# dgaddy/silent_speech

Measured on AMD Instinct MI355X. Metric: EMG frames/s training (transduction_model.py), higher is better.
Workload: dtype bf16

## Files before the change

include/silent_speech_hip.h:

```cpp
#ifndef SILENT_SPEECH_HIP_H
#define SILENT_SPEECH_HIP_H
#include <stdint.h>
#ifdef __cplusplus
extern "C" {
#endif

#define SS_F32 0
#define SS_BF16 1
#define SS_F32X3 3

const char* ss_last_error(void);
#define SS_ABI_VERSION 10
int ss_abi_version(void);
const char* ss_target_arch(void);

typedef struct ss_rowmap {
    int64_t base;
    int64_t batch_stride;
    int64_t row_stride;
    int32_t rows_per_batch;
} ss_rowmap;

typedef struct ss_gemm_epilogue {
    const float* bias;
    const void* gate;
    float gate_scale;
    float alpha;
    int32_t relu;
    float dropout_p;
    uint64_t seed;
    uint32_t rng_stream;
    int32_t mode;
    int32_t col_mod, col_mul, col_div_mul;
    float log_clamp;
    void* c2;
    ss_rowmap cmap2;
    int64_t col_stride2;
    float* col_sum;
    float* col_sumsq;
    const float* col_shift;
    void* planes_hi;
    void* planes_lo;
    int32_t planes_only;
    void* sign_out;
    int64_t sign_pitch;
    const void* gate_bits;
    int64_t gate_bits_pitch;
} ss_gemm_epilogue;

#define SS_OP_KC 0
#define SS_OP_OC 1

int ss_gemm(int dtype_in, int dtype_out, int a_mode, int b_mode, const void* A, const void* B, void* C,
            int M, int N, int K, const ss_rowmap* amap, const ss_rowmap* bmap, const ss_rowmap* cmap,
            const ss_gemm_epilogue* epilogue, int split_k, void* stream);

int ss_split_planes(const float* x, void* hi, void* lo, int64_t n, void* stream);
int ss_gemm_planes(int dtype_out, const void* A_hi, const void* A_lo, const void* B_hi, const void* B_lo, void* C, int M, int N, int K,
                   const ss_rowmap* amap, const ss_rowmap* bmap, const ss_rowmap* cmap, const ss_gemm_epilogue* epilogue, void* stream);
int ss_gemm_sign_bits_supported(int dtype_in, int dtype_out, int a_mode, int b_mode, const void* C, int M, int N, int K, const ss_rowmap* amap,
                                const ss_rowmap* bmap, const ss_rowmap* cmap, const ss_gemm_epilogue* epilogue, int split_k);
int ss_gemm_planes_supported(int dtype_out, const void* C, int M, int N, int K, const ss_rowmap* amap, const ss_rowmap* bmap, const ss_rowmap* cmap,
                             const ss_gemm_epilogue* epilogue);

int ss_gemm_set_blocks_per_cu(int n);
int ss_gemm_last_kernel(void);
int ss_gemm_fuses_column_stats(int dtype_in, int dtype_out, int a_mode, int b_mode, const void* C, int M, int N, int K, const ss_rowmap* amap,
                               const ss_rowmap* bmap, const ss_rowmap* cmap, const ss_gemm_epilogue* epilogue, int split_k);
int ss_gemm_set_option(int what, int value);

typedef struct ss_dw_job {
    const void* A;
    const void* B;
    float* C;
    ss_rowmap amap, bmap;
    int64_t ldc;
    int32_t M, N, K;
    int32_t flags;
} ss_dw_job;
int ss_gemm_dw_grouped(int n_jobs, const ss_dw_job* jobs , void* stream);
int ss_gemm_dw_set_option(int what, int value);

int ss_permute3d(const void* in, int in_dtype, void* out, int out_dtype, int d0, int d1, int d2,
                 int64_t s0, int64_t s1, int64_t s2, int valid1, int valid2, float scale, int accumulate,
                 void* stream);

int ss_permute3d_batch(const void* jobs_dev, const int32_t* job_of_block_dev, int total_blocks, int all_f32, void* stream);

int ss_dtw_source(int n, int m, int64_t stride_i, int64_t stride_j);
int64_t ss_dtw_workspace_bytes(int n, int m, int64_t* sk_bytes, int64_t* dirs_bytes, int64_t* bnd_bytes);
int ss_dtw_align(const float* costs, const int64_t* desc_dev, int n, int max_n, int max_m, void* workspace,
                 int32_t* results, void* stream);
int ss_dtw_align_skewed(const int64_t* desc_dev, int n, void* workspace, int32_t* results, void* stream);
int ss_dtw_cumulative(int dtype, const void* costs, int64_t stride_i, int64_t stride_j, int N, int M, void* dtw_out,
                      int32_t* results, void* stream);

int64_t ss_bn_scratch_floats(int B, int T, int C);
int ss_bn_stats_sums(int dtype, const void* x, int B, int T, int C, int pad, float* scratch, const float* shift, float* sums, void* stream);
int ss_bn_finalize(const float* sums, double n_total, int C, float* mean, float* invstd, float* running_mean, float* running_var,
                   float momentum, float eps, int training, void* stream);
int ss_bn_finalize_shift(const float* sums, const float* shift, double n_total, int C, float* mean, float* invstd, float* running_mean,
                         float* running_var, float momentum, float eps, int training, void* stream);
int ss_bn_apply(int dtype, const void* xa, const float* mean_a, const float* invstd_a, const float* gamma_a, const float* beta_a, int pad_xa,
                const void* xb, const float* mean_b, const float* invstd_b, const float* gamma_b, const float* beta_b, int pad_xb,
                void* y, int pad_y, int B, int T, int C, int relu, void* stream);
int ss_bn_backward_sums(int dtype, const void* dy, int pad_dy, const void* y, int pad_y,
                        const void* xa, int pad_xa, const float* mean_a, const float* invstd_a,
                        const void* xb, int pad_xb, const float* mean_b, const float* invstd_b,
                        float* dgamma_a, float* dbeta_a, float* dgamma_b, float* dbeta_b,
                        float* scratch, float* sums, int B, int T, int C, int relu,
                        const float* gate_gamma_a, const float* gate_beta_a, const float* gate_gamma_b, const float* gate_beta_b, void* stream);
int ss_bn_backward_apply(int dtype, const void* dy, int pad_dy, const void* y, int pad_y,
                         const void* xa, int pad_xa, const float* mean_a, const float* invstd_a, const float* gamma_a,
                         const void* xb, int pad_xb, const float* mean_b, const float* invstd_b, const float* gamma_b,
                         const float* sums, double n_total, void* dxa, int pad_dxa, void* dxb, int pad_dxb,
                         int B, int T, int C, int relu, const float* gate_beta_a, const float* gate_beta_b, void* stream);
int64_t ss_colsum_scratch_floats(int rows, int C);
int ss_colsum(int dtype, const void* x, int rows, int C, int64_t ld, float* scratch, float* out_accum, void* stream);

int ss_add_dropout_layernorm_forward(int dtype, const void* x, void* branch_inout, const float* gamma, const float* beta, void* y,
                                     float* mean, float* rstd, int rows, int C, float eps, float dropout_p, uint64_t seed,
                                     uint32_t rng_stream, void* stream);
int ss_layernorm_backward(int dtype, const void* dy, const void* z, const float* mean, const float* rstd, const float* gamma,
                          void* dres, void* dbranch, float* dgamma, float* dbeta, int rows, int C, float dropout_p, uint64_t seed,
                          uint32_t rng_stream, void* stream);

int ss_layernorm_backward_bias(int dtype, const void* dy, const void* z, const float* mean, const float* rstd, const float* gamma,
                               void* dres, void* dbranch, float* dgamma, float* dbeta, float* dbranch_colsum, int rows, int C, float dropout_p,
                               uint64_t seed, uint32_t rng_stream, void* stream);
int64_t ss_layernorm_backward_scratch_floats(int rows, int C);
int ss_layernorm_backward_ws(int dtype, const void* dy, const void* z, const float* mean, const float* rstd, const float* gamma,
                             void* dres, void* dbranch, float* dgamma, float* dbeta, float* dbranch_colsum, float* scratch, int64_t scratch_floats,
                             int rows, int C, float dropout_p, uint64_t seed, uint32_t rng_stream, void* stream);
int ss_add_dropout_layernorm_forward_planes(int dtype, const void* x, void* branch_inout, const float* gamma, const float* beta, void* y, void* y_hi, void* y_lo,
                                            float* mean, float* rstd, int rows, int C, float eps, float dropout_p, uint64_t seed, uint32_t rng_stream, void* stream);
int ss_layernorm_backward_ws_planes(int dtype, const void* dy, const void* z, const float* mean, const float* rstd, const float* gamma,
                                    void* dres, void* dbranch, void* dbranch_hi, void* dbranch_lo, float* dgamma, float* dbeta, float* dbranch_colsum, float* scratch,
                                    int64_t scratch_floats, int rows, int C, float dropout_p, uint64_t seed, uint32_t rng_stream, void* stream);

int ss_emg_prepare(int dtype, const float* x_raw, void* out_padded, float* shifted_copy, int B, int T0, int Cin, int shift, void* stream);

int ss_loss_index_tables(const int64_t* utt_dev, int n_utt, int32_t* vo_pred, int32_t* vo_tgt, int32_t* si_tgt, int32_t* si_base,
                         int32_t* si_res, void* stream);
int ss_frame_lse(const float* head, int64_t ld, int col0, int ncls, int rows, float* lse, int32_t* argmax, void* stream);
int ss_voiced_loss(const float* head, int64_t ld, int n_mel, int n_phone, const float* lse, const int32_t* argmax, const float* Y,
                   const int64_t* phones, const int32_t* pred_row, const int32_t* tgt_row, int nframes, float lam, float inv_total,
                   float* dhead, float* loss_accum, int32_t* correct_accum, void* stream);
int ss_silent_cost_skewed(const float* head, int64_t ld, int n_mel, const float* lse, const float* Y, const int64_t* phones,
                          const int64_t* desc_dev, int n, int max_n, int max_m, float lam, void* workspace, int32_t* results, void* stream);
int ss_silent_loss(const float* head, int64_t ld, int n_mel, int n_phone, const float* lse, const int32_t* argmax, const float* Y,
                   const int64_t* phones, const int32_t* results, const int32_t* tgt_row, const int32_t* pred_base,
                   const int32_t* res_idx, int nframes, float lam, float inv_total, float* dhead, float* loss_accum,
                   int32_t* correct_accum, void* stream);
int ss_phoneme_confusion(const int32_t* argmax, const int64_t* phones, const int32_t* results, const int32_t* vo_pred, const int32_t* vo_tgt,
                         int n_voiced, const int32_t* si_tgt, const int32_t* si_base, const int32_t* si_res, int n_silent_frames,
                         int32_t* confusion, int n_phone, void* stream);

int ss_ctc_loss(const float* logits, int64_t ld, int V, int blank, const float* lse, const int64_t* desc_dev, int n_utt, int max_target_len,
                int64_t rows, const int32_t* targets, float* alpha_ws, float* beta_ws, float* nll, float* dlogits, float* loss, void* stream);

int ss_adamw_step(float* p, const float* g, float* m, float* v, int64_t n, float lr, float beta1, float beta2, float eps,
                  float weight_decay, int step, float grad_scale, void* stream);
int ss_cast_f32(const float* in, void* out, int out_dtype, int64_t n, void* stream);
int ss_soft_clip(const float* x, float* out, int64_t n, int C, const float* mean, const float* stdv, float pre_div, float limit, void* stream);

int ss_concat_pad(const void* table_dev, int n, void* out, int64_t total_bytes, int granule, void* stream);

int ss_reflect_pad(const float* y, float* out, int B, int L, int pad, int64_t ld_out, void* stream);
int ss_reflect_pad_ragged(const float* y, const int64_t* offsets_dev, const int32_t* lengths_dev, float* out, int B, int min_len,
                          int pad, int64_t ld_out, int clip, void* stream);
int ss_stft_magnitude(const float* spec, int64_t ld_spec, int n_bins, float* mag, int64_t ld_mag, int rows, void* stream);
int ss_stft_logmel_fft(const float* y, const int64_t* offsets_dev, const int32_t* lengths_dev, int64_t uniform_len, int B, int F, int pad, int clip,
                       int n_fft, int hop, const float* window,
                       const int32_t* band_lo, const int32_t* band_cnt, const int32_t* band_off, const float* band_w, const int32_t* lane_bands, int n_mels, int n_w,
                       float log_clamp, float* out, int64_t stride_b, int64_t stride_f, int64_t stride_m, void* stream);

int ss_relpos_attention_needs_transposed(int dtype, int T, int dp, int D);
int ss_relpos_attention_family(int dtype, int T, int dp, int D);
int64_t ss_relpos_attention_table_bytes(int H, int dp, int D);
int ss_relpos_attention_prepare_tables(const float* emb, void* tab, int H, int D, int dh, int dp, float scale, void* stream);
int ss_relpos_attention_forward(int dtype, const void* qkv, const void* qkvT, const void* E, const void* tab, void* out, float* lse,
                                int B, int H, int T, int Tp, int dp, int D, float scale, float dropout_p, uint64_t seed,
                                uint32_t rng_stream, void* stream);
int ss_relpos_attention_backward(int dtype, const void* qkv, const void* qkvT, const void* E, const void* ET, const void* tab, const void* out,
                                 const float* lse, const void* dO, const void* dOT, float* Dscratch, void* dqkv,
                                 int B, int H, int T, int Tp, int dp, int D, float scale, float dropout_p, uint64_t seed,
                                 uint32_t rng_stream, void* stream);

int64_t ss_relpos_attention_saved_bytes(int dtype, int B, int H, int T, int dp, int D);
int ss_relpos_attention_forward_p(int dtype, const void* qkv, const void* qkvT, const void* E, const void* tab, void* out, float* lse, void* pimg,
                                  int B, int H, int T, int Tp, int dp, int D, float scale, float dropout_p, uint64_t seed,
                                  uint32_t rng_stream, void* stream);
int ss_relpos_attention_backward_p(int dtype, const void* qkv, const void* qkvT, const void* E, const void* ET, const void* tab, const void* out,
                                   const float* lse, const void* dO, const void* dOT, float* Dscratch, void* dqkv, const void* pimg,
                                   int B, int H, int T, int Tp, int dp, int D, float scale, float dropout_p, uint64_t seed,
                                   uint32_t rng_stream, void* stream);

int ss_relpos_attention_x3_supported(int T, int dp, int D);
int64_t ss_relpos_attention_x3_saved_bytes(int B, int H, int T, int dp, int D);
int64_t ss_relpos_attention_x3_table_bytes(int H, int dp, int D);
int ss_relpos_attention_x3_prepare_tables(const float* emb, void* tab, int H, int D, int dh, int dp, float scale, void* stream);
// ... 47 lines not shown
```

silent_speech_amd/_lib.py:

```python
import ctypes
import os

import torch

_HERE = os.path.dirname(os.path.abspath(__file__))
_LIB_PATH = os.environ.get('SS_AMD_LIBRARY') or os.path.join(_HERE, 'lib', 'libsilent_speech_hip.so')

SS_F32, SS_BF16, SS_F64, SS_F32X3 = 0, 1, 2, 3
ABI_VERSION = 10
OP_KC, OP_OC = 0, 1


class RowMap(ctypes.Structure):
    _fields_ = [('base', ctypes.c_int64), ('batch_stride', ctypes.c_int64), ('row_stride', ctypes.c_int64),
                ('rows_per_batch', ctypes.c_int32)]


class GemmEpilogue(ctypes.Structure):
    _fields_ = [('bias', ctypes.c_void_p), ('gate', ctypes.c_void_p), ('gate_scale', ctypes.c_float),
                ('alpha', ctypes.c_float), ('relu', ctypes.c_int32), ('dropout_p', ctypes.c_float),
                ('seed', ctypes.c_uint64), ('rng_stream', ctypes.c_uint32), ('mode', ctypes.c_int32),
                ('col_mod', ctypes.c_int32), ('col_mul', ctypes.c_int32), ('col_div_mul', ctypes.c_int32),
                ('log_clamp', ctypes.c_float), ('c2', ctypes.c_void_p), ('cmap2', RowMap), ('col_stride2', ctypes.c_int64),
                ('col_sum', ctypes.c_void_p), ('col_sumsq', ctypes.c_void_p), ('col_shift', ctypes.c_void_p),
                ('planes_hi', ctypes.c_void_p), ('planes_lo', ctypes.c_void_p), ('planes_only', ctypes.c_int32),
                ('sign_out', ctypes.c_void_p), ('sign_pitch', ctypes.c_int64), ('gate_bits', ctypes.c_void_p), ('gate_bits_pitch', ctypes.c_int64)]


class DwJob(ctypes.Structure):
    _fields_ = [('A', ctypes.c_void_p), ('B', ctypes.c_void_p), ('C', ctypes.c_void_p), ('amap', RowMap), ('bmap', RowMap),
                ('ldc', ctypes.c_int64), ('M', ctypes.c_int32), ('N', ctypes.c_int32), ('K', ctypes.c_int32), ('flags', ctypes.c_int32)]


class ProfileRow(ctypes.Structure):
    _fields_ = [('name', ctypes.c_char * 64), ('calls', ctypes.c_int64), ('seconds', ctypes.c_double), ('flops', ctypes.c_double), ('bytes', ctypes.c_double)]


class PermuteJob(ctypes.Structure):
    _fields_ = [('inp', ctypes.c_void_p), ('out', ctypes.c_void_p), ('s0', ctypes.c_int64), ('s1', ctypes.c_int64), ('s2', ctypes.c_int64),
                ('o0', ctypes.c_int64), ('o1', ctypes.c_int64), ('d0', ctypes.c_int32), ('d1', ctypes.c_int32), ('d2', ctypes.c_int32),
                ('valid1', ctypes.c_int32), ('valid2', ctypes.c_int32), ('in_dtype', ctypes.c_int32), ('out_dtype', ctypes.c_int32),
                ('accumulate', ctypes.c_int32), ('scale', ctypes.c_float), ('first_block', ctypes.c_int32), ('nblocks', ctypes.c_int32),
                ('pad_', ctypes.c_int32)]


_P, _I, _F, _L = ctypes.c_void_p, ctypes.c_int, ctypes.c_float, ctypes.c_int64
_U64, _U32 = ctypes.c_uint64, ctypes.c_uint32

SIGNATURES = {
    'ss_gemm': [_I, _I, _I, _I, _P, _P, _P, _I, _I, _I, ctypes.POINTER(RowMap), ctypes.POINTER(RowMap),
                ctypes.POINTER(RowMap), ctypes.POINTER(GemmEpilogue), _I, _P],
    'ss_gemm_dw_grouped': [_I, ctypes.POINTER(DwJob), _P],
    'ss_split_planes': [_P, _P, _P, _L, _P],
    'ss_gemm_planes': [_I, _P, _P, _P, _P, _P, _I, _I, _I, ctypes.POINTER(RowMap), ctypes.POINTER(RowMap), ctypes.POINTER(RowMap), ctypes.POINTER(GemmEpilogue), _P],
    'ss_permute3d': [_P, _I, _P, _I, _I, _I, _I, _L, _L, _L, _I, _I, _F, _I, _P],
    'ss_permute3d_batch': [_P, _P, _I, _I, _P],
    'ss_dtw_align': [_P, _P, _I, _I, _I, _P, _P, _P],
    'ss_dtw_align_skewed': [_P, _I, _P, _P, _P],
    'ss_reflect_pad_ragged': [_P, _P, _P, _P, _I, _I, _I, _L, _I, _P],
    'ss_concat_pad': [_P, _I, _P, _L, _I, _P],
    'ss_dtw_cumulative': [_I, _P, _L, _L, _I, _I, _P, _P, _P],
    'ss_relpos_attention_forward': [_I, _P, _P, _P, _P, _P, _P, _I, _I, _I, _I, _I, _I, _F, _F, _U64, _U32, _P],
    'ss_relpos_attention_backward': [_I, _P, _P, _P, _P, _P, _P, _P, _P, _P, _P, _P, _I, _I, _I, _I, _I, _I, _F, _F, _U64, _U32, _P],
    'ss_relpos_attention_forward_p': [_I, _P, _P, _P, _P, _P, _P, _P, _I, _I, _I, _I, _I, _I, _F, _F, _U64, _U32, _P],
    'ss_relpos_attention_backward_p': [_I, _P, _P, _P, _P, _P, _P, _P, _P, _P, _P, _P, _P, _I, _I, _I, _I, _I, _I, _F, _F, _U64, _U32, _P],
    'ss_relpos_attention_prepare_tables': [_P, _P, _I, _I, _I, _I, _F, _P],
    'ss_relpos_attention_x3_prepare_tables': [_P, _P, _I, _I, _I, _I, _F, _P],
    'ss_relpos_attention_x3_forward': [_P, _P, _P, _P, _P, _P, _P, _I, _I, _I, _I, _I, _F, _F, _U64, _U32, _P],
    'ss_relpos_attention_x3_backward': [_P, _P, _P, _P, _P, _P, _P, _P, _P, _P, _P, _I, _I, _I, _I, _I, _F, _F, _U64, _U32, _P],
    'ss_bn_stats_sums': [_I, _P, _I, _I, _I, _I, _P, _P, _P, _P],
    'ss_bn_finalize': [_P, ctypes.c_double, _I, _P, _P, _P, _P, _F, _F, _I, _P],
    'ss_bn_finalize_shift': [_P, _P, ctypes.c_double, _I, _P, _P, _P, _P, _F, _F, _I, _P],
    'ss_bn_apply': [_I, _P, _P, _P, _P, _P, _I, _P, _P, _P, _P, _P, _I, _P, _I, _I, _I, _I, _I, _P],
    'ss_bn_backward_sums': [_I, _P, _I, _P, _I, _P, _I, _P, _P, _P, _I, _P, _P, _P, _P, _P, _P, _P, _P, _I, _I, _I, _I, _P, _P, _P, _P, _P],
    'ss_bn_backward_apply': [_I, _P, _I, _P, _I, _P, _I, _P, _P, _P, _P, _I, _P, _P, _P, _P, ctypes.c_double, _P, _I, _P, _I, _I, _I, _I, _I, _P, _P, _P],
    'ss_colsum': [_I, _P, _I, _I, _L, _P, _P, _P],
    'ss_add_dropout_layernorm_forward': [_I, _P, _P, _P, _P, _P, _P, _P, _I, _I, _F, _F, _U64, _U32, _P],
    'ss_add_dropout_layernorm_forward_planes': [_I, _P, _P, _P, _P, _P, _P, _P, _P, _P, _I, _I, _F, _F, _U64, _U32, _P],
    'ss_layernorm_backward': [_I, _P, _P, _P, _P, _P, _P, _P, _P, _P, _I, _I, _F, _U64, _U32, _P],
    'ss_layernorm_backward_bias': [_I, _P, _P, _P, _P, _P, _P, _P, _P, _P, _P, _I, _I, _F, _U64, _U32, _P],
    'ss_layernorm_backward_ws': [_I, _P, _P, _P, _P, _P, _P, _P, _P, _P, _P, _P, _L, _I, _I, _F, _U64, _U32, _P],
    'ss_layernorm_backward_ws_planes': [_I, _P, _P, _P, _P, _P, _P, _P, _P, _P, _P, _P, _P, _P, _L, _I, _I, _F, _U64, _U32, _P],
    'ss_emg_prepare': [_I, _P, _P, _P, _I, _I, _I, _I, _P],
    'ss_frame_lse': [_P, _L, _I, _I, _I, _P, _P, _P],
    'ss_loss_index_tables': [_P, _I, _P, _P, _P, _P, _P, _P],
    'ss_voiced_loss': [_P, _L, _I, _I, _P, _P, _P, _P, _P, _P, _I, _F, _F, _P, _P, _P, _P],
    'ss_silent_cost_skewed': [_P, _L, _I, _P, _P, _P, _P, _I, _I, _I, _F, _P, _P, _P],
    'ss_silent_loss': [_P, _L, _I, _I, _P, _P, _P, _P, _P, _P, _P, _P, _I, _F, _F, _P, _P, _P, _P],
    'ss_phoneme_confusion': [_P, _P, _P, _P, _P, _I, _P, _P, _P, _I, _P, _I, _P],
    'ss_ctc_loss': [_P, _L, _I, _I, _P, _P, _I, _I, _L, _P, _P, _P, _P, _P, _P, _P],
    'ss_adamw_step': [_P, _P, _P, _P, _L, _F, _F, _F, _F, _F, _I, _F, _P],
    'ss_cast_f32': [_P, _P, _I, _L, _P],
    'ss_soft_clip': [_P, _P, _L, _I, _P, _P, _F, _F, _P],
    'ss_reflect_pad': [_P, _P, _I, _I, _I, _L, _P],
    'ss_iir_filtfilt': [_P, _P, _I, _I, _I, _P, _P, _L, _P],
    'ss_linear_resample': [_P, _P, _I, _I, ctypes.c_double, ctypes.c_double, _I, _P],
    'ss_iir_filtfilt_batch': [_P, _P, _P, _I, _I, _I, _P, _P, _L, _P],
    'ss_linear_resample_batch': [_P, _P, _P, _I, _I, ctypes.c_double, ctypes.c_double, _L, _P],
    'ss_emg_features_batch': [_P, _P, _P, _I, _I, _L, _P],
    'ss_stft_magnitude': [_P, _L, _I, _P, _L, _I, _P],
    'ss_stft_logmel_fft': [_P, _P, _P, _L, _I, _I, _I, _I, _I, _I, _P, _P, _P, _P, _P, _P, _I, _I, _F, _P, _L, _L, _L, _P],
}
_LP = ctypes.POINTER(ctypes.c_int64)
_HOST_FUNCS = {'ss_dtw_workspace_bytes': ([_I, _I, _LP, _LP, _LP], ctypes.c_int64),
               'ss_dtw_source': ([_I, _I, _L, _L], ctypes.c_int),
               'ss_bn_scratch_floats': ([_I, _I, _I], ctypes.c_int64),
               'ss_iir_filtfilt_workspace_bytes': ([_I, _I, _I], ctypes.c_int64),
               'ss_iir_filtfilt_batch_workspace_bytes': ([_P, _I, _I, _I, _I], ctypes.c_int64),
               'ss_colsum_scratch_floats': ([_I, _I], ctypes.c_int64),
               'ss_gemm_set_blocks_per_cu': ([_I], ctypes.c_int),
               'ss_gemm_last_kernel': ([], ctypes.c_int),
               'ss_gemm_set_option': ([_I, _I], ctypes.c_int),
               'ss_gemm_fuses_column_stats': ([_I, _I, _I, _I, _P, _I, _I, _I, ctypes.POINTER(RowMap), ctypes.POINTER(RowMap), ctypes.POINTER(RowMap),
                                               ctypes.POINTER(GemmEpilogue), _I], ctypes.c_int),
               'ss_gemm_sign_bits_supported': ([_I, _I, _I, _I, _P, _I, _I, _I, ctypes.POINTER(RowMap), ctypes.POINTER(RowMap), ctypes.POINTER(RowMap),
                                                ctypes.POINTER(GemmEpilogue), _I], ctypes.c_int),
               'ss_gemm_planes_supported': ([_I, _P, _I, _I, _I, ctypes.POINTER(RowMap), ctypes.POINTER(RowMap), ctypes.POINTER(RowMap), ctypes.POINTER(GemmEpilogue)], ctypes.c_int),
               'ss_gemm_dw_set_option': ([_I, _I], ctypes.c_int),
               'ss_plan_create': ([_P], _P), 'ss_plan_destroy': ([_P], None), 'ss_plan_slot_count': ([_P], ctypes.c_int),
               'ss_plan_slot_name': ([_P, _I], ctypes.c_char_p), 'ss_plan_bind': ([_P, _I, _P], ctypes.c_int),
               'ss_plan_set_option': ([_P, _I, _I], ctypes.c_int), 'ss_plan_set_reduce_hook': ([_P, _P, _P], ctypes.c_int),
               'ss_plan_set_event_hook': ([_P, _P, _P], ctypes.c_int), 'ss_plan_ctx_bytes': ([], ctypes.c_int64),
               'ss_plan_workspace_bytes': ([_P, _I, _I, _I], ctypes.c_int64),
               'ss_plan_forward': ([_P, _P, _P, _P, _L, _I, _I, _I, _I, _F, _U64, _P, _P, _P], ctypes.c_int),
               'ss_plan_backward': ([_P, _P, _P, _P, _P], ctypes.c_int),
               'ss_counters_add': ([_I, _P, _L, _P], ctypes.c_int),
               'ss_plan_profile': ([_P, _I], ctypes.c_int), 'ss_plan_profile_read': ([_P, _P, _I], ctypes.c_int),
               'ss_relpos_attention_needs_transposed': ([_I, _I, _I, _I], ctypes.c_int),
               'ss_relpos_attention_family': ([_I, _I, _I, _I], ctypes.c_int),
               'ss_relpos_attention_table_bytes': ([_I, _I, _I], ctypes.c_int64),
               'ss_relpos_attention_x3_supported': ([_I, _I, _I], ctypes.c_int),
               'ss_relpos_attention_x3_saved_bytes': ([_I, _I, _I, _I, _I], ctypes.c_int64),
               'ss_relpos_attention_x3_table_bytes': ([_I, _I, _I], ctypes.c_int64),
               'ss_relpos_attention_saved_bytes': ([_I, _I, _I, _I, _I, _I], ctypes.c_int64),
               'ss_layernorm_backward_scratch_floats': ([_I, _I], ctypes.c_int64)}
_RESTYPES = {'ss_last_error': ctypes.c_char_p, 'ss_target_arch': ctypes.c_char_p, 'ss_abi_version': ctypes.c_int}

_lib = None
_is_emulator = False


def _declare(lib):
    for name, restype in _RESTYPES.items():
        fn = getattr(lib, name)
        fn.restype = restype
        fn.argtypes = []
    for name, argtypes in SIGNATURES.items():
        fn = getattr(lib, name)
        fn.argtypes = argtypes
        fn.restype = ctypes.c_int
    for name, (argtypes, restype) in _HOST_FUNCS.items():
        fn = getattr(lib, name)
        fn.argtypes = argtypes
        fn.restype = restype
    return lib


def load(path=None, _testing=False):
    global _lib, _is_emulator
# ... 75 lines not shown
```

silent_speech_amd/csrc/gemm8_dw.hip:

```cpp
#include "gemm8_common.h"

struct DwJob {
    const bf16_t* A; const bf16_t* B; float* C;
    RowMap amap, bmap;
    long long ldc;
    int M, N, K;
    int tiles_n, ntiles, split, k_chunk, item0, nitem, atomic;
};
constexpr int DW_MAX_JOBS = 24;
struct DwJobs { DwJob job[DW_MAX_JOBS]; int n; };

namespace g8 {
constexpr int TRP = 544;
constexpr int TR_STAGE = 2 * 64 * TRP;

template <int NR>
struct StageTR8 {
    static constexpr int RS = 64 / NR;
    const unsigned char* pa; const unsigned char* pb;
    unsigned offa[NR], offb[NR];
    int tt[NR];
    int c, r0, rpb, wraps;
    unsigned stepa, stepb, wrapa, wrapb;
    __device__ __forceinline__ void init(const DwJob& J, int m0, int n0, int k_begin, int tid) {
        c = tid & 31; r0 = tid >> 5;
        const int ca = m0 + c * 8 < J.M ? m0 + c * 8 : 0, cb = n0 + c * 8 < J.N ? n0 + c * 8 : 0;
        pa = (const unsigned char*)(J.A + J.amap.base + ca); pb = (const unsigned char*)(J.B + J.bmap.base + cb);
        rpb = J.amap.rows_per_batch;
        wraps = rpb >= BK8 ? 1 : (BK8 + rpb - 1) / rpb;
        stepa = (unsigned)(J.amap.row_stride * BK8 * 2); stepb = (unsigned)(J.bmap.row_stride * BK8 * 2);
        wrapa = (unsigned)((J.amap.batch_stride - (long long)rpb * J.amap.row_stride) * 2);
        wrapb = (unsigned)((J.bmap.batch_stride - (long long)rpb * J.bmap.row_stride) * 2);
#pragma unroll
        for (int i = 0; i < NR; ++i) {
            const int rr = k_begin + r0 + RS * i;
            int b_ = 0, t_ = rr;
            if (rpb != 0x7fffffff) { b_ = rr / rpb; t_ = rr - b_ * rpb; }
            tt[i] = t_;
            offa[i] = (unsigned)(((long long)b_ * J.amap.batch_stride + (long long)t_ * J.amap.row_stride) * 2);
            offb[i] = (unsigned)(((long long)b_ * J.bmap.batch_stride + (long long)t_ * J.bmap.row_stride) * 2);
        }
    }
    __device__ __forceinline__ void advance() {
#pragma unroll
        for (int i = 0; i < NR; ++i) {
            tt[i] += BK8; offa[i] += stepa; offb[i] += stepb;
            for (int w = 0; w < wraps; ++w) { const bool over = tt[i] >= rpb; tt[i] -= over ? rpb : 0; offa[i] += over ? wrapa : 0u; offb[i] += over ? wrapb : 0u; }
        }
    }
    template <bool PRED>
    __device__ __forceinline__ void load(int k0, int kend, u32x4 (&ra)[NR], u32x4 (&rb)[NR]) {
#pragma unroll
        for (int i = 0; i < NR; ++i) {
            if (PRED) {
                u32x4 z = {0u, 0u, 0u, 0u};
                const bool v = k0 + r0 + RS * i < kend;
                ra[i] = v ? *(const u32x4*)(pa + offa[i]) : z;
                rb[i] = v ? *(const u32x4*)(pb + offb[i]) : z;
            } else {
                ra[i] = *(const u32x4*)(pa + offa[i]);
                rb[i] = *(const u32x4*)(pb + offb[i]);
            }
        }
    }
    __device__ __forceinline__ void store(unsigned char* stage, const u32x4 (&ra)[NR], const u32x4 (&rb)[NR]) {
#pragma unroll
        for (int i = 0; i < NR; ++i) { *(u32x4*)(stage + (r0 + RS * i) * TRP + c * 16) = ra[i]; *(u32x4*)(stage + (64 + r0 + RS * i) * TRP + c * 16) = rb[i]; }
    }
};
__device__ __forceinline__ bf16x8 tr_frag8(const unsigned char* tile, int sub, int kk, int c, int q) {
    const unsigned char* a0 = tile + (kk * 32 + q * 4 + (c >> 2)) * TRP + sub * 32 + (c & 3) * 8;
    const s16x4 lo = lds_read_tr16(a0), hi = lds_read_tr16(a0 + 16 * TRP);
    bf16x8 f = {lo[0], lo[1], lo[2], lo[3], hi[0], hi[1], hi[2], hi[3]};
    return f;
}
}

template <int PIN, int NW>
__global__ __launch_bounds__(NW * 64) void gemm8_dw_kernel(DwJobs jobs, int nitems, int xorder)
{
    constexpr int NWN = NW / 2, NJ = 16 / NWN, NR = 2048 / (NW * 64);
    using namespace g8;
    SS_DYN_SMEM(lds_raw);
    unsigned char* lds = (unsigned char*)lds_raw;
    const int tid = threadIdx.x, lane = tid & 63, c = lane & 15, q = lane >> 4;
    const int wave = wave_uniform(tid >> 6);
    const int wm = wave / NWN, wn = wave % NWN, G = gridDim.x;
    StageTR8<NR> st;
    u32x4 ra[NR], rb[NR];
    int it = blockIdx.x, ji = 0, m0, n0, k_begin, k_end, nsteps;

#define G8_SETUP()                                                                                                          \
    do {                                                                                                                     \
                                                                                   \
        const int ch0_ = it / G * G, pos_ = it - ch0_;                                                                       \
        int R_ = nitems - ch0_; R_ = R_ > G ? G : R_;                                                                        \
        const int xq_ = R_ >> 3, xr_ = R_ & 7, xcd_ = pos_ & 7;                                                             \
        const int lit = xorder ? ch0_ + (xcd_ < xr_ ? xcd_ * (xq_ + 1) : xr_ * (xq_ + 1) + (xcd_ - xr_) * xq_) + (pos_ >> 3) : it; \
        ji = 0;                                                                                                              \
        while (ji + 1 < jobs.n && lit >= jobs.job[ji].item0 + jobs.job[ji].nitem) ++ji;                                     \
        const DwJob& J_ = jobs.job[ji];                                                                                      \
        const int local = lit - J_.item0, z = local / J_.ntiles, tile = local - z * J_.ntiles;                               \
        const int mt_ = tile / J_.tiles_n, nt_ = tile - mt_ * J_.tiles_n;                                                    \
        m0 = mt_ * 256; n0 = nt_ * 256;                                                                                      \
        k_begin = z * J_.k_chunk; k_end = min(J_.K, k_begin + J_.k_chunk);                                                   \
        nsteps = (k_end - k_begin + BK8 - 1) / BK8;                                                                          \
        st.init(J_, m0, n0, k_begin, tid);                                                                                   \
        if (nsteps == 1) st.template load<true>(k_begin, k_end, ra, rb); else if (nsteps > 1) st.template load<false>(k_begin, k_end, ra, rb); \
    } while (0)

    G8_SETUP();
    for (;;) {
        f32x4 acc[8][NJ];
#pragma unroll
        for (int i = 0; i < 8; ++i)
#pragma unroll
            for (int j = 0; j < NJ; ++j) { f32x4 z = {0.f, 0.f, 0.f, 0.f}; acc[i][j] = z; }
        if (nsteps > 0) st.store(lds, ra, rb);
        __syncthreads();
        for (int s = 0; s < nsteps; ++s) {
            const int cur = s & 1;
            const bool more = s + 1 < nsteps;
            if (more) {
                st.advance();
                const int k0 = k_begin + (s + 1) * BK8;
                if (s + 2 == nsteps) st.template load<true>(k0, k_end, ra, rb); else st.template load<false>(k0, k_end, ra, rb);
            }
            const unsigned char* As = lds + cur * TR_STAGE;
            const unsigned char* Bs = As + 64 * TRP;
#pragma unroll
            for (int kk = 0; kk < 2; ++kk) {
                bf16x8 a[8], b[NJ];
#pragma unroll
                for (int i = 0; i < 8; ++i) a[i] = tr_frag8(As, wm * 8 + i, kk, c, q);
#pragma unroll
                for (int j = 0; j < NJ; ++j) b[j] = tr_frag8(Bs, wn * NJ + j, kk, c, q);
                if (PIN) sched_fence();
#pragma unroll
                for (int i = 0; i < 8; ++i)
#pragma unroll
                    for (int j = 0; j < NJ; ++j) acc[i][j] = mfma_bf16_16x16x32(a[i], b[j], acc[i][j]);
                if (PIN) sched_fence();
            }
            if (more) st.store(lds + (cur ^ 1) * TR_STAGE, ra, rb);
            __syncthreads();
        }
        const DwJob& J = jobs.job[ji];
        float* Cj = J.C; const long long ldc = J.ldc; const int Mj = J.M, Nj = J.N, atomic = J.atomic, cm0 = m0, cn0 = n0;
        const bool has_next = it + G < nitems;
        if (has_next) { it += G; G8_SETUP(); }
#pragma unroll
        for (int i = 0; i < 8; ++i)
#pragma unroll
            for (int j = 0; j < NJ; ++j) {
                const int col = cn0 + (wn * NJ + j) * 16 + c, row0 = cm0 + (wm * 8 + i) * 16 + q * 4;
                if (col < Nj) {
#pragma unroll
                    for (int reg = 0; reg < 4; ++reg) {
                        if (row0 + reg < Mj) {
                            float* dst = Cj + (long long)(row0 + reg) * ldc + col;
                            if (atomic) atomicAdd(dst, acc[i][j][reg]); else *dst += acc[i][j][reg];
                        }
                    }
                }
            }
        if (!has_next) break;
    }
#undef G8_SETUP
}

namespace g8 {
constexpr int KP = 144;
constexpr int KS = 34;
constexpr int KROWS = 8 * KS;
constexpr int KT_STAGE = 2 * KROWS * KP;

__device__ __forceinline__ unsigned perm_lo(unsigned hi_src, unsigned lo_src) {
#if defined(SS_EMU)
    return (lo_src & 0xffffu) | (hi_src << 16);
#else
    return __builtin_amdgcn_perm(hi_src, lo_src, 0x05040100u);
#endif
}
__device__ __forceinline__ unsigned perm_hi(unsigned hi_src, unsigned lo_src) {
#if defined(SS_EMU)
    return (lo_src >> 16) | (hi_src & 0xffff0000u);
#else
    return __builtin_amdgcn_perm(hi_src, lo_src, 0x07060302u);
#endif
}

struct StageKT {
    const unsigned char* p;
    unsigned off[2], step, wrap, rs;
    int tt[2], rpb, kb;
    unsigned wr;
    __device__ __forceinline__ void init(const DwJob& J, int opsel, int m0, int n0, int k_begin, int wave, int lane) {
        const int c = (lane & 15) + 16 * (wave & 1), r = (lane >> 4) + 4 * ((wave >> 1) & 1);
        const RowMap& map = opsel ? J.bmap : J.amap;
        const int outer = opsel ? n0 : m0, lim = opsel ? J.N : J.M;
        const int col = outer + c * 8 < lim ? outer + c * 8 : 0;
        p = (const unsigned char*)((opsel ? J.B : J.A) + map.base + col);
        rpb = map.rows_per_batch; kb = 4 * r;
        rs = (unsigned)(map.row_stride * 2); step = (unsigned)(map.row_stride * BK8 * 2);
        wrap = (unsigned)((map.batch_stride - (long long)rpb * map.row_stride) * 2);
#pragma unroll
        for (int h = 0; h < 2; ++h) {
            const int rr = k_begin + 32 * h + kb;
            int b_ = 0, t_ = rr;
            if (rpb != 0x7fffffff) { b_ = rr / rpb; t_ = rr - b_ * rpb; }
            tt[h] = t_;
            off[h] = (unsigned)(((long long)b_ * map.batch_stride + (long long)t_ * map.row_stride) * 2);
        }
        wr = (unsigned)((opsel * KROWS + c) * KP + r * 8);
    }
    template <int H>
    __device__ __forceinline__ void advance() {
        tt[H] += BK8; off[H] += step;
        const bool over = tt[H] >= rpb; tt[H] -= over ? rpb : 0; off[H] += over ? wrap : 0u;
    }
    template <int H, bool PRED>
    __device__ __forceinline__ void load(int k0, int kend, u32x4 (&L)[4]) {
        const unsigned char* q = p + off[H];
        if constexpr (PRED) {
            u32x4 T[4];
#pragma unroll
            for (int i = 0; i < 4; ++i) { const u32x4 z = {0u, 0u, 0u, 0u}; T[i] = k0 + 32 * H + kb + i < kend ? *(const u32x4*)(q + i * rs) : z; }
#if !defined(SS_EMU)
            __builtin_amdgcn_s_waitcnt(0x0F70);
#endif
#pragma unroll
            for (int i = 0; i < 4; ++i) L[i] = T[i];
        } else {
#pragma unroll
            for (int i = 0; i < 4; ++i) {
#if defined(SS_EMU)
                L[i] = *(const u32x4*)(q + i * rs);
#else
                asm volatile("global_load_dwordx4 %0, %1, off" : "=v"(L[i]) : "v"(q + i * rs) : "memory");
#endif
            }
        }
    }
    template <int N>
    __device__ __forceinline__ static void wait_vm(u32x4 (&L)[4]) {
#if !defined(SS_EMU)
        asm volatile("s_waitcnt vmcnt(%4)" : "+v"(L[0]), "+v"(L[1]), "+v"(L[2]), "+v"(L[3]) : "n"(N));
#endif
// ... 56 lines not shown
    } while (0)

    G8K_SETUP();
    for (;;) {
        f32x4 acc[8][4];
#pragma unroll
        for (int i = 0; i < 8; ++i)
#pragma unroll
            for (int j = 0; j < 4; ++j) { f32x4 z = {0.f, 0.f, 0.f, 0.f}; acc[i][j] = z; }
        bf16x8 fa[2][HR], fb[2][4];
        auto read_a = [&](auto phc, auto xc, unsigned sb) {
            constexpr int ph = phc, x = xc, kk = ph / NPK, i = (ph % NPK) * HR + x;
            lds_read128_async<i * 2 * KP + kk * 64>(fa[ph & 1][x], lds, lbase + sb + aoff);
        };
        auto read_b = [&](auto phc, auto jc, unsigned sb) {
            constexpr int ph = phc, j = jc, kk = ph / NPK;
            lds_read128_async<j * 2 * KP + kk * 64>(fb[kk][j], lds, lbase + sb + boff);
        };
        auto wait_frags = [&](auto phc) {
            constexpr int ph = phc;
            lds_wait_pin(fa[ph & 1]);
            if constexpr (ph % NPK == 0) lds_wait_pin(fb[ph / NPK]);
        };
        auto mfma_row = [&](auto phc, auto xc) {
            constexpr int ph = phc, x = xc, kk = ph / NPK, i = (ph % NPK) * HR + x;
#pragma unroll
            for (int j = 0; j < 4; ++j) acc[i][j] = mfma_bf16_16x16x32(fa[ph & 1][x], fb[kk][j], acc[i][j]);
        };
        auto phase = [&](auto phc, auto steady_c, auto shc, const unsigned S, const unsigned O, const int s) {
            constexpr int ph = phc, nx = ph + 1 < NPH ? ph + 1 : 0, SH = shc;
            constexpr bool last = ph + 1 == NPH, STEADY = steady_c;
            bool rd = true; unsigned rst = S;
            if constexpr (last) {
                if (STEADY || s + 1 < nsteps) { barrier_lds(); rst = O; }
                else rd = false;
            }
            static_for<0, HR>([&](auto xc) {
                constexpr int x = xc, g = ph * HR + x;
                if (rd) {
                    read_a(std::integral_constant<int, nx>{}, xc, rst);
                    if constexpr (nx % NPK == 0) static_for<x * 4 / HR, (x + 1) * 4 / HR>([&](auto j) { read_b(std::integral_constant<int, nx>{}, j, rst); });
                }
                const bool wr_ok = (STEADY && !(ABL & 2)) || (!STEADY && s + 1 < nsteps);
                if constexpr (g == 0 + SH) { if (wr_ok) { if (STEADY) StageKT::wait_vm<4>(L0); else StageKT::wait_vm<0>(L0); st.template write2<0, 0>(lds + O, L0); st.template write2<0, 1>(lds + O, L0); } }
                if constexpr (g == 1 + SH) { if (wr_ok) { st.template write2<0, 2>(lds + O, L0); st.template write2<0, 3>(lds + O, L0); } }
                if constexpr (g == 8 + SH) { if (wr_ok) { if (STEADY) StageKT::wait_vm<4>(L1); else StageKT::wait_vm<0>(L1); st.template write2<1, 0>(lds + O, L1); st.template write2<1, 1>(lds + O, L1); } }
                if constexpr (g == 9 + SH) { if (wr_ok) { st.template write2<1, 2>(lds + O, L1); st.template write2<1, 3>(lds + O, L1); } }
                if constexpr (g == 2 + SH) {
                    if (STEADY) { st.template advance<0>(); if (!(ABL & 1)) st.template load<0, false>(0, 0, L0); }
                    else if (s + 2 < nsteps) { st.template advance<0>(); st.template load<0, true>(k_begin + (s + 2) * BK8, k_end, L0); }
                }
                if constexpr (g == 10 + SH) {
                    if (STEADY) { st.template advance<1>(); if (!(ABL & 1)) st.template load<1, false>(0, 0, L1); }
                    else if (s + 2 < nsteps) { st.template advance<1>(); st.template load<1, true>(k_begin + (s + 2) * BK8, k_end, L1); }
                }
                sched_fence();
                if (!(STEADY && (ABL & 4))) mfma_row(phc, xc);
                sched_fence();
            });
            if (rd) wait_frags(std::integral_constant<int, nx>{});
            sched_fence();
        };
        if (nsteps > 0) { StageKT::wait_vm<0>(L0); StageKT::wait_vm<0>(L1); st.template write_all<0>(lds + cur * KT_STAGE, L0); st.template write_all<1>(lds + cur * KT_STAGE, L1); }
        if (nsteps > 1) {
            st.template advance<0>(); st.template advance<1>();
            if (nsteps == 2) { st.template load<0, true>(k_begin + BK8, k_end, L0); st.template load<1, true>(k_begin + BK8, k_end, L1); }
            else { st.template load<0, false>(0, 0, L0); st.template load<1, false>(0, 0, L1); }
        }
        barrier_lds();
        if (nsteps > 0) {
            static_for<0, HR>([&](auto x) { read_a(std::integral_constant<int, 0>{}, x, (unsigned)(cur * KT_STAGE)); });
            static_for<0, 4>([&](auto j) { read_b(std::integral_constant<int, 0>{}, j, (unsigned)(cur * KT_STAGE)); });
            wait_frags(std::integral_constant<int, 0>{});
        }
        sched_fence();
        {
            auto run = [&](auto shc) {
                int s = 0;
                for (; s + 3 < nsteps; ++s) { const unsigned S = cur * KT_STAGE, O = (cur ^ 1) * KT_STAGE; static_for<0, NPH>([&](auto ph) { phase(ph, std::true_type{}, shc, S, O, s); }); cur ^= 1; }
                for (; s < nsteps; ++s) { const unsigned S = cur * KT_STAGE, O = (cur ^ 1) * KT_STAGE; static_for<0, NPH>([&](auto ph) { phase(ph, std::false_type{}, shc, S, O, s); }); cur ^= 1; }
            };
            if (SHIFT && opsel) run(std::integral_constant<int, 2>{}); else run(std::integral_constant<int, 0>{});
        }
        const DwJob& J = jobs.job[ji];
        float* Cj = J.C; const long long ldc = J.ldc; const int Mj = J.M, Nj = J.N, atomic = J.atomic, cm0 = m0, cn0 = n0;
        const bool has_next = it + G < nitems;
        if (has_next) { it += G; G8K_SETUP(); }
#pragma unroll
        for (int i = 0; i < 8; ++i)
#pragma unroll
            for (int j = 0; j < 4; ++j) {
                const int col = cn0 + (wn * 4 + j) * 16 + c, row0 = cm0 + (wm * 8 + i) * 16 + q * 4;
                if (col < Nj && !((ABL & 8) && acc[i][j][0] != 12345.f)) {
#pragma unroll
                    for (int reg = 0; reg < 4; ++reg) {
                        if (row0 + reg < Mj) {
                            float* dst = Cj + (long long)(row0 + reg) * ldc + col;
                            if (atomic) atomicAdd(dst, acc[i][j][reg]); else *dst += acc[i][j][reg];
                        }
                    }
                }
            }
        if (!has_next) break;
    }
#undef G8K_SETUP
}

static thread_local int g_dw_split_override = 0, g_dw_pin = 1, g_dw_xorder = -1, g_dw_kt = -1;
extern "C" int ss_gemm_dw_set_option(int what, int value) {
    int old = 0;
    if (what == 0) { old = g_dw_split_override; g_dw_split_override = value; }
    else if (what == 1) { old = g_dw_pin; g_dw_pin = value; }
    else if (what == 2) { old = g_dw_xorder; g_dw_xorder = value; }
    else if (what == 3) { old = g_dw_kt; g_dw_kt = value; }
    return old;
}

extern "C" int ss_gemm_dw_grouped(int n_jobs, const ss_dw_job* jobs, void* stream)
{
    SS_CHECK(jobs && n_jobs >= 1 && n_jobs <= DW_MAX_JOBS, "ss_gemm_dw_grouped: 1..%d jobs per launch", DW_MAX_JOBS);
    DwJobs J; memset(&J, 0, sizeof(J));
    J.n = n_jobs;
    long long tiles_total = 0; int kmax = 0;
    int s_flags[DW_MAX_JOBS];
    for (int i = 0; i < n_jobs; ++i) {
        const ss_dw_job& s = jobs[i];
        s_flags[i] = s.flags;
        SS_CHECK(s.A && s.B && s.C, "ss_gemm_dw_grouped: null pointer in job %d", i);
        SS_CHECK(s.M > 0 && s.N > 0 && s.K > 0 && s.M % 8 == 0 && s.N % 8 == 0, "ss_gemm_dw_grouped: job %d: M=%d, N=%d must be positive multiples of 8 (16-byte rows), K=%d > 0", i, s.M, s.N, s.K);
        SS_CHECK(((uintptr_t)s.A) % 16 == 0 && ((uintptr_t)s.B) % 16 == 0, "ss_gemm_dw_grouped: job %d: operands must be 16-byte aligned", i);
        const ss_rowmap* maps[2] = {&s.amap, &s.bmap};
        for (int o = 0; o < 2; ++o)
            SS_CHECK(maps[o]->base % 8 == 0 && maps[o]->batch_stride % 8 == 0 && maps[o]->row_stride % 8 == 0, "ss_gemm_dw_grouped: job %d operand %d: strides must be multiples of 8 elements", i, o);
        DwJob& d = J.job[i];
        d.A = (const bf16_t*)s.A; d.B = (const bf16_t*)s.B; d.C = s.C; d.ldc = s.ldc; d.M = s.M; d.N = s.N; d.K = s.K;
        d.amap.base = s.amap.base; d.amap.batch_stride = s.amap.batch_stride; d.amap.row_stride = s.amap.row_stride; d.amap.rows_per_batch = s.amap.rows_per_batch > 0 ? s.amap.rows_per_batch : 0x7fffffff;
        d.bmap.base = s.bmap.base; d.bmap.batch_stride = s.bmap.batch_stride; d.bmap.row_stride = s.bmap.row_stride; d.bmap.rows_per_batch = s.bmap.rows_per_batch > 0 ? s.bmap.rows_per_batch : 0x7fffffff;
        SS_CHECK(d.amap.rows_per_batch == d.bmap.rows_per_batch, "ss_gemm_dw_grouped: job %d: both operands must split their rows into batches of the same length", i);
        d.tiles_n = (s.N + 255) / 256; d.ntiles = ((s.M + 255) / 256) * d.tiles_n;
        tiles_total += d.ntiles; kmax = s.K > kmax ? s.K : kmax;
    }
    const int cus = g8_cus();
    int split = (int)(cus / (tiles_total > 0 ? tiles_total : 1)); split = split < 1 ? 1 : split;
    if (tiles_total > cus) {
        const int ks = (kmax + 63) / 64;
        double best = 0;
        for (int cand = 1; cand <= 8; ++cand) {
            const long long items = tiles_total * cand, rounds = (items + cus - 1) / cus;
            const double cost = (double)rounds * ((ks + cand - 1) / cand + 12);
            if (cand == 1 || cost < best) { best = cost; split = cand; }
        }
    }
    if (g_dw_split_override > 0) split = g_dw_split_override;
    int item0 = 0;
    for (int i = 0; i < n_jobs; ++i) {
        DwJob& d = J.job[i];
        const int ksteps = (d.K + 63) / 64;
        int sp = split; if (sp > ksteps / 4) sp = ksteps / 4 > 0 ? ksteps / 4 : 1;
        const int per = (ksteps + sp - 1) / sp;
        d.k_chunk = per * 64; d.split = (ksteps + per - 1) / per;
        d.atomic = (d.split > 1 || (s_flags[i] & 1)) ? 1 : 0;
        d.item0 = item0; d.nitem = d.ntiles * d.split; item0 += d.nitem;
    }
    const int nitems = item0;
    if (g_dw_xorder < 0) { const char* e = getenv("SS_GEMM_DW_XCD"); g_dw_xorder = e ? atoi(e) : 1; }
    dim3 grid(nitems < cus ? nitems : cus), block(512);
    if (g_dw_kt < 0) { const char* e = getenv("SS_GEMM_DW_KT"); g_dw_kt = e ? atoi(e) : 4; }
    bool kt_ok = g_dw_kt != 0;
    for (int i = 0; i < n_jobs; ++i) { const int rpb = J.job[i].amap.rows_per_batch; if (rpb != 0x7fffffff && (rpb % 8 != 0 || rpb < 64)) kt_ok = false; }
    if (kt_ok) {
        const size_t smem = 2 * g8::KT_STAGE;
#define G8_DWK(HR_)                                                                                                          \
    do {                                                                                                                      \
        static bool granted = false;                                                                                          \
        if (!granted) { if (g8_grant((const void*)gemm8_dwk_kernel<HR_, ABL_>, smem)) return 1; granted = true; }             \
        SS_LAUNCH(SS_KERNEL(gemm8_dwk_kernel<HR_, ABL_>), grid, block, smem, stream, J, nitems, g_dw_xorder);                 \
    } while (0)
#define ABL_ 0
        static const int abl = getenv("SS_GEMM_DW_ABL") ? atoi(getenv("SS_GEMM_DW_ABL")) : 0;
        if (abl == 0) { if (g_dw_kt == 2) G8_DWK(2); else G8_DWK(4); }
#undef ABL_
#if defined(G8_DW_ABLATION)
#define ABL_CASE(A_) else if (abl == A_) { constexpr int ABL_ = A_; G8_DWK(4); }
        ABL_CASE(1) ABL_CASE(2) ABL_CASE(3) ABL_CASE(4) ABL_CASE(8) ABL_CASE(11) ABL_CASE(7)
#undef ABL_CASE
#endif
        else { ss_set_error("ss_gemm_dw_grouped: SS_GEMM_DW_ABL needs a -DG8_DW_ABLATION build"); return 1; }
#undef G8_DWK
        SS_LAUNCH_CHECK("ss_gemm_dw_grouped");
        return 0;
    }
    const size_t smem = 2 * g8::TR_STAGE;
#define G8_DW(PIN_, NW_)                                                                                                     \
    do {                                                                                                                      \
        static bool granted = false;                                                                                          \
        if (!granted) { if (g8_grant((const void*)gemm8_dw_kernel<PIN_, NW_>, smem)) return 1; granted = true; }              \
        SS_LAUNCH(SS_KERNEL(gemm8_dw_kernel<PIN_, NW_>), grid, block, smem, stream, J, nitems, g_dw_xorder);                  \
    } while (0)
    if (g_dw_pin) G8_DW(1, 8); else G8_DW(0, 8);
#undef G8_DW
    SS_LAUNCH_CHECK("ss_gemm_dw_grouped");
    return 0;
}
```

silent_speech_amd/csrc/norm.hip:

```cpp
#include "common.h"
#include <stdlib.h>
#include "silent_speech_hip.h"

namespace {
struct Seq {
    int T, pad;
    __device__ __forceinline__ long long row(int r) const { int b = r / T, t = r - b * T; return (long long)b * (T + 2 * pad) + pad + t; }
    __device__ __forceinline__ long long at(int b, int t) const { return (long long)b * (T + 2 * pad) + pad + t; }
};

__device__ __forceinline__ void ld8(const float* __restrict__ p, float (&v)[8]) {
    const f32x4 a = *(const f32x4*)p, b = *(const f32x4*)(p + 4);
    v[0] = a[0]; v[1] = a[1]; v[2] = a[2]; v[3] = a[3]; v[4] = b[0]; v[5] = b[1]; v[6] = b[2]; v[7] = b[3];
}

struct ColMap {
    int CV, CVb, RY, cx0, ry; bool active;
    __device__ __forceinline__ ColMap(int C, int tid, int nthreads) {
        CV = C >> 3; CVb = CV < nthreads ? CV : nthreads; RY = nthreads / CVb;
        cx0 = tid % CVb; ry = tid / CVb; active = ry < RY;
    }
};
constexpr int RED_THREADS = 256;

// ... 512 lines not shown
                  (const TT*)xb, sb, mean_b, invstd_b, gate_gamma_a, gate_beta_a, gate_gamma_b, gate_beta_b, rows, C, rpc, relu, scratch);       \
    SS_LAUNCH(bn_bwd_finalize_kernel, dim3((C + 31) / 32), dim3(256), 0, stream, (const float*)scratch, nch, C, sums, dgamma_a, dbeta_a, dgamma_b, dbeta_b)
    if (dtype == SS_BF16) { SS_BNB(bf16_t); } else { SS_BNB(float); }
#undef SS_BNB
    SS_LAUNCH_CHECK("ss_bn_backward_sums");
    return 0;
}

extern "C" int ss_bn_backward_apply(int dtype, const void* dy, int pad_dy, const void* y, int pad_y,
                                    const void* xa, int pad_xa, const float* mean_a, const float* invstd_a, const float* gamma_a,
                                    const void* xb, int pad_xb, const float* mean_b, const float* invstd_b, const float* gamma_b,
                                    const float* sums, double n_total, void* dxa, int pad_dxa, void* dxb, int pad_dxb,
                                    int B, int T, int C, int relu, const float* gate_beta_a, const float* gate_beta_b, void* stream)
{
    SS_CHECK(dy && xa && mean_a && invstd_a && gamma_a && dxa && sums, "ss_bn_backward_apply: null pointer");
    SS_CHECK(!relu || y || gate_beta_a, "ss_bn_backward_apply: relu backward needs the saved output or the affine parameters to recompute its sign");
    SS_CHECK(!gate_beta_a || !xb || gate_beta_b, "ss_bn_backward_apply: gate recomputation needs beta of every branch");
    SS_CHECK(!xb || (mean_b && invstd_b && gamma_b && dxb), "ss_bn_backward_apply: second branch incomplete");
    SS_CHECK(C % 8 == 0 && C > 0 && B > 0 && T > 0 && n_total >= 1.0, "ss_bn_backward_apply: bad shape");
    Seq sdy = {T, pad_dy}, sy = {T, pad_y}, sa = {T, pad_xa}, sb = {T, pad_xb}, sda = {T, pad_dxa}, sdb = {T, pad_dxb};
    const int padmax = pad_dxa > pad_dxb ? pad_dxa : pad_dxb;
    const long long total = (long long)B * (T + 2 * padmax) * (C / 8);
    SS_CHECK(total < (1LL << 31) - (1LL << 22), "ss_bn_backward_apply: tensor too large for 32-bit chunk indices");
    const float inv_n = (float)(1.0 / n_total);
#define SS_BNA(TT)                                                                                                                             \
    if (relu && gate_beta_a)                                                                                                                  \
        SS_LAUNCH(SS_KERNEL(bn_bwd_apply_kernel<TT, true>), ew_grid(total, 256, C / 8), dim3(256), 0, stream, (const TT*)dy, sdy, (const TT*)y, sy, (const TT*)xa, sa, mean_a, invstd_a, gamma_a, \
                  (const TT*)xb, sb, mean_b, invstd_b, gamma_b, sums, inv_n, (TT*)dxa, sda, (TT*)dxb, sdb, B, C, relu, gate_beta_a, gate_beta_b); \
    else                                                                                                                                      \
        SS_LAUNCH(SS_KERNEL(bn_bwd_apply_kernel<TT, false>), ew_grid(total, 256, C / 8), dim3(256), 0, stream, (const TT*)dy, sdy, (const TT*)y, sy, (const TT*)xa, sa, mean_a, invstd_a, gamma_a, \
                  (const TT*)xb, sb, mean_b, invstd_b, gamma_b, sums, inv_n, (TT*)dxa, sda, (TT*)dxb, sdb, B, C, relu, gate_beta_a, gate_beta_b)
    if (dtype == SS_BF16) { SS_BNA(bf16_t); } else { SS_BNA(float); }
#undef SS_BNA
    SS_LAUNCH_CHECK("ss_bn_backward_apply");
    return 0;
}

template <class T>
__global__ __launch_bounds__(RED_THREADS) void colsum_partial_kernel(const T* __restrict__ x, int rows, int C, long long ld, int rows_per_chunk, float* __restrict__ partial)
{
    __shared__ float red[RED_THREADS * 8];
    ColMap m(C, threadIdx.x, (int)blockDim.x);
    const int r0 = blockIdx.x * rows_per_chunk, r1 = min(rows, r0 + rows_per_chunk);
    for (int cb = 0; cb < m.CV; cb += m.CVb) {
        const int cx = cb + m.cx0;
        float s[8];
#pragma unroll
        for (int e = 0; e < 8; ++e) s[e] = 0.f;
        const bool cv = m.active && cx < m.CV;
        if (cv) {
            int r = r0 + m.ry;
            for (; r + 3 * m.RY < r1; r += 4 * m.RY) {
                float v[4][8];
#pragma unroll
                for (int u = 0; u < 4; ++u) Vec8<T>::load(x + (long long)(r + u * m.RY) * ld + cx * 8, v[u]);
#pragma unroll
                for (int e = 0; e < 8; ++e) s[e] += (v[0][e] + v[1][e]) + (v[2][e] + v[3][e]);
            }
            for (; r < r1; r += m.RY) { float v[8]; Vec8<T>::load(x + (long long)r * ld + cx * 8, v);
#pragma unroll
                for (int e = 0; e < 8; ++e) s[e] += v[e]; }
        }
        __syncthreads();
#pragma unroll
        for (int e = 0; e < 8; ++e) red[threadIdx.x * 8 + e] = s[e];
        __syncthreads();
        if (cv && m.ry == 0) {
            for (int yy = 1; yy < m.RY; ++yy)
#pragma unroll
                for (int e = 0; e < 8; ++e) s[e] += red[(yy * m.CVb + m.cx0) * 8 + e];
#pragma unroll
            for (int e = 0; e < 8; ++e) partial[(long long)blockIdx.x * C + cx * 8 + e] = s[e];
        }
    }
}

__global__ __launch_bounds__(256) void colsum_finalize_kernel(const float* __restrict__ partial, int nchunks, int C, float* __restrict__ out)
{
    float t[1]; int c;
    if (!chunk_reduce<1>(partial, nchunks, C, t, c)) return;
    out[c] += t[0];
}

static int colsum_chunks(int rows) { int c = (rows + 31) / 32; if (c > 512) c = 512; if (c < 1) c = 1; return c; }
extern "C" int64_t ss_colsum_scratch_floats(int rows, int C) { return (int64_t)colsum_chunks(rows) * C; }

extern "C" int ss_colsum(int dtype, const void* x, int rows, int C, int64_t ld, float* scratch, float* out_accum, void* stream)
{
    SS_CHECK(x && out_accum && scratch, "ss_colsum: null pointer");
    SS_CHECK(C % 8 == 0 && C > 0 && rows >= 0 && ld % 8 == 0, "ss_colsum: C and ld must be multiples of 8");
    if (rows == 0) return 0;
    const int nch = colsum_chunks(rows), rpc = (rows + nch - 1) / nch;
    if (dtype == SS_BF16) SS_LAUNCH(colsum_partial_kernel<bf16_t>, dim3(nch), dim3(red_threads(C)), 0, stream, (const bf16_t*)x, rows, C, (long long)ld, rpc, scratch);
    else SS_LAUNCH(colsum_partial_kernel<float>, dim3(nch), dim3(red_threads(C)), 0, stream, (const float*)x, rows, C, (long long)ld, rpc, scratch);
    SS_LAUNCH(colsum_finalize_kernel, dim3((C + 31) / 32), dim3(256), 0, stream, (const float*)scratch, nch, C, out_accum);
    SS_LAUNCH_CHECK("ss_colsum");
    return 0;
}

template <class T, int NV>
__global__ __launch_bounds__(256) void add_dropout_ln_fwd_kernel(const T* __restrict__ x, T* __restrict__ a_z, const float* __restrict__ gamma, const float* __restrict__ beta,
                                                                 T* __restrict__ y, float* __restrict__ mean, float* __restrict__ rstd, int rows, int C, float eps,
                                                                 unsigned thresh, float keep_scale, unsigned long long seed, unsigned stream_id,
                                                                 bf16_t* __restrict__ y_hi = nullptr, bf16_t* __restrict__ y_lo = nullptr)
{
    const int lane = threadIdx.x & 63, wpb = blockDim.x >> 6, CV = C >> 3;
    typedef typename RawVec8<T>::type Raw;
    constexpr bool HOIST = NV <= 2;
    float gm[HOIST ? NV : 1][8], bt[HOIST ? NV : 1][8];
    if (HOIST) {
#pragma unroll
        for (int i = 0; i < NV; ++i) {
            const int cx = lane + 64 * i, cc = cx < CV ? cx : CV - 1;
            ld8(gamma + cc * 8, gm[HOIST ? i : 0]); ld8(beta + cc * 8, bt[HOIST ? i : 0]);
        }
    }
    const int rstep = gridDim.x * wpb;
    int r = blockIdx.x * wpb + (threadIdx.x >> 6);
    Raw nx[NV], na[NV];
    auto fetch = [&](int row) {
#pragma unroll
        for (int i = 0; i < NV; ++i) {
            const int cx = lane + 64 * i;
            if (cx < CV) { nx[i] = RawVec8<T>::load(x + (long long)row * C + cx * 8); na[i] = RawVec8<T>::load(a_z + (long long)row * C + cx * 8); }
            else { nx[i] = RawVec8<T>::zero(); na[i] = RawVec8<T>::zero(); }
        }
    };
    if (r < rows) fetch(r);
    for (; r < rows; r += rstep) {
        Raw cx_[NV], ca_[NV];
#pragma unroll
        for (int i = 0; i < NV; ++i) { cx_[i] = nx[i]; ca_[i] = na[i]; }
        if (r + rstep < rows) fetch(r + rstep);
        float z[NV][8];
        float s = 0.f;
#pragma unroll
        for (int i = 0; i < NV; ++i) {
            const int cx = lane + 64 * i;
            if (cx < CV) {
                float xv[8], av[8];
                RawVec8<T>::unpack(cx_[i], xv); RawVec8<T>::unpack(ca_[i], av);
                bool kp[8];
#pragma unroll
                for (int e = 0; e < 8; ++e) kp[e] = true;
                if (thresh) {
                    bool k0[4], k1[4];
                    dropout_keep4(seed, stream_id, ((unsigned long long)r * C + cx * 8) >> 2, thresh, k0);
                    dropout_keep4(seed, stream_id, (((unsigned long long)r * C + cx * 8) >> 2) + 1, thresh, k1);
#pragma unroll
                    for (int e = 0; e < 4; ++e) { kp[e] = k0[e]; kp[4 + e] = k1[e]; }
                }
#pragma unroll
                for (int e = 0; e < 8; ++e) {
                    float br = av[e];
                    if (thresh) br = kp[e] ? br * keep_scale : 0.f;
                    z[i][e] = rnd<T>(xv[e] + br);
                    s += z[i][e];
                }
                Vec8<T>::store(a_z + (long long)r * C + cx * 8, z[i]);
            } else {
#pragma unroll
                for (int e = 0; e < 8; ++e) z[i][e] = 0.f;
            }
        }
        const float mu = wave_sum(s) / (float)C;
        float q = 0.f;
#pragma unroll
        for (int i = 0; i < NV; ++i)
            if (lane + 64 * i < CV)
#pragma unroll
                for (int e = 0; e < 8; ++e) { const float d = z[i][e] - mu; q += d * d; }
        const float rs = rsqrtf(wave_sum(q) / (float)C + eps);
        if (lane == 0) { mean[r] = mu; rstd[r] = rs; }
#pragma unroll
        for (int i = 0; i < NV; ++i) {
            const int cx = lane + 64 * i;
            if (cx < CV) {
                float o[8];
                if (!HOIST) { ld8(gamma + cx * 8, gm[0]); ld8(beta + cx * 8, bt[0]); }
// ... 380 lines not shown
```

silent_speech_amd/csrc/plan.hip:

```cpp
#include "common.h"
#include "silent_speech_hip.h"
#include <math.h>
#include <stdlib.h>
#include <string>
#include <vector>

namespace {

struct BnP { float *gamma = 0, *beta = 0, *rmean = 0, *rvar = 0, *dgamma = 0, *dbeta = 0; long long* nbt = 0; };
struct PermB { void* jobs = 0; void* blocks = 0; long long total = 0, all_f32 = 0; };
struct BlockP {
    void *w1f = 0, *w2f = 0, *wr = 0, *wrT = 0, *w2b = 0, *w1b_even = 0, *w1b_odd = 0;
    float *b1 = 0, *br = 0, *b2 = 0;
    BnP bn1, bn2, bnr;
    float *c2_stage = 0, *c1_stage = 0, *wr_grad = 0;
    PermB unpack;
    int O = 0, I = 0;
};
struct LayerP {
    void *wqkv = 0, *wqkvT = 0, *wo = 0, *woT = 0, *E = 0, *ET = 0, *EF = 0, *w1 = 0, *w2 = 0, *w1T = 0, *w2T = 0;
    float *b1 = 0, *b2 = 0, *g1 = 0, *be1 = 0, *g2 = 0, *be2 = 0;
    float *dg1 = 0, *dbe1 = 0, *dg2 = 0, *dbe2 = 0, *dw1 = 0, *db1 = 0, *dw2 = 0, *db2 = 0, *wo_stage = 0, *wqkv_stage = 0;
    PermB unpack;
};

struct BlockCtx { void *xin, *c1, *cr, *h1, *c2, *y; float *m1, *i1, *m2, *i2, *mr, *ir, *scratch; int Tin, Cin, Tout, O, pad_y; };
struct LayerCtx { void *x, *qkv, *qkvT, *o, *z1, *y1, *hid, *z2, *pimg; float *lse, *mean1, *rstd1, *mean2, *rstd2; unsigned char* hid_sign; };
constexpr int MAX_LAYERS = 16;
constexpr int MAX_PLANES = 384;
struct PlaneCache { int n; const void* key[MAX_PLANES]; void* hi[MAX_PLANES]; long long elems[MAX_PLANES]; };
struct Ctx {
    int B, T0, T, M, Tp, need_T, n_layers;
    float p_drop, scale; unsigned long long seed;
    BlockCtx blk[3];
    LayerCtx layer[MAX_LAYERS];
    void *conv_out, *x_final;
    PlaneCache planes;
    unsigned long long ws_used;
    char* ws; unsigned long long ws_bytes;
};

struct Exec {
    bool dry; char* base; size_t off, cap; void* stream; void* side;
    void* alloc(size_t bytes) { off = (off + 255) & ~(size_t)255; char* p = base + off; off += bytes; return p; }
};

static ss_rowmap RM(long long row_stride, int rows_per_batch = 0, long long batch_stride = 0, long long base = 0) {
    ss_rowmap m; m.base = base; m.batch_stride = batch_stride; m.row_stride = row_stride; m.rows_per_batch = rows_per_batch; return m;
}
static ss_gemm_epilogue EPI() { ss_gemm_epilogue e; memset(&e, 0, sizeof(e)); e.alpha = 1.f; e.gate_scale = 1.f; return e; }
static int round_up(int x, int m) { return (x + m - 1) / m * m; }

typedef double (*reduce_fn)(void* user, float* sums, int n_floats, double n_local, void* stream);
typedef void (*event_fn)(void* user, int what, void* stream);

struct Plan {
    ss_model_dims D;
    std::vector<std::string> names; std::vector<void**> targets;
    BlockP blk[3]; std::vector<LayerP> layers;
    void *w_raw_in = 0, *w_raw_in_T = 0, *w_head = 0, *w_head_T = 0;
    float *b_raw_in = 0, *dw_raw_in = 0, *db_raw_in = 0, *b_head = 0, *head_w_stage = 0, *head_b_stage = 0, *stage_arena = 0;
    long long stage_arena_bytes = 0;
    PermB unpack_enc, unpack_all;
    reduce_fn hook = 0; void* hook_user = 0;
    event_fn on_event = 0; void* event_user = 0;
    int side_enabled = 1, dw_grouped = 1, side_blocks = 2, fuse_stats = 1, regate_on = 1, f32_x3 = 0;
    int x3_attn = 0;
    int sign_gate = 1;
    int x3_emit = 1;
    int x3_planes = 1;
    Ctx* cur = nullptr;
    bool use_planes() const { return D.dtype == SS_F32 && f32_x3 && x3_planes; }
    bool use_x3_attention(int T) const { return use_planes() && x3_attn && dw_grouped && ss_relpos_attention_x3_supported(T, D.dp, D.max_rel); }
    void adopt_planes(const void* key, void* hi, long long n) {
        PlaneCache& pc = cur->planes;
        if (key && pc.n < MAX_PLANES) { pc.key[pc.n] = key; pc.hi[pc.n] = hi; pc.elems[pc.n] = n; ++pc.n; }
    }
    int keep_input = 0;
    hipEvent_t ev_fork = 0, ev_join = 0;
    size_t esz() const { return D.dtype == SS_BF16 ? 2 : 4; }

    struct ProfRec { const char* tag; int sub; double flops, bytes; hipEvent_t e0, e1; };
    bool profiling = false;
    std::vector<ProfRec> recs; std::vector<hipEvent_t> ev_pool; size_t ev_used = 0;
    hipEvent_t prof_event() {
#if !defined(SS_EMU)
        if (ev_used == ev_pool.size()) { hipEvent_t e; hipEventCreate(&e); ev_pool.push_back(e); }
        return ev_pool[ev_used++];
#else
        return 0;
#endif
    }
    template <class F>
    int timed(Exec& X, const char* tag, double flops, double bytes, void* stream, F&& f, bool gemm_sub = false) {
        if (X.dry) return f();
#if !defined(SS_EMU)
        if (profiling) {
            ProfRec r{tag, 0, flops, bytes, prof_event(), prof_event()};
            hipEventRecord(r.e0, (hipStream_t)stream);
            const int rc = f();
            hipEventRecord(r.e1, (hipStream_t)stream);
            if (gemm_sub) r.sub = ss_gemm_last_kernel();
            recs.push_back(r);
            return rc;
        }
#endif
        return f();
    }

    void slot(const std::string& n, void** t) { names.push_back(n); targets.push_back(t); }
    void slot_bn(const std::string& p, BnP& b) {
        slot(p + ".weight", (void**)&b.gamma); slot(p + ".bias", (void**)&b.beta); slot(p + ".running_mean", (void**)&b.rmean); slot(p + ".running_var", (void**)&b.rvar);
        slot(p + ".weight.grad", (void**)&b.dgamma); slot(p + ".bias.grad", (void**)&b.dbeta); slot(p + ".num_batches_tracked", (void**)&b.nbt);
    }
    void slot_perm(const std::string& p, PermB& b) { slot(p + ".jobs", &b.jobs); slot(p + ".blocks", &b.blocks); slot(p + ".total", (void**)&b.total); slot(p + ".all_f32", (void**)&b.all_f32); }

    explicit Plan(const ss_model_dims& d) : D(d), layers(d.n_layers) {
        for (int i = 0; i < 3; ++i) {
            const std::string p = "conv_blocks." + std::to_string(i) + ".";
            BlockP& b = blk[i];
            b.O = D.d_model; b.I = i == 0 ? 8 : D.d_model;
            slot(p + "w1f", &b.w1f); slot(p + "w2f", &b.w2f); slot(p + "wr", &b.wr); slot(p + "wrT", &b.wrT); slot(p + "w2b", &b.w2b);
            if (i > 0) { slot(p + "w1b_even", &b.w1b_even); slot(p + "w1b_odd", &b.w1b_odd); }
            slot(p + "conv1.bias", (void**)&b.b1); slot(p + "residual_path.bias", (void**)&b.br); slot(p + "conv2.bias", (void**)&b.b2);
            slot_bn(p + "bn1", b.bn1); slot_bn(p + "bn2", b.bn2); slot_bn(p + "res_norm", b.bnr);
            slot(p + "conv2.weight.stage", (void**)&b.c2_stage); slot(p + "conv1.weight.stage", (void**)&b.c1_stage); slot(p + "residual_path.weight.grad", (void**)&b.wr_grad);
            slot_perm(p + "unpack", b.unpack);
        }
        slot("w_raw_in", &w_raw_in); slot("w_raw_in_T", &w_raw_in_T); slot("w_raw_in.bias", (void**)&b_raw_in);
        slot("w_raw_in.weight.grad", (void**)&dw_raw_in); slot("w_raw_in.bias.grad", (void**)&db_raw_in);
        for (int l = 0; l < D.n_layers; ++l) {
            const std::string p = "transformer.layers." + std::to_string(l) + ".";
            LayerP& L = layers[l];
            slot(p + "wqkv", &L.wqkv); slot(p + "wqkvT", &L.wqkvT); slot(p + "wo", &L.wo); slot(p + "woT", &L.woT); slot(p + "E", &L.E); slot(p + "ET", &L.ET); slot(p + "EF", &L.EF);
            slot(p + "w1", &L.w1); slot(p + "w2", &L.w2); slot(p + "w1T", &L.w1T); slot(p + "w2T", &L.w2T);
            slot(p + "linear1.bias", (void**)&L.b1); slot(p + "linear2.bias", (void**)&L.b2);
            slot(p + "norm1.weight", (void**)&L.g1); slot(p + "norm1.bias", (void**)&L.be1); slot(p + "norm2.weight", (void**)&L.g2); slot(p + "norm2.bias", (void**)&L.be2);
            slot(p + "norm1.weight.grad", (void**)&L.dg1); slot(p + "norm1.bias.grad", (void**)&L.dbe1); slot(p + "norm2.weight.grad", (void**)&L.dg2); slot(p + "norm2.bias.grad", (void**)&L.dbe2);
            slot(p + "linear1.weight.grad", (void**)&L.dw1); slot(p + "linear1.bias.grad", (void**)&L.db1); slot(p + "linear2.weight.grad", (void**)&L.dw2); slot(p + "linear2.bias.grad", (void**)&L.db2);
            slot(p + "w_o.stage", (void**)&L.wo_stage); slot(p + "w_qkv.stage", (void**)&L.wqkv_stage);
            slot_perm(p + "unpack", L.unpack);
        }
        slot("w_head", &w_head); slot("w_head_T", &w_head_T); slot("b_head", (void**)&b_head);
        slot("head_w.stage", (void**)&head_w_stage); slot("head_b.stage", (void**)&head_b_stage);
        slot("stage_arena", (void**)&stage_arena); slot("stage_arena.bytes", (void**)&stage_arena_bytes);
        slot_perm("unpack_encoder", unpack_enc); slot_perm("unpack_encoder_all", unpack_all);
    }

    static long long extent(const ss_rowmap& m, int rows, int row_len) {
        const long long nb = m.rows_per_batch > 0 ? (rows - 1) / m.rows_per_batch : 0, rr = m.rows_per_batch > 0 ? (rows < m.rows_per_batch ? rows : m.rows_per_batch) - 1 : rows - 1;
        return m.base + nb * m.batch_stride + rr * m.row_stride + row_len;
    }
    struct Pl { void* hi; void* lo; };
    Pl new_planes(Exec& X, const void* key, long long n) {
        if (!(use_planes() && x3_emit)) return Pl{nullptr, nullptr};
        n = (n + 7) & ~7LL;
        void* hi = X.alloc((size_t)n * 4);
        adopt_planes(key, hi, n);
        return Pl{hi, (char*)hi + n * 2};
    }
    Pl planes(Exec& X, const void* key, const void* src, long long n) {
        PlaneCache& pc = cur->planes;
        if (key) for (int i = 0; i < pc.n; ++i) if (pc.key[i] == key && pc.elems[i] >= n) return Pl{pc.hi[i], (char*)pc.hi[i] + pc.elems[i] * 2};
        n = (n + 7) & ~7LL;
        void* hi = X.alloc((size_t)n * 4);
        if (key && pc.n < MAX_PLANES) { pc.key[pc.n] = key; pc.hi[pc.n] = hi; pc.elems[pc.n] = n; ++pc.n; }
        if (!X.dry) {
            if (timed(X, "split_planes", 0, (double)n * 8, X.stream, [&] { return ss_split_planes((const float*)src, hi, (char*)hi + n * 2, n, X.stream); })) return Pl{nullptr, nullptr};
        }
        return Pl{hi, (char*)hi + n * 2};
    }

    int gemm(Exec& X, int dt_out, const void* A, const void* B, void* C, int M, int N, int K, ss_rowmap am, ss_rowmap bm, ss_rowmap cm, const ss_gemm_epilogue* e = 0,
             int a_mode = SS_OP_KC, int b_mode = SS_OP_KC, int split = 1, void* stream = 0, const void* wkey = nullptr, int emit = 0) {
        void* st = stream ? stream : X.stream;
        if (use_planes() && st == X.stream && a_mode == SS_OP_KC && b_mode == SS_OP_KC && dt_out == SS_F32 && split == 1 &&
            ss_gemm_planes_supported(SS_F32, C, M, N, K, &am, &bm, &cm, e)) {
            const Pl a = planes(X, A, A, extent(am, M, K)), b = planes(X, wkey ? wkey : B, B, extent(bm, N, K));
            ss_gemm_epilogue ee = e ? *e : EPI();
            if (emit && x3_emit) {
                const long long n = (extent(cm, M, N) + 7) & ~7LL;
                void* hi = X.alloc((size_t)n * 4);
                adopt_planes(C, hi, n);
                ee.planes_hi = hi; ee.planes_lo = (char*)hi + n * 2; ee.planes_only = emit == 2;
            }
            if (X.dry) return 0;
            if (!a.hi || !b.hi) return 1;
            return timed(X, "gemm", 2.0 * M * N * K, ((double)M * K + (double)N * K) * 4 + (double)M * N * 4.0, st,
                         [&] { return ss_gemm_planes(SS_F32, a.hi, a.lo, b.hi, b.lo, C, M, N, K, &am, &bm, &cm, &ee, st); }, true);
        }
        if (X.dry) return 0;
        const double ob = dt_out == SS_BF16 ? 2.0 : 4.0;
        return timed(X, a_mode == SS_OP_OC && b_mode == SS_OP_OC ? "gemm_dw" : "gemm", 2.0 * M * N * K, ((double)M * K + (double)N * K) * esz() + (double)M * N * ob, st,
                     [&] { return ss_gemm(D.dtype == SS_F32 && f32_x3 ? SS_F32X3 : D.dtype, dt_out, a_mode, b_mode, A, B, C, M, N, K, &am, &bm, &cm, e, split, st); }, true);
    }
    int colsum(Exec& X, const void* x, int rows, int C, float* out, void* stream) {
        float* scratch = (float*)X.alloc((size_t)ss_colsum_scratch_floats(rows, C) * 4);
        if (X.dry) return 0;
        return timed(X, "colsum", 0, (double)rows * C * esz(), stream, [&] { return ss_colsum(D.dtype, x, rows, C, C, scratch, out, stream); });
    }
    int permute_batch(Exec& X, const PermB& b, void* stream) {
        if (X.dry || !b.jobs || b.total <= 0) return 0;
        return timed(X, "grad_unlayout", 0, 0, stream, [&] { return ss_permute3d_batch(b.jobs, (const int32_t*)b.blocks, (int)b.total, (int)b.all_f32, stream); });
    }
    int bn_stats(Exec& X, const void* x, int B, int T, int C, float* scratch, BnP& bn, bool training, float** mean, float** invstd, float* fused = nullptr, double reduced_n = 0.0) {
        *mean = (float*)X.alloc((size_t)C * 4); *invstd = (float*)X.alloc((size_t)C * 4);
        float* sums = (training && !fused) ? (float*)X.alloc((size_t)3 * C * 4) : fused;
        if (X.dry) return 0;
        double n_total = (double)B * T;
        if (training) {
            if (!fused && timed(X, "bn_stats", 0, (double)B * T * C * esz(), X.stream, [&] { return ss_bn_stats_sums(D.dtype, x, B, T, C, 0, scratch, hook ? bn.rmean : nullptr, sums, X.stream); })) return 1;
            if (reduced_n > 0.0) n_total = reduced_n;
            else if (hook) n_total = hook(hook_user, sums, 2 * C, n_total, X.stream);
        }
        if (fused) return timed(X, "bn_finalize", 0, 0, X.stream, [&] { return ss_bn_finalize_shift(sums, bn.rmean, n_total, C, *mean, *invstd, bn.rmean, bn.rvar, 0.1f, 1e-5f, 1, X.stream); });
        return timed(X, "bn_finalize", 0, 0, X.stream, [&] { return ss_bn_finalize(sums, n_total, C, *mean, *invstd, bn.rmean, bn.rvar, 0.1f, 1e-5f, training ? 1 : 0, X.stream); });
    }
    float* conv_gemm(Exec& X, const void* A, const void* Bw, void* C, int M, int N, int K, ss_rowmap am, ss_rowmap bm, const float* bias, BnP& bn, float* stat_slot, int* rc) {
        ss_gemm_epilogue e = EPI(); e.bias = bias;
        ss_rowmap cm = RM(N);
        float* fused = nullptr;
        if (!X.dry && stat_slot && fuse_stats) {
            ss_gemm_epilogue es = e; es.col_sum = stat_slot; es.col_sumsq = stat_slot + N; es.col_shift = bn.rmean;
            const bool ok = use_planes() ? ss_gemm_planes_supported(SS_F32, C, M, N, K, &am, &bm, &cm, &es) != 0
                                         : ss_gemm_fuses_column_stats(D.dtype, D.dtype, SS_OP_KC, SS_OP_KC, C, M, N, K, &am, &bm, &cm, &e, 1) != 0;
            if (ok) { fused = stat_slot; e = es; }
        }
        *rc = gemm(X, D.dtype, A, Bw, C, M, N, K, am, bm, cm, &e);
        return fused;
    }
    void fork(Exec& X) {
#if !defined(SS_EMU)
        if (X.dry || !X.side || X.side == X.stream) return;
        hipEventRecord(ev_fork, (hipStream_t)X.stream); hipStreamWaitEvent((hipStream_t)X.side, ev_fork, 0);
#endif
    }
    void join(Exec& X) {
#if !defined(SS_EMU)
        if (X.dry || !X.side || X.side == X.stream) return;
        hipEventRecord(ev_join, (hipStream_t)X.side); hipStreamWaitEvent((hipStream_t)X.stream, ev_join, 0);
#endif
    }
    int split_k(int M, int N, int K, bool overlapped) const {
        const int tiles = ((M + 127) / 128) * ((N + 127) / 128);
        int s = (overlapped ? 400 : 512) / (tiles > 0 ? tiles : 1); s = s < 1 ? 1 : (s > 64 ? 64 : s);
        const int cap = K >= 512 ? K / 512 : 1;
        return s < cap ? s : (cap < 1 ? 1 : cap);
    }

    struct DwGroup {
        Plan* P; Exec* X; bool grouped; int n = 0; ss_dw_job jobs[24];
        int add(const void* dy, const void* x, float* grad, int N, int K, int rows, ss_rowmap am, ss_rowmap bm, void* stream) {
            if (grouped && P->use_planes()) {
                if (n + 3 > 24 && launch(stream)) return 1;
                const Pl a = P->planes(*X, dy, dy, extent(am, rows, N)), b = P->planes(*X, x, x, extent(bm, rows, K));
                if (X->dry) return 0;
                if (!a.hi || !b.hi) return 1;
                const void* as[3] = {a.lo, a.hi, a.hi}; const void* bs[3] = {b.hi, b.lo, b.hi};
                for (int t = 0; t < 3; ++t) {
                    ss_dw_job& j = jobs[n++]; memset(&j, 0, sizeof(j));
                    j.A = as[t]; j.B = bs[t]; j.C = grad; j.amap = am; j.bmap = bm; j.ldc = K; j.M = N; j.N = K; j.K = rows; j.flags = 1;
                }
                return 0;
            }
            if (grouped) {
                if (n == 8 && launch(stream)) return 1;
                ss_dw_job& j = jobs[n++]; memset(&j, 0, sizeof(j));
                j.A = dy; j.B = x; j.C = grad; j.amap = am; j.bmap = bm; j.ldc = K; j.M = N; j.N = K; j.K = rows;
                return 0;
            }
            ss_gemm_epilogue e = EPI(); e.mode = 2;
            const bool ov = X->side && X->side != X->stream;
            P->fork(*X);
            if (ov) ss_gemm_set_blocks_per_cu(P->side_blocks);
            const int rc = P->gemm(*X, SS_F32, dy, x, grad, N, K, rows, am, bm, RM(K), &e, SS_OP_OC, SS_OP_OC, P->split_k(N, K, rows, ov), stream);
            if (ov) ss_gemm_set_blocks_per_cu(2);
            return rc;
        }
        int launch(void* stream) {
            int rc = 0;
            if (n && !X->dry) {
                double fl = 0, by = 0;
                const double pl = P->use_planes() ? 3.0 : 1.0;
                for (int i = 0; i < n; ++i) { fl += 2.0 * jobs[i].M * jobs[i].N * jobs[i].K / pl; by += ((double)jobs[i].M + jobs[i].N) * jobs[i].K * 2.0 + (double)jobs[i].M * jobs[i].N * 4.0 / pl; }
                rc = P->timed(*X, "gemm_dw_grouped", fl, by, stream, [&] { return ss_gemm_dw_grouped(n, jobs, stream); });
            }
            n = 0; return rc;
        }
    };

    int forward(Exec& X, const float* x_raw, float* shifted, int B, int T0, int training, int shift_r, float p_drop, unsigned long long seed, float* head, Ctx* c);
    int backward(Exec& X, Ctx* c, const float* dhead);
};

#define L_(call) do { if (call) return 1; } while (0)

static double band_pairs(int T, int D) { double n = 0; for (int q = 0; q < T; ++q) { const int lo = q - (D - 1) < 0 ? 0 : q - (D - 1), hi = q + (D - 1) > T - 1 ? T - 1 : q + (D - 1); n += hi - lo + 1; } return n; }

int Plan::forward(Exec& X, const float* x_raw, float* shifted, int B, int T0, int training, int shift_r, float p_drop, unsigned long long seed, float* head, Ctx* c)
{
    const int dt = D.dtype, d = D.d_model; const size_t es = esz();
    const int Cin0 = 8;
    SS_CHECK(T0 % 8 == 0, "raw EMG length %d must be a multiple of 8 (three stride-2 convolutions)", T0);
    SS_CHECK(D.n_layers <= MAX_LAYERS, "at most %d encoder layers", MAX_LAYERS);
    void* stream = X.stream;
    cur = c; c->planes.n = 0;
    if (!training) p_drop = 0.f;
    c->B = B; c->T0 = T0; c->p_drop = p_drop; c->seed = seed; c->n_layers = D.n_layers;

    void* xin = X.alloc((size_t)B * (T0 + 2) * Cin0 * es);
    if (!X.dry) {
        L_(timed(X, "emg_prepare", 0, (double)B * T0 * Cin0 * (4 + es), stream, [&] { return ss_emg_prepare(dt, x_raw, xin, (training && shift_r > 0) ? shifted : nullptr, B, T0, Cin0, training ? shift_r : 0, stream); }));
        if (training && shift_r > 0 && shifted && !keep_input)
            if (!ss_copy_d2d_async((void*)x_raw, shifted, (size_t)B * T0 * Cin0 * 4, stream)) { ss_set_error("forward: input write-back failed"); return 1; }
    }
    float* bnsums = training ? (float*)X.alloc((size_t)9 * 2 * d * 4) : nullptr;
    if (bnsums && !X.dry) {
        if (!ss_memset_async(bnsums, 0, (size_t)9 * 2 * d * 4, stream)) { ss_set_error("forward: memset failed"); return 1; }
    }
    int Tin = T0, Cin = Cin0;
    for (int i = 0; i < 3; ++i) {
        BlockP& w = blk[i]; BlockCtx& s = c->blk[i];
        const int O = w.O, Tout = Tin / 2, rows = B * Tout;
        s.xin = xin; s.Tin = Tin; s.Cin = Cin; s.Tout = Tout; s.O = O;
        s.scratch = (float*)X.alloc((size_t)ss_bn_scratch_floats(B, Tout, O) * 4);
        const long long in_bs = (long long)(Tin + 2) * Cin;
        int rc = 0;
        float* slot = bnsums ? bnsums + (size_t)i * 3 * 2 * d : nullptr;
        void* c1 = X.alloc((size_t)rows * O * es);
        float* f1 = conv_gemm(X, xin, w.w1f, c1, rows, O, 3 * Cin, RM(2 * Cin, Tout, in_bs), RM(3 * Cin), w.b1, w.bn1, slot, &rc); L_(rc);
        void* cr = X.alloc((size_t)rows * O * es);
        float* fr = conv_gemm(X, xin, w.wr, cr, rows, O, Cin, RM(2 * Cin, Tout, in_bs, Cin), RM(Cin), w.br, w.bnr, slot ? slot + 2 * d : nullptr, &rc); L_(rc);
        double nred = 0.0;
        if (training && hook && f1 && fr == f1 + 2 * d && O == d && !X.dry) nred = hook(hook_user, f1, 4 * O, (double)B * Tout, stream);
        L_(bn_stats(X, c1, B, Tout, O, s.scratch, w.bn1, training, &s.m1, &s.i1, f1, nred));
        void* h1 = X.alloc((size_t)B * (Tout + 2) * O * es);
        if (!X.dry) L_(timed(X, "bn_apply", 0, (double)B * Tout * O * es * 2, stream, [&] { return ss_bn_apply(dt, c1, s.m1, s.i1, w.bn1.gamma, w.bn1.beta, 0, nullptr, nullptr, nullptr, nullptr, nullptr, 0, h1, 1, B, Tout, O, 1, stream); }));
        void* c2 = X.alloc((size_t)rows * O * es);
        float* f2 = conv_gemm(X, h1, w.w2f, c2, rows, O, 3 * O, RM(O, Tout, (long long)(Tout + 2) * O), RM(3 * O), w.b2, w.bn2, slot ? slot + 4 * d : nullptr, &rc); L_(rc);
        L_(bn_stats(X, c2, B, Tout, O, s.scratch, w.bn2, training, &s.m2, &s.i2, f2));
        L_(bn_stats(X, cr, B, Tout, O, s.scratch, w.bnr, training, &s.mr, &s.ir, fr, nred));
        const int pad_y = i == 2 ? 0 : 1;
        void* y = X.alloc((size_t)B * (Tout + 2 * pad_y) * O * es);
        if (!X.dry) L_(timed(X, "bn_apply", 0, (double)B * Tout * O * es * 3, stream, [&] { return ss_bn_apply(dt, c2, s.m2, s.i2, w.bn2.gamma, w.bn2.beta, 0, cr, s.mr, s.ir, w.bnr.gamma, w.bnr.beta, 0, y, pad_y, B, Tout, O, 1, stream); }));
        s.c1 = c1; s.cr = cr; s.h1 = h1; s.c2 = c2; s.y = y; s.pad_y = pad_y;
        xin = y; Tin = Tout; Cin = O;
    }
    if (training && !X.dry) {
        long long* ctrs[9];
        for (int i = 0; i < 3; ++i) { ctrs[3 * i] = blk[i].bn1.nbt; ctrs[3 * i + 1] = blk[i].bn2.nbt; ctrs[3 * i + 2] = blk[i].bnr.nbt; }
        L_(timed(X, "counters", 0, 0, stream, [&] { return ss_counters_add(9, (int64_t**)ctrs, 1, stream); }));
    }
    const int T = Tin, M = B * T;
    c->T = T; c->M = M; c->conv_out = xin;
    void* x = X.alloc((size_t)M * d * es);
    { ss_gemm_epilogue e = EPI(); e.bias = b_raw_in; L_(gemm(X, dt, xin, w_raw_in, x, M, d, d, RM(d), RM(d), RM(d), &e, SS_OP_KC, SS_OP_KC, 1, 0, nullptr, 1)); }

    const int H = D.n_head, dp = D.dp, Dr = D.max_rel, ff = D.ff, HD = H * dp;
    const int Tp = round_up(T, 8);
    const float scale = 1.0f / sqrtf((float)D.d_qkv);
    c->Tp = Tp; c->scale = scale;
    const bool x3att = use_x3_attention(T);
    c->need_T = x3att ? 0 : ss_relpos_attention_needs_transposed(dt, T, dp, Dr);
    for (int l = 0; l < D.n_layers; ++l) {
        LayerP& w = layers[l]; LayerCtx& s = c->layer[l];
        s.x = x;
        void* qkv = X.alloc((size_t)M * 3 * HD * es);
        void* qkvT = nullptr;
        if (c->need_T) {
            qkvT = X.alloc((size_t)B * 3 * HD * Tp * es);
            ss_gemm_epilogue e = EPI(); e.c2 = qkvT; e.cmap2 = RM(1, T, (long long)3 * HD * Tp); e.col_stride2 = Tp;
            L_(gemm(X, dt, x, w.wqkv, qkv, M, 3 * HD, d, RM(d), RM(d), RM(3 * HD), &e));
        } else L_(gemm(X, dt, x, w.wqkv, qkv, M, 3 * HD, d, RM(d), RM(d), RM(3 * HD), nullptr, SS_OP_KC, SS_OP_KC, 1, 0, nullptr, x3att ? 2 : 0));
        void* o = X.alloc((size_t)M * HD * es);
        float* lse = (float*)X.alloc((size_t)B * H * T * 4);
        const size_t pimg_bytes = training ? (size_t)(x3att ? ss_relpos_attention_x3_saved_bytes(B, H, T, dp, Dr) : ss_relpos_attention_saved_bytes(dt, B, H, T, dp, Dr)) : 0;
        void* pimg = pimg_bytes ? X.alloc(pimg_bytes) : nullptr;
        if (x3att) {
            const Pl q = planes(X, qkv, qkv, (long long)M * 3 * HD);
            adopt_planes(o, o, (long long)M * HD);
            if (!X.dry) {
                if (!q.hi) return 1;
                L_(timed(X, "attn_fwd", 2.0 * B * H * band_pairs(T, Dr) * dp * 3.0, (double)M * 4 * HD * es, stream, [&] { return ss_relpos_attention_x3_forward(q.hi, q.lo, w.EF, o, (char*)o + (size_t)M * HD * 2, lse, pimg, B, H, T, dp, Dr, scale, p_drop, seed, 4 * l, stream); }));
            }
        } else
        if (!X.dry) L_(timed(X, "attn_fwd", 2.0 * B * H * band_pairs(T, Dr) * dp * 3.0, (double)M * 4 * HD * es, stream, [&] { return ss_relpos_attention_forward_p(dt == SS_F32 && f32_x3 ? SS_F32X3 : dt, qkv, qkvT, w.E, w.EF, o, lse, pimg, B, H, T, Tp, dp, Dr, scale, p_drop, seed, 4 * l, stream); }));
        s.pimg = pimg;
        void* a = X.alloc((size_t)M * d * es);
        L_(gemm(X, dt, o, w.wo, a, M, d, HD, RM(HD), RM(HD), RM(d)));
        void* y1 = X.alloc((size_t)M * d * es);
        float* mean1 = (float*)X.alloc((size_t)M * 4); float* rstd1 = (float*)X.alloc((size_t)M * 4);
        const Pl y1p = new_planes(X, y1, (long long)M * d);
        if (!X.dry) L_(timed(X, "add_dropout_ln_fwd", 0, (double)M * d * es * 5, stream, [&] { return ss_add_dropout_layernorm_forward_planes(dt, x, a, w.g1, w.be1, y1, y1p.hi, y1p.lo, mean1, rstd1, M, d, D.ln_eps, p_drop, seed, 4 * l + 1, stream); }));
        void* hid = X.alloc((size_t)M * ff * es);
        unsigned char* hid_sign = nullptr;
        { ss_gemm_epilogue e = EPI(); e.bias = w.b1; e.relu = 1; e.dropout_p = p_drop; e.seed = seed; e.rng_stream = 4 * l + 2;
          ss_rowmap am_ = RM(d), bm_ = RM(d), cm_ = RM(ff);
          if (training && dt == SS_BF16 && sign_gate && ff % 8 == 0 && ss_gemm_sign_bits_supported(dt, dt, SS_OP_KC, SS_OP_KC, hid, M, ff, d, &am_, &bm_, &cm_, &e, 1)) {
              hid_sign = (unsigned char*)X.alloc((size_t)M * (ff / 8));
              e.sign_out = hid_sign; e.sign_pitch = ff / 8;
          }
          L_(gemm(X, dt, y1, w.w1, hid, M, ff, d, am_, bm_, cm_, &e, SS_OP_KC, SS_OP_KC, 1, 0, nullptr, 1)); }
        void* f = X.alloc((size_t)M * d * es);
        { ss_gemm_epilogue e = EPI(); e.bias = w.b2; L_(gemm(X, dt, hid, w.w2, f, M, d, ff, RM(ff), RM(ff), RM(d), &e)); }
        void* y2 = X.alloc((size_t)M * d * es);
        float* mean2 = (float*)X.alloc((size_t)M * 4); float* rstd2 = (float*)X.alloc((size_t)M * 4);
        const Pl y2p = new_planes(X, y2, (long long)M * d);
        if (!X.dry) L_(timed(X, "add_dropout_ln_fwd", 0, (double)M * d * es * 5, stream, [&] { return ss_add_dropout_layernorm_forward_planes(dt, y1, f, w.g2, w.be2, y2, y2p.hi, y2p.lo, mean2, rstd2, M, d, D.ln_eps, p_drop, seed, 4 * l + 3, stream); }));
        s.qkv = qkv; s.qkvT = qkvT; s.o = o; s.lse = lse; s.z1 = a; s.mean1 = mean1; s.rstd1 = rstd1; s.y1 = y1;
        s.hid = hid; s.hid_sign = hid_sign; s.z2 = f; s.mean2 = mean2; s.rstd2 = rstd2;
        x = y2;
    }
    c->x_final = x;
    const int nh = D.n_head_cols;
    { ss_gemm_epilogue e = EPI(); e.bias = b_head; L_(gemm(X, SS_F32, x, w_head, head, M, nh, d, RM(d), RM(d), RM(nh), &e)); }
    c->ws_used = X.off;
    return 0;
}

int Plan::backward(Exec& X, Ctx* c, const float* dhead)
{
    const int dt = D.dtype, d = D.d_model; const size_t es = esz();
    const int B = c->B, T = c->T, M = c->M, H = D.n_head, dp = D.dp, Dr = D.max_rel, ff = D.ff, HD = H * dp, Tp = c->Tp, nh = D.n_head_cols;
    const float p_drop = c->p_drop, keep_scale = 1.0f / (1.0f - p_drop);
    const unsigned long long seed = c->seed;
    void* stream = X.stream;
    void* side = (side_enabled && X.side) ? X.side : X.stream;
    const bool overlapped = side != stream;
    X.side = side;
    Exec& XS = X;
    const bool grouped = (dt == SS_BF16 || use_planes()) && dw_grouped;
    cur = c;
    const bool x3att = use_x3_attention(T);

    const void* dh_t = dhead;
    if (dt != SS_F32) { void* t = X.alloc((size_t)M * nh * es); if (!X.dry) L_(timed(X, "cast", 0, (double)M * nh * (4 + es), stream, [&] { return ss_cast_f32(dhead, t, dt, (long long)M * nh, stream); })); dh_t = t; }
    if (!X.dry && stage_arena && stage_arena_bytes > 0) {
        if (!ss_memset_async(stage_arena, 0, (size_t)stage_arena_bytes, stream)) { ss_set_error("backward: memset failed"); return 1; }
    }
    const int old_blocks = ss_gemm_set_blocks_per_cu(overlapped ? side_blocks : 2);
    struct Restore { int v; ~Restore() { ss_gemm_set_blocks_per_cu(v); } } restore{old_blocks};
    ss_gemm_set_blocks_per_cu(2);
#define SIDE_BEGIN() do { fork(X); if (overlapped) ss_gemm_set_blocks_per_cu(side_blocks); } while (0)
#define SIDE_END() do { if (overlapped) ss_gemm_set_blocks_per_cu(2); } while (0)

    DwGroup grp{this, &XS, grouped};
    L_(grp.add(dh_t, c->x_final, head_w_stage, nh, d, M, RM(nh), RM(d), side));
    SIDE_BEGIN(); L_(colsum(X, dh_t, M, nh, head_b_stage, side)); SIDE_END();
    void* G = X.alloc((size_t)M * d * es);
    L_(gemm(X, dt, dh_t, w_head_T, G, M, d, nh, RM(nh), RM(nh), RM(d)));

    const int64_t ln_floats = ss_layernorm_backward_scratch_floats(M, d);
    float* ln_scratch = ln_floats ? (float*)X.alloc((size_t)ln_floats * 4) : nullptr;
    const bool per_layer = on_event != nullptr || !unpack_all.jobs;
    for (int l = c->n_layers - 1; l >= 0; --l) {
        LayerP& w = layers[l]; LayerCtx& s = c->layer[l];
        void* dF = X.alloc((size_t)M * d * es);
        const Pl dFp = ln_floats ? new_planes(X, dF, (long long)M * d) : Pl{nullptr, nullptr};
        if (!X.dry) L_(timed(X, "ln_bwd", 0, (double)M * d * es * 4, stream, [&] { return ss_layernorm_backward_ws_planes(dt, G, s.z2, s.mean2, s.rstd2, w.g2, G, dF, dFp.hi, dFp.lo, w.dg2, w.dbe2, w.db2, ln_scratch, ln_floats, M, d, p_drop, seed, 4 * l + 3, stream); }));
        L_(grp.add(dF, s.hid, w.dw2, d, ff, M, RM(d), RM(ff), side));
        void* dHid = X.alloc((size_t)M * ff * es);
        bool db1_fused = false;
        { ss_gemm_epilogue e = EPI(); e.gate = s.hid; e.gate_scale = keep_scale;
          ss_rowmap am_ = RM(d), bm_ = RM(d), cm_ = RM(ff);
          if (!X.dry && fuse_stats) {
              ss_gemm_epilogue es = e; es.col_sum = w.db1;
              if (s.hid_sign && !use_planes()) {
                  ss_gemm_epilogue eb = es; eb.gate = nullptr; eb.gate_bits = s.hid_sign; eb.gate_bits_pitch = ff / 8;
                  if (ss_gemm_fuses_column_stats(dt, dt, SS_OP_KC, SS_OP_KC, dHid, M, ff, d, &am_, &bm_, &cm_, &eb, 1) != 0) { e = eb; db1_fused = true; }
              }
              if (db1_fused) {}
              else if (use_planes() ? ss_gemm_planes_supported(SS_F32, dHid, M, ff, d, &am_, &bm_, &cm_, &es) != 0 : ss_gemm_fuses_column_stats(dt, dt, SS_OP_KC, SS_OP_KC, dHid, M, ff, d, &am_, &bm_, &cm_, &e, 1) != 0) { e = es; db1_fused = true; }
          }
          L_(gemm(X, dt, dF, w.w2T, dHid, M, ff, d, am_, bm_, cm_, &e, SS_OP_KC, SS_OP_KC, 1, 0, nullptr, db1_fused ? 2 : 1)); }
        L_(grp.add(dHid, s.y1, w.dw1, ff, d, M, RM(ff), RM(d), side));
        if (!db1_fused) { SIDE_BEGIN(); L_(colsum(X, dHid, M, ff, w.db1, side)); SIDE_END(); }
        { ss_gemm_epilogue e = EPI(); e.mode = 1; L_(gemm(X, dt, dHid, w.w1T, G, M, d, ff, RM(ff), RM(ff), RM(d), &e)); }
        void* dA = X.alloc((size_t)M * d * es);
        const Pl dAp = ln_floats ? new_planes(X, dA, (long long)M * d) : Pl{nullptr, nullptr};
        if (!X.dry) L_(timed(X, "ln_bwd", 0, (double)M * d * es * 4, stream, [&] { return ss_layernorm_backward_ws_planes(dt, G, s.z1, s.mean1, s.rstd1, w.g1, G, dA, dAp.hi, dAp.lo, w.dg1, w.dbe1, nullptr, ln_scratch, ln_floats, M, d, p_drop, seed, 4 * l + 1, stream); }));
        L_(grp.add(dA, s.o, w.wo_stage, d, HD, M, RM(d), RM(HD), side));
        void* dO = X.alloc((size_t)M * HD * es);
        void* dOT = nullptr;
        if (c->need_T) {
            dOT = X.alloc((size_t)B * HD * Tp * es);
            ss_gemm_epilogue e = EPI(); e.c2 = dOT; e.cmap2 = RM(1, T, (long long)HD * Tp); e.col_stride2 = Tp;
            L_(gemm(X, dt, dA, w.woT, dO, M, HD, d, RM(d), RM(d), RM(HD), &e));
        } else L_(gemm(X, dt, dA, w.woT, dO, M, HD, d, RM(d), RM(d), RM(HD), nullptr, SS_OP_KC, SS_OP_KC, 1, 0, nullptr, x3att ? 2 : 0));
        void* dqkv = X.alloc((size_t)M * 3 * HD * es);
        float* dsc = (float*)X.alloc((size_t)B * H * T * 4);
        if (x3att) {
            const Pl q = planes(X, s.qkv, s.qkv, (long long)M * 3 * HD), ol = planes(X, s.o, s.o, (long long)M * HD), dop = planes(X, dO, dO, (long long)M * HD);
            adopt_planes(dqkv, dqkv, (long long)M * 3 * HD);
            if (!X.dry) {
                if (!q.hi || !ol.hi || !dop.hi) return 1;
                L_(timed(X, "attn_bwd", 2.0 * B * H * band_pairs(T, Dr) * dp * 5.0, (double)M * 8 * HD * es, stream, [&] { return ss_relpos_attention_x3_backward(q.hi, q.lo, w.EF, ol.hi, ol.lo, dop.hi, dop.lo, dsc, dqkv, (char*)dqkv + (size_t)M * 3 * HD * 2, s.pimg, B, H, T, dp, Dr, c->scale, p_drop, seed, 4 * l, stream); }));
            }
        } else
        if (!X.dry) L_(timed(X, "attn_bwd", 2.0 * B * H * band_pairs(T, Dr) * dp * 5.0, (double)M * 8 * HD * es, stream, [&] { return ss_relpos_attention_backward_p(dt == SS_F32 && f32_x3 ? SS_F32X3 : dt, s.qkv, s.qkvT, w.E, w.ET, w.EF, s.o, s.lse, dO, dOT, dsc, dqkv, s.pimg, B, H, T, Tp, dp, Dr, c->scale, p_drop, seed, 4 * l, stream); }));
        L_(grp.add(dqkv, s.x, w.wqkv_stage, 3 * HD, d, M, RM(3 * HD), RM(d), side));
        { ss_gemm_epilogue e = EPI(); e.mode = 1; L_(gemm(X, dt, dqkv, w.wqkvT, G, M, d, 3 * HD, RM(3 * HD), RM(3 * HD), RM(d), &e)); }
        if (l > 0) {
            SIDE_BEGIN(); L_(grp.launch(side)); if (per_layer) L_(permute_batch(X, w.unpack, side)); SIDE_END();
            if (on_event && !X.dry) on_event(event_user, 4 + l, side);
        }
    }
    L_(grp.add(G, c->conv_out, dw_raw_in, d, d, M, RM(d), RM(d), side));
    SIDE_BEGIN(); L_(grp.launch(side)); L_(colsum(X, G, M, d, db_raw_in, side));
    if (per_layer) {
        if (c->n_layers > 0) L_(permute_batch(X, layers[0].unpack, side));
        L_(permute_batch(X, unpack_enc, side));
    } else L_(permute_batch(X, unpack_all, side));
    SIDE_END();
    if (on_event && !X.dry) {
        if (c->n_layers > 0) on_event(event_user, 4, side);
        on_event(event_user, 0, side);
    }
    void* dy = X.alloc((size_t)M * d * es);
    L_(gemm(X, dt, G, w_raw_in_T, dy, M, d, d, RM(d), RM(d), RM(d)));

    const bool regate = regate_on != 0;
    for (int i = 2; i >= 0; --i) {
        BlockP& w = blk[i]; BlockCtx& s = c->blk[i];
        const int O = s.O, Cin = s.Cin, Tin = s.Tin, Tout = s.Tout, rows = B * Tout;
        const long long pbs = (long long)(Tout + 2) * O;
        void* dc2 = X.alloc((size_t)B * (Tout + 2) * O * es);
        void* dcr = X.alloc((size_t)rows * O * es);
        float* sums = (float*)X.alloc((size_t)3 * O * 4);
        if (!X.dry) {
            L_(timed(X, "bn_bwd_sums", 0, (double)B * Tout * O * es * (regate ? 3 : 4), stream, [&] { return ss_bn_backward_sums(dt, dy, 0, s.y, s.pad_y, s.c2, 0, s.m2, s.i2, s.cr, 0, s.mr, s.ir, w.bn2.dgamma, w.bn2.dbeta, w.bnr.dgamma, w.bnr.dbeta, s.scratch, sums, B, Tout, O, 1, regate ? w.bn2.gamma : nullptr, regate ? w.bn2.beta : nullptr, regate ? w.bnr.gamma : nullptr, regate ? w.bnr.beta : nullptr, stream); }));
            double n_total = (double)B * Tout;
            if (hook) n_total = hook(hook_user, sums, 3 * O, n_total, stream);
            L_(timed(X, "bn_bwd_apply", 0, (double)B * Tout * O * es * (regate ? 5 : 6), stream, [&] { return ss_bn_backward_apply(dt, dy, 0, s.y, s.pad_y, s.c2, 0, s.m2, s.i2, w.bn2.gamma, s.cr, 0, s.mr, s.ir, w.bnr.gamma, sums, n_total, dc2, 1, dcr, 0, B, Tout, O, 1, regate ? w.bn2.beta : nullptr, regate ? w.bnr.beta : nullptr, stream); }));
        }
        DwGroup cg{this, &XS, grouped};
        L_(cg.add(dc2, s.h1, w.c2_stage, O, 3 * O, rows, RM(O, Tout, pbs, O), RM(O, Tout, pbs), side));
        void* dh1 = X.alloc((size_t)rows * O * es);
        L_(gemm(X, dt, dc2, w.w2b, dh1, rows, O, 3 * O, RM(O, Tout, pbs), RM(3 * O), RM(O)));
        void* dc1 = X.alloc((size_t)B * (Tout + 2) * O * es);
        float* sums1 = (float*)X.alloc((size_t)3 * O * 4);
        if (!X.dry) {
            L_(timed(X, "bn_bwd_sums", 0, (double)B * Tout * O * es * (regate ? 2 : 3), stream, [&] { return ss_bn_backward_sums(dt, dh1, 0, s.h1, 1, s.c1, 0, s.m1, s.i1, nullptr, 0, nullptr, nullptr, w.bn1.dgamma, w.bn1.dbeta, nullptr, nullptr, s.scratch, sums1, B, Tout, O, 1, regate ? w.bn1.gamma : nullptr, regate ? w.bn1.beta : nullptr, nullptr, nullptr, stream); }));
            double n_total = (double)B * Tout;
            if (hook) n_total = hook(hook_user, sums1, 3 * O, n_total, stream);
            L_(timed(X, "bn_bwd_apply", 0, (double)B * Tout * O * es * (regate ? 3 : 4), stream, [&] { return ss_bn_backward_apply(dt, dh1, 0, s.h1, 1, s.c1, 0, s.m1, s.i1, w.bn1.gamma, nullptr, 0, nullptr, nullptr, nullptr, sums1, n_total, dc1, 1, nullptr, 0, B, Tout, O, 1, regate ? w.bn1.beta : nullptr, nullptr, stream); }));
        }
        const long long in_bs = (long long)(Tin + 2) * Cin;
        L_(cg.add(dc1, s.xin, w.c1_stage, O, 3 * Cin, rows, RM(O, Tout, pbs, O), RM(2 * Cin, Tout, in_bs), side));
        L_(cg.add(dcr, s.xin, w.wr_grad, O, Cin, rows, RM(O, Tout, (long long)Tout * O), RM(2 * Cin, Tout, in_bs, Cin), side));
        SIDE_BEGIN(); L_(cg.launch(side)); L_(permute_batch(X, w.unpack, side)); SIDE_END();
        if (on_event && !X.dry) on_event(event_user, 1 + (2 - i), side);
        if (i > 0) {
            void* dx = X.alloc((size_t)B * Tin * Cin * es);
            const ss_rowmap out_even = RM(2 * Cin, Tout, (long long)Tin * Cin), out_odd = RM(2 * Cin, Tout, (long long)Tin * Cin, Cin);
            L_(gemm(X, dt, dc1, w.w1b_even, dx, rows, Cin, O, RM(O, Tout, pbs, O), RM(O), out_even));
            { ss_gemm_epilogue e = EPI(); e.mode = 1; L_(gemm(X, dt, dcr, w.wrT, dx, rows, Cin, O, RM(O), RM(O), out_even, &e)); }
            L_(gemm(X, dt, dc1, w.w1b_odd, dx, rows, Cin, 2 * O, RM(O, Tout, pbs, O), RM(2 * O), out_odd));
            dy = dx;
        }
    }
    join(X);
#undef SIDE_BEGIN
#undef SIDE_END
    c->ws_used = X.off;
    return 0;
}

}

struct ss_plan { Plan* p; };

extern "C" ss_plan* ss_plan_create(const ss_model_dims* dims)
{
    if (!dims || dims->n_layers < 0 || dims->n_layers > MAX_LAYERS || dims->d_model % 8 || (dims->dtype != SS_F32 && dims->dtype != SS_BF16)) { ss_set_error("ss_plan_create: bad model dimensions"); return nullptr; }
    ss_plan* h = new ss_plan; h->p = new Plan(*dims);
#if !defined(SS_EMU)
    hipEventCreateWithFlags(&h->p->ev_fork, hipEventDisableTiming); hipEventCreateWithFlags(&h->p->ev_join, hipEventDisableTiming);
#endif
    return h;
}
extern "C" void ss_plan_destroy(ss_plan* h)
{
    if (!h) return;
#if !defined(SS_EMU)
    if (h->p->ev_fork) hipEventDestroy(h->p->ev_fork);
    if (h->p->ev_join) hipEventDestroy(h->p->ev_join);
#endif
    delete h->p; delete h;
}
extern "C" int ss_plan_slot_count(const ss_plan* h) { return h ? (int)h->p->names.size() : 0; }
extern "C" const char* ss_plan_slot_name(const ss_plan* h, int i) { return (h && i >= 0 && i < (int)h->p->names.size()) ? h->p->names[i].c_str() : nullptr; }
extern "C" int ss_plan_bind(ss_plan* h, int i, void* ptr)
{
    SS_CHECK(h && i >= 0 && i < (int)h->p->names.size(), "ss_plan_bind: bad slot %d", i);
    *h->p->targets[i] = ptr;
    return 0;
}
extern "C" int ss_plan_set_option(ss_plan* h, int what, int value)
{
    SS_CHECK(h, "ss_plan_set_option: null plan");
    int old = -1;
    if (what == 0) { old = h->p->side_enabled; h->p->side_enabled = value; }
    else if (what == 1) { old = h->p->dw_grouped; h->p->dw_grouped = value; }
    else if (what == 2) { old = h->p->side_blocks; h->p->side_blocks = value >= 1 && value <= 2 ? value : 2; }
    else if (what == 3) { old = h->p->fuse_stats; h->p->fuse_stats = value; }
    else if (what == 4) { old = h->p->regate_on; h->p->regate_on = value; }
    else if (what == 5) { old = h->p->f32_x3; h->p->f32_x3 = value != 0; }
    else if (what == 6) { old = h->p->keep_input; h->p->keep_input = value != 0; }
    else if (what == 7) { old = h->p->x3_planes; h->p->x3_planes = value != 0; }
    else if (what == 9) { old = h->p->x3_emit; h->p->x3_emit = value != 0; }
    else if (what == 10) { old = h->p->sign_gate; h->p->sign_gate = value != 0; }
    else if (what == 8) { old = h->p->x3_attn; h->p->x3_attn = value != 0; }
    return old;
}
extern "C" int ss_plan_set_reduce_hook(ss_plan* h, ss_reduce_hook fn, void* user) { SS_CHECK(h, "null plan"); h->p->hook = (reduce_fn)fn; h->p->hook_user = user; return 0; }
extern "C" int ss_plan_set_event_hook(ss_plan* h, ss_event_hook fn, void* user) { SS_CHECK(h, "null plan"); h->p->on_event = (event_fn)fn; h->p->event_user = user; return 0; }
extern "C" int64_t ss_plan_ctx_bytes(void) { return (int64_t)sizeof(Ctx); }

extern "C" int ss_plan_profile(ss_plan* h, int enable)
{
    SS_CHECK(h, "ss_plan_profile: null plan");
    const int old = h->p->profiling ? 1 : 0;
    h->p->profiling = enable != 0;
    return old;
}
extern "C" int ss_plan_profile_read(ss_plan* h, ss_profile_row* rows, int max_rows)
{
    SS_CHECK(h && rows && max_rows > 0, "ss_plan_profile_read: bad arguments");
    int n = 0;
#if !defined(SS_EMU)
    Plan* P = h->p;
    static const char* gemm_names[5] = {"gemm_kernel (128x128, register-staged)", "gemm_glds_kernel (128x128)", "gemm_w2_kernel (128|144 x 128)", "gemm8_kc_kernel (256x256)", "gemm8_kc_kernel (288x256)"};
    for (const Plan::ProfRec& r : P->recs) {
        hipEventSynchronize(r.e1);
        float ms = 0.f; hipEventElapsedTime(&ms, r.e0, r.e1);
        const char* name = r.tag;
        double flops = r.flops;
        if (!strcmp(r.tag, "gemm") && r.sub >= 0 && r.sub < 5) name = gemm_names[r.sub];
        else if (!strcmp(r.tag, "gemm") && r.sub == 5) { name = "gemm_smallk_kernel (K <= 32, first conv)"; flops = 0; }
        else if (!strcmp(r.tag, "gemm_dw")) name = "gemm_kernel<OC,OC> (128x128 dW, split-K atomics)";
        int k = 0;
        for (; k < n; ++k) if (!strcmp(rows[k].name, name)) break;
        if (k == n) { if (n == max_rows) continue; memset(&rows[n], 0, sizeof(rows[n])); strncpy(rows[n].name, name, sizeof(rows[n].name) - 1); ++n; }
        rows[k].calls += 1; rows[k].seconds += ms * 1e-3; rows[k].flops += flops; rows[k].bytes += r.bytes;
    }
    P->recs.clear(); P->ev_used = 0;
#else
    (void)h; (void)rows; (void)max_rows;
#endif
    return n;
}

extern "C" int64_t ss_plan_workspace_bytes(ss_plan* h, int B, int T0, int training)
{
    if (!h) return -1;
    Exec X{true, nullptr, 0, 0, nullptr, nullptr};
    Ctx c; memset(&c, 0, sizeof(c));
    if (h->p->forward(X, nullptr, nullptr, B, T0, training, 0, 0.f, 0, nullptr, &c)) return -1;
    if (training && h->p->backward(X, &c, nullptr)) return -1;
    return (int64_t)((X.off + 255) & ~(size_t)255) + 256;
}

extern "C" int ss_plan_forward(ss_plan* h, const float* x_raw, float* shifted_scratch, void* workspace, int64_t workspace_bytes, int B, int T0, int training, int shift_r,
                               float dropout_p, uint64_t seed, float* head, void* ctx_out, void* stream)
{
    SS_CHECK(h && x_raw && workspace && head && ctx_out, "ss_plan_forward: null pointer");
    for (size_t i = 0; i < h->p->targets.size(); ++i) {
        const std::string& n = h->p->names[i];
        const bool optional = n.find(".grad") != std::string::npos || n.find(".stage") != std::string::npos || n.find("unpack") != std::string::npos || n.find("stage_arena") != std::string::npos ||
                              n.find("num_batches_tracked") != std::string::npos;
        SS_CHECK(*h->p->targets[i] || optional, "ss_plan_forward: slot '%s' is not bound", n.c_str());
    }
    Exec X{false, (char*)workspace, 0, (size_t)workspace_bytes, stream, nullptr};
    Ctx* c = (Ctx*)ctx_out; memset(c, 0, sizeof(Ctx));
    c->ws = (char*)workspace; c->ws_bytes = (unsigned long long)workspace_bytes;
    const int64_t need = ss_plan_workspace_bytes(h, B, T0, training);
    SS_CHECK(need >= 0 && need <= workspace_bytes, "ss_plan_forward: workspace of %lld bytes, %lld needed", (long long)workspace_bytes, (long long)need);
    return h->p->forward(X, x_raw, shifted_scratch, B, T0, training, shift_r, dropout_p, seed, head, c);
}

extern "C" int ss_plan_backward(ss_plan* h, void* ctx, const float* dhead, void* stream, void* side_stream)
{
    SS_CHECK(h && ctx && dhead, "ss_plan_backward: null pointer");
    Ctx* c = (Ctx*)ctx;
    SS_CHECK(c->ws && c->M > 0, "ss_plan_backward: context of an eval-mode or failed forward");
    for (size_t i = 0; i < h->p->targets.size(); ++i) SS_CHECK(*h->p->targets[i] || h->p->names[i].find("w1b_") != std::string::npos, "ss_plan_backward: slot '%s' is not bound", h->p->names[i].c_str());
    Exec X{false, c->ws, (size_t)c->ws_used, (size_t)c->ws_bytes, stream, side_stream};
    return h->p->backward(X, c, dhead);
}
```

silent_speech_amd/engine.py:

```python
import ctypes
import math
import os

import torch

from . import _lib, ops
from ._lib import OP_KC, OP_OC

RM = ops.rowmap


def _round_up(x, m):
    return (x + m - 1) // m * m


class Prepared(object):

    def __init__(self, model):
        self.build(model)

    @staticmethod
    def layout_signature(model):
        return (tuple(p.data_ptr() for p in model.all_parameters()), model.compute_dtype, str(model.w_out.weight.device))

# ... 23 lines not shown
        for blk in model.conv_blocks:
            O, I, _ = blk.conv1.weight.shape
            e = {}
            w1, w2 = blk.conv1.weight.detach(), blk.conv2.weight.detach()
            e['w1f'] = b1.add(w1, new(O, 3 * I), (O, 3, I), (3 * I, 1, 3))
            e['w2f'] = b1.add(w2, new(O, 3 * O), (O, 3, O), (3 * O, 1, 3))
            e['wr'] = b1.add(blk.residual_path.weight.detach(), new(O, I), (O, 1, I), (I, 0, 1))
            e['wrT'] = transposed(e['wr'], O, I)
            e['w2b'] = b1.add(w2.view(-1)[2:], new(O, 3 * O), (O, 3, O), (3, -1, 3 * O))
            if I % 8 == 0:
                e['w1b_even'] = b1.add(w1.view(-1)[1:], new(I, O), (I, 1, O), (3, 0, 3 * I))
                e['w1b_odd'] = b1.add(w1.view(-1)[2:], new(I, 2 * O), (I, 2, O), (3, -2, 3 * I))
            self.blocks.append(e)

        self.w_raw_in = cast(model.w_raw_in.weight)
        self.w_raw_in_T = transposed(self.w_raw_in, d, d)
        H, dh, dp, D = model.n_head, model.d_qkv, model.dp, model.max_rel
        MPt = _round_up(2 * D - 1, 32)
        self.layers = []
        for layer in model.transformer.layers:
            a = layer.self_attn
            e = {}
            wqkv = new(3, H, dp, d)
            for i, w in enumerate((a.w_q, a.w_k, a.w_v)):
                b1.add(w.detach(), wqkv[i], (H, dp, d), (d * dh, 1, dh), valid1=dh)
            e['wqkv'] = wqkv.view(3 * H * dp, d)
            e['wqkvT'] = transposed(e['wqkv'], 3 * H * dp, d)
            e['wo'] = b1.add(a.w_o.detach(), new(d, H * dp), (d, H, dp), (1, dh * d, d), valid2=dh)
            e['woT'] = transposed(e['wo'], d, H * dp)
            emb = a.relative_positional.embeddings.detach()
            e['E'] = b1.add(emb, new(H, 2 * D - 1, dp), (H, 2 * D - 1, dp), ((2 * D - 1) * dh, dh, 1), valid2=dh)
            e['ET'] = b1.add(emb, new(H, dp, MPt), (H, dp, MPt), ((2 * D - 1) * dh, 1, dh), valid1=dh, valid2=2 * D - 1)
            nb = int(_lib.lib().ss_relpos_attention_table_bytes(H, dp, D)) if dt == torch.bfloat16 else int(_lib.lib().ss_relpos_attention_x3_table_bytes(H, dp, D))
            e['EF.x3'] = dt != torch.bfloat16 and nb > 0
            e['EF'] = new(max(nb // 2, 8), dtype=torch.bfloat16)
            e['EF.src'], e['EF.version'], e['EF.scale'] = a.relative_positional.embeddings, None, 1.0 / math.sqrt(dh)
            e['w1'] = cast(layer.linear1.weight)
            e['w2'] = cast(layer.linear2.weight)
            e['w1T'] = transposed(e['w1'], layer.linear1.weight.shape[0], d)
            e['w2T'] = transposed(e['w2'], d, layer.linear2.weight.shape[1])
            self.layers.append(e)
        n_out = model.w_out.weight.shape[0]
        n_aux = model.w_aux.weight.shape[0] if model.has_aux_out else 0
        nh = _round_up(n_out + n_aux, 8)
        wh = new(nh, d, zero=True)
        bh = new(nh, dtype=torch.float32, zero=True)
        b1.add(model.w_out.weight.detach(), wh[:n_out], (1, n_out, d), (0, d, 1))
        b1.add(model.w_out.bias.detach(), bh[:n_out], (1, 1, n_out), (0, 0, 1))
        if n_aux:
            b1.add(model.w_aux.weight.detach(), wh[n_out:n_out + n_aux], (1, n_aux, d), (0, d, 1))
            b1.add(model.w_aux.bias.detach(), bh[n_out:n_out + n_aux], (1, 1, n_aux), (0, 0, 1))
        self.w_head, self.b_head, self.n_head_cols = wh, bh, nh
        self.w_head_T = transposed(wh, nh, d)
        self.layout_sig = self.layout_signature(model)
        self.refresh(model)

    def refresh(self, model):
        self.b1.run(self.dev)
        self.b2.run(self.dev)
        for e in self.layers:
            src = e['EF.src']
            if e['EF'].numel() > 8 and e['EF.version'] != (src._version, src.data_ptr()):
                (ops.relpos_attention_x3_tables if e['EF.x3'] else ops.relpos_attention_tables)(src, model.dp, e['EF.scale'], out=e['EF'])
                e['EF.version'] = (src._version, src.data_ptr())
        self.version_sig = self.version_signature(model)


def prepared(model):
    pr = getattr(model, '_prepared', None)
    if pr is None or pr.layout_sig != Prepared.layout_signature(model):
        pr = Prepared(model)
        model._prepared = pr
    elif pr.version_sig != Prepared.version_signature(model):
        pr.refresh(model)
    return pr


class ModelDims(ctypes.Structure):
    _fields_ = [('d_model', ctypes.c_int32), ('n_layers', ctypes.c_int32), ('n_head', ctypes.c_int32), ('d_qkv', ctypes.c_int32),
                ('dp', ctypes.c_int32), ('max_rel', ctypes.c_int32), ('ff', ctypes.c_int32), ('n_head_cols', ctypes.c_int32),
                ('dtype', ctypes.c_int32), ('ln_eps', ctypes.c_float)]


class GradUnpack(object):

    def __init__(self, model, dev):
        d, H, dh, dp = model.d_model, model.n_head, model.d_qkv, model.dp
        pr = prepared(model)
        nh = pr.n_head_cols
        sizes = [('head_w', nh * d), ('head_b', nh)]
        for l in range(len(model.transformer.layers)):
            sizes += [('wo%d' % l, d * H * dp), ('wqkv%d' % l, 3 * H * dp * d)]
        for i, blk in enumerate(model.conv_blocks):
            O, I, _ = blk.conv1.weight.shape
            sizes += [('c2_%d' % i, O * 3 * O), ('c1_%d' % i, O * 3 * I)]
        total = sum((n + 3) // 4 * 4 for _, n in sizes)
        self.arena = torch.zeros(total, dtype=torch.float32, device=dev)
        self.buf, off = {}, 0
        for k, n in sizes:
            self.buf[k] = self.arena[off:off + n]
            off += (n + 3) // 4 * 4
        ub = ops.PermuteBatch()
        n_out = model.w_out.weight.shape[0]
        n_aux = model.w_aux.weight.shape[0] if model.has_aux_out else 0
        hw, hb = self.buf['head_w'].view(nh, d), self.buf['head_b']
        ub.add(hw[:n_out], model.w_out.weight.grad, (1, n_out, d), (0, d, 1), accumulate=True)
        ub.add(hb[:n_out], model.w_out.bias.grad, (1, 1, n_out), (0, 0, 1), accumulate=True)
        if n_aux:
            ub.add(hw[n_out:n_out + n_aux], model.w_aux.weight.grad, (1, n_aux, d), (0, d, 1), accumulate=True)
            ub.add(hb[n_out:n_out + n_aux], model.w_aux.bias.grad, (1, 1, n_aux), (0, 0, 1), accumulate=True)
        self.head_batch = ub
        ua = ops.PermuteBatch()
        ua.add(hw[:n_out], model.w_out.weight.grad, (1, n_out, d), (0, d, 1), accumulate=True)
        ua.add(hb[:n_out], model.w_out.bias.grad, (1, 1, n_out), (0, 0, 1), accumulate=True)
        if n_aux:
            ua.add(hw[n_out:n_out + n_aux], model.w_aux.weight.grad, (1, n_aux, d), (0, d, 1), accumulate=True)
            ua.add(hb[n_out:n_out + n_aux], model.w_aux.bias.grad, (1, 1, n_aux), (0, 0, 1), accumulate=True)
        self.all_batch = ua
        self.layer_batches = []
        for l, layer in enumerate(model.transformer.layers):
            a = layer.self_attn
            lb = ops.PermuteBatch()
            lb.add(self.buf['wo%d' % l], a.w_o.grad, (H, dh, d), (dp, 1, H * dp), accumulate=True)
            for i, wp in enumerate((a.w_q, a.w_k, a.w_v)):
                lb.add(self.buf['wqkv%d' % l][i * H * dp * d:], wp.grad, (H, d, dh), (dp * d, 1, d), accumulate=True)
            self.layer_batches.append(lb)
            ua.add(self.buf['wo%d' % l], a.w_o.grad, (H, dh, d), (dp, 1, H * dp), accumulate=True)
            for i, wp in enumerate((a.w_q, a.w_k, a.w_v)):
                ua.add(self.buf['wqkv%d' % l][i * H * dp * d:], wp.grad, (H, d, dh), (dp * d, 1, d), accumulate=True)
        self.conv_batches = []
        for i, blk in enumerate(model.conv_blocks):
            O, I, _ = blk.conv1.weight.shape
            cb = ops.PermuteBatch()
            cb.add(self.buf['c2_%d' % i], blk.conv2.weight.grad, (O, O, 3), (3 * O, 1, O), accumulate=True)
            cb.add(self.buf['c1_%d' % i], blk.conv1.weight.grad, (O, I, 3), (3 * I, 1, I), accumulate=True)
            self.conv_batches.append(cb)
        self.sig = self.signature(model)

    @staticmethod
    def signature(model):
        return (model._gflat.data_ptr() if getattr(model, '_gflat', None) is not None else 0,
                tuple(p.grad.data_ptr() for p in model.optimized_parameters()), str(model.w_out.weight.device))


def grad_unpack(model, dev):
    gu = getattr(model, '_grad_unpack', None)
    if gu is None or gu.sig != GradUnpack.signature(model):
        gu = GradUnpack(model, dev)
        model._grad_unpack = gu
    return gu


SIDE_STREAM_ENABLED = True


def _split_k(M, N, K):
    tiles = ((M + 127) // 128) * ((N + 127) // 128)
    overlapped = SIDE_STREAM_ENABLED and os.environ.get('SS_AMD_SIDE_STREAM', '1') != '0'
    s = max(1, min(64, (400 if overlapped else 512) // max(tiles, 1)))
    return max(1, min(s, K // 512 if K >= 512 else 1))


_REDUCE_HOOK = ctypes.CFUNCTYPE(ctypes.c_double, ctypes.c_void_p, ctypes.c_void_p, ctypes.c_int, ctypes.c_double, ctypes.c_void_p)
_EVENT_HOOK = ctypes.CFUNCTYPE(None, ctypes.c_void_p, ctypes.c_int, ctypes.c_void_p)


class PlanBinding(object):

    def __init__(self, model):
        L = _lib.lib()
        pr = prepared(model)
        layer0 = model.transformer.layers[0] if len(model.transformer.layers) else None
        dims = ModelDims(model.d_model, len(model.transformer.layers), model.n_head, model.d_qkv, model.dp, model.max_rel,
                         layer0.linear1.weight.shape[0] if layer0 is not None else 0, pr.n_head_cols, _lib.dtype_code(model.compute_dtype),
                         float(layer0.norm1.eps) if layer0 is not None else 1e-5)
        self.handle = L.ss_plan_create(ctypes.byref(dims))
        if not self.handle:
            raise RuntimeError('ss_plan_create failed: %s' % L.ss_last_error().decode())
        self.lib = L
        self.names = [L.ss_plan_slot_name(self.handle, i).decode() for i in range(L.ss_plan_slot_count(self.handle))]
        self.sig = None
        self.layout = (model.d_model, len(model.transformer.layers), model.compute_dtype)
        self.ctx_bytes = int(L.ss_plan_ctx_bytes())
        self.keep = None
        self.ws = None
        self._hook = self._hook_fn = None
        self._event = self._event_fn = None
        self.callback_error = None

    def __del__(self):
        try:
            if self.handle:
                self.lib.ss_plan_destroy(self.handle)
        except Exception:
            pass

    @staticmethod
    def _table(model, pr, gu, dev):
        t = {}

        def bn(prefix, m, grads):
            t[prefix + '.weight'], t[prefix + '.bias'] = m.weight, m.bias
            t[prefix + '.running_mean'], t[prefix + '.running_var'], t[prefix + '.num_batches_tracked'] = m.running_mean, m.running_var, m.num_batches_tracked
            if grads:
                t[prefix + '.weight.grad'], t[prefix + '.bias.grad'] = m.weight.grad, m.bias.grad

        def batch(prefix, pb):
            jobs, jb, total = pb.device_tables(dev)
            t[prefix + '.jobs'], t[prefix + '.blocks'], t[prefix + '.total'], t[prefix + '.all_f32'] = jobs, jb, int(total), 1

        g = gu is not None
        for i, (blk, w) in enumerate(zip(model.conv_blocks, pr.blocks)):
            p = 'conv_blocks.%d.' % i
            for k in ('w1f', 'w2f', 'wr', 'wrT', 'w2b', 'w1b_even', 'w1b_odd'):
                if k in w:
                    t[p + k] = w[k]
            t[p + 'conv1.bias'], t[p + 'residual_path.bias'], t[p + 'conv2.bias'] = blk.conv1.bias, blk.residual_path.bias, blk.conv2.bias
            bn(p + 'bn1', blk.bn1, g); bn(p + 'bn2', blk.bn2, g); bn(p + 'res_norm', blk.res_norm, g)
            if g:
                t[p + 'conv2.weight.stage'], t[p + 'conv1.weight.stage'] = gu.buf['c2_%d' % i], gu.buf['c1_%d' % i]
                t[p + 'residual_path.weight.grad'] = blk.residual_path.weight.grad
                batch(p + 'unpack', gu.conv_batches[i])
        t['w_raw_in'], t['w_raw_in_T'], t['w_raw_in.bias'] = pr.w_raw_in, pr.w_raw_in_T, model.w_raw_in.bias
        if g:
            t['w_raw_in.weight.grad'], t['w_raw_in.bias.grad'] = model.w_raw_in.weight.grad, model.w_raw_in.bias.grad
        for l, (layer, w) in enumerate(zip(model.transformer.layers, pr.layers)):
            p = 'transformer.layers.%d.' % l
            for k in ('wqkv', 'wqkvT', 'wo', 'woT', 'E', 'ET', 'EF', 'w1', 'w2', 'w1T', 'w2T'):
                t[p + k] = w[k]
            t[p + 'linear1.bias'], t[p + 'linear2.bias'] = layer.linear1.bias, layer.linear2.bias
            t[p + 'norm1.weight'], t[p + 'norm1.bias'], t[p + 'norm2.weight'], t[p + 'norm2.bias'] = layer.norm1.weight, layer.norm1.bias, layer.norm2.weight, layer.norm2.bias
            if g:
                for k in ('norm1.weight', 'norm1.bias', 'norm2.weight', 'norm2.bias', 'linear1.weight', 'linear1.bias', 'linear2.weight', 'linear2.bias'):
                    mod, attr = k.split('.')
                    t[p + k + '.grad'] = getattr(getattr(layer, mod), attr).grad
                t[p + 'w_o.stage'], t[p + 'w_qkv.stage'] = gu.buf['wo%d' % l], gu.buf['wqkv%d' % l]
                batch(p + 'unpack', gu.layer_batches[l])
        t['w_head'], t['w_head_T'], t['b_head'] = pr.w_head, pr.w_head_T, pr.b_head
        if g:
            t['head_w.stage'], t['head_b.stage'] = gu.buf['head_w'], gu.buf['head_b']
            t['stage_arena'], t['stage_arena.bytes'] = gu.arena, int(gu.arena.numel() * 4)
            batch('unpack_encoder', gu.head_batch)
            batch('unpack_encoder_all', gu.all_batch)
        return t

    def ensure_bound(self, model, pr, gu, dev):
        sig = (pr.layout_sig, gu.sig if gu is not None else None, tuple(b.data_ptr() for b in model.all_buffers()))
        if sig == self.sig:
            return
        table = self._table(model, pr, gu, dev)
        for i, n in enumerate(self.names):
            v = table.get(n)
            if v is None:
                val = None
            elif isinstance(v, int):
                val = ctypes.c_void_p(v)
            else:
                val = _lib.ptr(v.detach() if v.requires_grad else v)
            _lib.check(self.lib.ss_plan_bind(self.handle, i, val), 'ss_plan_bind')
        self.keep, self.sig = table, sig

    def set_reduce_hook(self, fn):
        if fn is self._hook_fn:
            return
        self._hook_fn = fn
        if fn is None:
            self._hook = None
            self.lib.ss_plan_set_reduce_hook(self.handle, ctypes.cast(None, _REDUCE_HOOK), None)
            return

        def trampoline(user, sums_ptr, n_floats, n_local, stream):
            try:
                off = int(sums_ptr) - self.ws.data_ptr()
                sums = self.ws[off:off + 4 * n_floats].view(torch.float32)
                return float(fn(sums, n_local))
            except BaseException as e:
                self.callback_error = self.callback_error or e
                return float(n_local)
        self._hook = _REDUCE_HOOK(trampoline)
        self.lib.ss_plan_set_reduce_hook(self.handle, self._hook, None)

    def set_event_hook(self, fn):
        if fn is self._event_fn:
            return
        self._event_fn = fn
        if fn is None:
            self._event = None
            self.lib.ss_plan_set_event_hook(self.handle, ctypes.cast(None, _EVENT_HOOK), None)
            return
        def trampoline(user, what, stream):
            try:
                fn(int(what), int(stream or 0))
            except BaseException as e:
                self.callback_error = self.callback_error or e
        self._event = _EVENT_HOOK(trampoline)
        self.lib.ss_plan_set_event_hook(self.handle, self._event, None)

    def raise_callback_error(self):
        e, self.callback_error = self.callback_error, None
        if e is not None:
            raise e


def plan_binding(model):
    pb = getattr(model, '_plan', None)
    if pb is None or pb.layout != (model.d_model, len(model.transformer.layers), model.compute_dtype):
        pb = PlanBinding(model)
        model._plan = pb
    return pb


def _side_stream(model, dev):
    if dev.type != 'cuda' or not SIDE_STREAM_ENABLED or os.environ.get('SS_AMD_SIDE_STREAM', '1') == '0':
        return None
    st = getattr(model, '_side_stream', None)
    if st is None or st.device != dev:
        st = torch.cuda.Stream(device=dev)
        model._side_stream = st
    return st


class Ctx(object):

    def __init__(self, buf, ws, M):
# ... 63 lines not shown
```

silent_speech_amd/ops.py:

```python
import ctypes

import torch

from . import _lib
from ._lib import OP_KC, OP_OC, RowMap, GemmEpilogue


def rowmap(row_stride, rows_per_batch=0, batch_stride=0, base=0):
    return RowMap(int(base), int(batch_stride), int(row_stride), int(rows_per_batch))


PROFILER = None


class LaunchProfiler(object):

    def __init__(self):
        self.records = []
        self.enabled = True

    def run(self, name, flops, nbytes, fn):
        if not self.enabled or not torch.cuda.is_available():
            return fn()
        s = torch.cuda.Event(enable_timing=True)
# ... 41 lines not shown
def _L():
    return _lib.lib()


def _p(t):
    return _lib.ptr(t)


def _s(t):
    return _lib.stream_of(t)


def _dt(t):
    return _lib.dtype_code(t.dtype)


_epi_defaults = dict(log_clamp=0.0, c2=None, cmap2=None, col_stride2=0, sign_out=None, gate_bits=None)


def gemm_ex(A, B, C, M, N, K, amap, bmap, cmap, **kw):
    extras = {k: kw.pop(k) for k in list(kw) if k in _epi_defaults}
    if not extras:
        return gemm(A, B, C, M, N, K, amap, bmap, cmap, **kw)
    return _gemm_full(A, B, C, M, N, K, amap, bmap, cmap, extras, **kw)


def _gemm_full(A, B, C, M, N, K, amap, bmap, cmap, extras, a_mode=OP_KC, b_mode=OP_KC, bias=None, relu=False, gate=None,
               gate_scale=1.0, alpha=1.0, dropout_p=0.0, seed=0, rng_stream=0, mode=0, split_k=1, col_perm=None, col_stats=None, f32_math='exact'):
    epi = GemmEpilogue()
    if col_stats is not None:
        cs, cq, sh = col_stats
        epi.col_sum, epi.col_sumsq, epi.col_shift = _p(cs).value, (_p(cq).value if cq is not None else None), (_p(sh).value if sh is not None else None)
    epi.bias = _p(bias).value if bias is not None else None
    epi.gate = _p(gate).value if gate is not None else None
    epi.gate_scale, epi.alpha, epi.relu, epi.dropout_p = gate_scale, alpha, int(bool(relu)), float(dropout_p)
    epi.seed, epi.rng_stream, epi.mode = int(seed) & 0xFFFFFFFFFFFFFFFF, int(rng_stream), int(mode)
    if col_perm is not None:
        epi.col_mod, epi.col_mul, epi.col_div_mul = col_perm
    epi.log_clamp = float(extras.get('log_clamp', 0.0))
    if extras.get('sign_out') is not None:
        assert extras['sign_out'].dtype == torch.uint8 and extras['sign_out'].numel() >= M * (N // 8)
        epi.sign_out, epi.sign_pitch = _p(extras['sign_out']).value, N // 8
    if extras.get('gate_bits') is not None:
        assert extras['gate_bits'].dtype == torch.uint8 and extras['gate_bits'].numel() >= M * (N // 8)
        epi.gate_bits, epi.gate_bits_pitch = _p(extras['gate_bits']).value, N // 8
    c2 = extras.get('c2')
    if c2 is not None:
        assert c2.dtype == C.dtype
        epi.c2 = _p(c2).value
        epi.cmap2 = extras['cmap2']
        epi.col_stride2 = int(extras['col_stride2'])
    assert A.dtype == B.dtype
    if bias is not None:
        assert bias.dtype == torch.float32 and bias.numel() >= N
    if gate is not None:
        assert gate.dtype == C.dtype

    dt_in = _dt(A)
    if f32_math != 'exact':
        if f32_math != 'bf16x3' or A.dtype != torch.float32:
            raise ValueError("f32_math is 'exact' or 'bf16x3', and 'bf16x3' needs float32 operands")
        dt_in = _lib.SS_F32X3

    def launch():
        rc = _L().ss_gemm(dt_in, _dt(C), a_mode, b_mode, _p(A), _p(B), _p(C), M, N, K, ctypes.byref(amap), ctypes.byref(bmap),
                          ctypes.byref(cmap), ctypes.byref(epi), split_k, _s(C))
        _lib.check(rc, 'ss_gemm')
    if PROFILER is not None and C.is_cuda:
        PROFILER.run('ss_gemm (from Python)', 2.0 * M * N * K, (M * K + N * K) * A.element_size() + M * N * C.element_size(), launch)
    else:
        launch()
    return C


GEMM_OPT_W2, GEMM_OPT_W2_BM, GEMM_OPT_G8, GEMM_OPT_G8_NI, GEMM_OPT_G8_PIN, GEMM_OPT_DEBUG, GEMM_OPT_SMALLK = range(7)


def gemm_set_option(what, value):
    return _L().ss_gemm_set_option(int(what), int(value))


def gemm_dw_grouped(jobs):
    flat = []
    for (dy, x, dw, M, N, K, amap, bmap, ldc) in jobs:
        if isinstance(dy, tuple):
            (dh, dl), (xh, xl) = dy, x
            flat += [(dl, xh, dw, M, N, K, amap, bmap, ldc, 1), (dh, xl, dw, M, N, K, amap, bmap, ldc, 1), (dh, xh, dw, M, N, K, amap, bmap, ldc, 1)]
        else:
            flat.append((dy, x, dw, M, N, K, amap, bmap, ldc, 0))
    cap = 24 if any(f[9] for f in flat) else 8
    for g0 in range(0, len(flat), cap):
        grp = flat[g0:g0 + cap]
        arr = (_lib.DwJob * len(grp))()
        for j, (dy, x, dw, M, N, K, amap, bmap, ldc, flags) in zip(arr, grp):
            assert dy.dtype == torch.bfloat16 and x.dtype == torch.bfloat16 and dw.dtype == torch.float32
            j.A, j.B, j.C = _p(dy).value, _p(x).value, _p(dw).value
            j.amap, j.bmap, j.ldc, j.M, j.N, j.K, j.flags = amap, bmap, int(ldc), int(M), int(N), int(K), flags
        _lib.check(_L().ss_gemm_dw_grouped(len(grp), arr, _s(grp[0][2])), 'ss_gemm_dw_grouped')


def split_planes(x):
    assert x.dtype == torch.float32 and x.is_contiguous()
    hi = torch.empty(x.shape, dtype=torch.bfloat16, device=x.device)
    lo = torch.empty(x.shape, dtype=torch.bfloat16, device=x.device)
    _lib.check(_L().ss_split_planes(_p(x), _p(hi), _p(lo), x.numel(), _s(x)), 'ss_split_planes')
    return hi, lo


def gemm_planes_supported(C, M, N, K, amap, bmap, cmap, epi=None):
    return bool(_L().ss_gemm_planes_supported(_lib.SS_F32, _p(C), M, N, K, ctypes.byref(amap), ctypes.byref(bmap), ctypes.byref(cmap), ctypes.byref(epi) if epi is not None else None))


def gemm_planes(A, B, C, M, N, K, amap, bmap, cmap, bias=None, relu=False, gate=None, gate_scale=1.0, alpha=1.0, dropout_p=0.0, seed=0, rng_stream=0,
                mode=0, col_stats=None, planes_out=None, planes_only=False):
    epi = GemmEpilogue()
    if planes_out is not None:
        assert all(t.dtype == torch.bfloat16 for t in planes_out)
        epi.planes_hi, epi.planes_lo, epi.planes_only = _p(planes_out[0]).value, _p(planes_out[1]).value, int(bool(planes_only))
    if col_stats is not None:
        cs, cq, sh = col_stats
        epi.col_sum, epi.col_sumsq, epi.col_shift = _p(cs).value, (_p(cq).value if cq is not None else None), (_p(sh).value if sh is not None else None)
    epi.bias = _p(bias).value if bias is not None else None
    epi.gate = _p(gate).value if gate is not None else None
    epi.gate_scale, epi.alpha, epi.relu, epi.dropout_p = gate_scale, alpha, int(bool(relu)), float(dropout_p)
    epi.seed, epi.rng_stream, epi.mode = int(seed) & 0xFFFFFFFFFFFFFFFF, int(rng_stream), int(mode)
    assert C.dtype == torch.float32 and all(t.dtype == torch.bfloat16 for t in (A[0], A[1], B[0], B[1]))
    rc = _L().ss_gemm_planes(_lib.SS_F32, _p(A[0]), _p(A[1]), _p(B[0]), _p(B[1]), _p(C), M, N, K, ctypes.byref(amap), ctypes.byref(bmap), ctypes.byref(cmap),
                             ctypes.byref(epi), _s(C))
    _lib.check(rc, 'ss_gemm_planes')
    return C


def bn_scratch(B, T, C, device):
    return torch.empty(int(_L().ss_bn_scratch_floats(B, T, C)), dtype=torch.float32, device=device)


def bn_stats(x, B, T, C, pad, scratch, running_mean, running_var, momentum=0.1, eps=1e-5, training=True, shift=None,
             reduce_fn=None):
    mean = torch.empty(C, dtype=torch.float32, device=x.device)
    invstd = torch.empty(C, dtype=torch.float32, device=x.device)
    n_total, sums = float(B * T), None
    if training:
        sums = torch.empty(3 * C, dtype=torch.float32, device=x.device)
        _lib.check(_L().ss_bn_stats_sums(_dt(x), _p(x), B, T, C, pad, _p(scratch), _p(shift), _p(sums), _s(x)), 'ss_bn_stats_sums')
        if reduce_fn is not None:
            n_total = reduce_fn(sums[:2 * C], n_total)
    rc = _L().ss_bn_finalize(_p(sums), n_total, C, _p(mean), _p(invstd), _p(running_mean), _p(running_var), momentum, eps, int(training), _s(x))
    _lib.check(rc, 'ss_bn_finalize')
    return mean, invstd


def bn_apply(xa, sa, pad_xa, y, pad_y, B, T, C, relu, xb=None, sb=None, pad_xb=0):
    n4 = [None] * 4
    b4 = sb if sb is not None else n4
    rc = _L().ss_bn_apply(_dt(xa), _p(xa), _p(sa[0]), _p(sa[1]), _p(sa[2]), _p(sa[3]), pad_xa,
                          _p(xb), _p(b4[0]), _p(b4[1]), _p(b4[2]), _p(b4[3]), pad_xb, _p(y), pad_y, B, T, C, int(relu), _s(xa))
    _lib.check(rc, 'ss_bn_apply')
    return y


def bn_backward(dy, pad_dy, y, pad_y, xa, pad_xa, sa, dxa, pad_dxa, dgamma_a, dbeta_a, scratch, B, T, C, relu,
                xb=None, pad_xb=0, sb=None, dxb=None, pad_dxb=0, dgamma_b=None, dbeta_b=None, reduce_fn=None, beta_a=None, beta_b=None):
    b3 = sb if sb is not None else [None] * 3
    gate = (sa[2], beta_a, b3[2], beta_b) if beta_a is not None else (None, None, None, None)
    sums = torch.empty(3 * C, dtype=torch.float32, device=dy.device)
    rc = _L().ss_bn_backward_sums(_dt(dy), _p(dy), pad_dy, _p(y), pad_y, _p(xa), pad_xa, _p(sa[0]), _p(sa[1]),
                                  _p(xb), pad_xb, _p(b3[0]), _p(b3[1]), _p(dgamma_a), _p(dbeta_a), _p(dgamma_b), _p(dbeta_b),
                                  _p(scratch), _p(sums), B, T, C, int(relu), _p(gate[0]), _p(gate[1]), _p(gate[2]), _p(gate[3]), _s(dy))
    _lib.check(rc, 'ss_bn_backward_sums')
    n_total = float(B * T)
    if reduce_fn is not None:
        n_total = reduce_fn(sums, n_total)
    rc = _L().ss_bn_backward_apply(_dt(dy), _p(dy), pad_dy, _p(y), pad_y, _p(xa), pad_xa, _p(sa[0]), _p(sa[1]), _p(sa[2]),
                                   _p(xb), pad_xb, _p(b3[0]), _p(b3[1]), _p(b3[2]), _p(sums), n_total, _p(dxa), pad_dxa, _p(dxb), pad_dxb,
                                   B, T, C, int(relu), _p(gate[1]), _p(gate[3]), _s(dy))
    _lib.check(rc, 'ss_bn_backward_apply')


def colsum(x, rows, C, ld, out_accum):
    scratch = torch.empty(int(_L().ss_colsum_scratch_floats(rows, C)), dtype=torch.float32, device=x.device)
    _lib.check(_L().ss_colsum(_dt(x), _p(x), rows, C, ld, _p(scratch), _p(out_accum), _s(x)), 'ss_colsum')


def add_dropout_layernorm(x, branch_inout, gamma, beta, y, rows, C, eps=1e-5, p=0.0, seed=0, rng_stream=0, planes=None):
    mean = torch.empty(rows, dtype=torch.float32, device=x.device)
    rstd = torch.empty(rows, dtype=torch.float32, device=x.device)
    rc = _L().ss_add_dropout_layernorm_forward_planes(_dt(x), _p(x), _p(branch_inout), _p(gamma), _p(beta), _p(y), _p(planes[0]) if planes else None, _p(planes[1]) if planes else None,
                                                      _p(mean), _p(rstd), rows, C, eps, p, int(seed) & 0xFFFFFFFFFFFFFFFF, rng_stream, _s(x))
    _lib.check(rc, 'ss_add_dropout_layernorm_forward')
    return mean, rstd


_ln_scratch = {}


def layernorm_backward(dy, z, mean, rstd, gamma, dres, dbranch, dgamma, dbeta, rows, C, p=0.0, seed=0, rng_stream=0, dbranch_colsum=None, planes=None):
    n = int(_L().ss_layernorm_backward_scratch_floats(rows, C))
    scratch = None
    if n:
        key = (str(dy.device), n, int(_s(dy).value or 0))
        scratch = _ln_scratch.get(key)
        if scratch is None:
            scratch = _ln_scratch[key] = torch.empty(n, dtype=torch.float32, device=dy.device)
    rc = _L().ss_layernorm_backward_ws_planes(_dt(dy), _p(dy), _p(z), _p(mean), _p(rstd), _p(gamma), _p(dres), _p(dbranch), _p(planes[0]) if planes else None,
                                              _p(planes[1]) if planes else None, _p(dgamma), _p(dbeta),
                                              _p(dbranch_colsum), _p(scratch), n, rows, C, p, int(seed) & 0xFFFFFFFFFFFFFFFF, rng_stream, _s(dy))
    _lib.check(rc, 'ss_layernorm_backward')


def emg_prepare(x_raw, out_padded, shifted_copy, B, T0, Cin, shift):
    rc = _L().ss_emg_prepare(_dt(out_padded), _p(x_raw), _p(out_padded), _p(shifted_copy), B, T0, Cin, shift, _s(x_raw))
    _lib.check(rc, 'ss_emg_prepare')


def adamw_step(p, g, m, v, n, lr, step, beta1=0.9, beta2=0.999, eps=1e-8, weight_decay=0.0, grad_scale=1.0):
    timed('adamw_kernel', 0, 28.0 * n,
          lambda: _lib.check(_L().ss_adamw_step(_p(p), _p(g), _p(m), _p(v), n, lr, beta1, beta2, eps, weight_decay, step, grad_scale, _s(p)), 'ss_adamw_step'))


def cast_f32(src, dst, n):
    _lib.check(_L().ss_cast_f32(_p(src), _p(dst), _dt(dst), n, _s(src)), 'ss_cast_f32')


def relpos_attention_saved_bytes(dtype, B, H, T, dp, D):
    return int(_L().ss_relpos_attention_saved_bytes(dtype if isinstance(dtype, int) else _lib.dtype_code(dtype), B, H, T, dp, D))


def _attn_dt(qkv, f32_math):
    if f32_math == 'exact':
        return _dt(qkv)
    if f32_math != 'bf16x3' or qkv.dtype != torch.float32:
        raise ValueError("f32_math is 'exact' or 'bf16x3', and 'bf16x3' needs float32 tensors")
    return _lib.SS_F32X3


def relpos_attention_family(dtype, T, dp, D):
    return int(_L().ss_relpos_attention_family(dtype if isinstance(dtype, int) else _lib.dtype_code(dtype), T, dp, D))


def relpos_attention_tables(emb, dp, scale, out=None):
    emb = emb.detach().reshape(emb.shape[0], emb.shape[1], -1).float().contiguous()
    H, NE, dh = emb.shape
    D = (NE + 1) // 2
    nbytes = int(_L().ss_relpos_attention_table_bytes(H, dp, D))
    if nbytes <= 0:
        raise ValueError('no transposed-score attention tables for H=%d dp=%d' % (H, dp))
    if out is None:
        out = torch.empty(nbytes // 2, dtype=torch.bfloat16, device=emb.device)
    _lib.check(_L().ss_relpos_attention_prepare_tables(_p(emb), _p(out), H, D, dh, dp, scale, _s(emb)), 'ss_relpos_attention_prepare_tables')
    return out


def _attn_tab(qkv, E, T, dp, D, scale, f32_math, tab):
    if tab is None and f32_math == 'exact' and relpos_attention_family(_dt(qkv), T, dp, D) == 2:
        tab = relpos_attention_tables(E, dp, scale)
    return tab


def relpos_attention_forward(qkv, qkvT, E, out, lse, B, H, T, Tp, dp, D, scale, p=0.0, seed=0, rng_stream=0, saved=None, f32_math='exact', tab=None):
    tab = _attn_tab(qkv, E, T, dp, D, scale, f32_math, tab)
    rc = _L().ss_relpos_attention_forward_p(_attn_dt(qkv, f32_math), _p(qkv), _p(qkvT), _p(E), _p(tab), _p(out), _p(lse), _p(saved), B, H, T, Tp, dp, D, scale, p,
                                            int(seed) & 0xFFFFFFFFFFFFFFFF, rng_stream, _s(qkv))
    _lib.check(rc, 'ss_relpos_attention_forward')

# ... 94 lines not shown
```

Before: 1.682 million.

## Write weight gradients directly into parameter layout from grouped dW GEMM epilogue

```diff
diff --git a/include/silent_speech_hip.h b/include/silent_speech_hip.h
--- a/include/silent_speech_hip.h
+++ b/include/silent_speech_hip.h
@@ -10,7 +10,7 @@
 #define SS_F32X3 3
 
 const char* ss_last_error(void);
-#define SS_ABI_VERSION 10
+#define SS_ABI_VERSION 11
 int ss_abi_version(void);
 const char* ss_target_arch(void);
 
@@ -77,6 +77,8 @@
     int64_t ldc;
     int32_t M, N, K;
     int32_t flags;
+    int32_t rs, r_valid, cs, c_valid;
+    int64_t r_hi, r_lo, c_hi, c_lo;
 } ss_dw_job;
 int ss_gemm_dw_grouped(int n_jobs, const ss_dw_job* jobs , void* stream);
 int ss_gemm_dw_set_option(int what, int value);
@@ -117,6 +119,7 @@
                          int B, int T, int C, int relu, const float* gate_beta_a, const float* gate_beta_b, void* stream);
 int64_t ss_colsum_scratch_floats(int rows, int C);
 int ss_colsum(int dtype, const void* x, int rows, int C, int64_t ld, float* scratch, float* out_accum, void* stream);
+int ss_colsum_split(int dtype, const void* x, int rows, int C, int64_t ld, float* scratch, float* out_a, int n_a, float* out_b, int n_b, void* stream);
 
 int ss_add_dropout_layernorm_forward(int dtype, const void* x, void* branch_inout, const float* gamma, const float* beta, void* y,
                                      float* mean, float* rstd, int rows, int C, float eps, float dropout_p, uint64_t seed,
diff --git a/silent_speech_amd/_lib.py b/silent_speech_amd/_lib.py
--- a/silent_speech_amd/_lib.py
+++ b/silent_speech_amd/_lib.py
@@ -7,7 +7,7 @@
 _LIB_PATH = os.environ.get('SS_AMD_LIBRARY') or os.path.join(_HERE, 'lib', 'libsilent_speech_hip.so')
 
 SS_F32, SS_BF16, SS_F64, SS_F32X3 = 0, 1, 2, 3
-ABI_VERSION = 10
+ABI_VERSION = 11
 OP_KC, OP_OC = 0, 1
 
 
@@ -29,7 +29,9 @@
 
 class DwJob(ctypes.Structure):
     _fields_ = [('A', ctypes.c_void_p), ('B', ctypes.c_void_p), ('C', ctypes.c_void_p), ('amap', RowMap), ('bmap', RowMap),
-                ('ldc', ctypes.c_int64), ('M', ctypes.c_int32), ('N', ctypes.c_int32), ('K', ctypes.c_int32), ('flags', ctypes.c_int32)]
+                ('ldc', ctypes.c_int64), ('M', ctypes.c_int32), ('N', ctypes.c_int32), ('K', ctypes.c_int32), ('flags', ctypes.c_int32),
+                ('rs', ctypes.c_int32), ('r_valid', ctypes.c_int32), ('cs', ctypes.c_int32), ('c_valid', ctypes.c_int32),
+                ('r_hi', ctypes.c_int64), ('r_lo', ctypes.c_int64), ('c_hi', ctypes.c_int64), ('c_lo', ctypes.c_int64)]
 
 
 class ProfileRow(ctypes.Structure):
@@ -75,6 +77,7 @@
     'ss_bn_backward_sums': [_I, _P, _I, _P, _I, _P, _I, _P, _P, _P, _I, _P, _P, _P, _P, _P, _P, _P, _P, _I, _I, _I, _I, _P, _P, _P, _P, _P],
     'ss_bn_backward_apply': [_I, _P, _I, _P, _I, _P, _I, _P, _P, _P, _P, _I, _P, _P, _P, _P, ctypes.c_double, _P, _I, _P, _I, _I, _I, _I, _I, _P, _P, _P],
     'ss_colsum': [_I, _P, _I, _I, _L, _P, _P, _P],
+    'ss_colsum_split': [_I, _P, _I, _I, _L, _P, _P, _I, _P, _I, _P],
     'ss_add_dropout_layernorm_forward': [_I, _P, _P, _P, _P, _P, _P, _P, _I, _I, _F, _F, _U64, _U32, _P],
     'ss_add_dropout_layernorm_forward_planes': [_I, _P, _P, _P, _P, _P, _P, _P, _P, _P, _I, _I, _F, _F, _U64, _U32, _P],
     'ss_layernorm_backward': [_I, _P, _P, _P, _P, _P, _P, _P, _P, _P, _I, _I, _F, _U64, _U32, _P],
diff --git a/silent_speech_amd/csrc/gemm8_dw.hip b/silent_speech_amd/csrc/gemm8_dw.hip
--- a/silent_speech_amd/csrc/gemm8_dw.hip
+++ b/silent_speech_amd/csrc/gemm8_dw.hip
@@ -3,12 +3,36 @@
 struct DwJob {
     const bf16_t* A; const bf16_t* B; float* C;
     RowMap amap, bmap;
-    long long ldc;
     int M, N, K;
     int tiles_n, ntiles, split, k_chunk, item0, nitem, atomic;
+    int rs, r_valid, cs, c_valid, r_hi, r_lo, c_hi, c_lo;
 };
 constexpr int DW_MAX_JOBS = 24;
 struct DwJobs { DwJob job[DW_MAX_JOBS]; int n; };
+static_assert(sizeof(DwJobs) <= 4096, "the job table travels as kernel arguments");
+
+struct DwOut {
+    float* C; int M, N, atomic, rs, r_valid, r_hi, r_lo;
+    __device__ __forceinline__ explicit DwOut(const DwJob& J) : C(J.C), M(J.M), N(J.N), atomic(J.atomic), rs(J.rs), r_valid(J.r_valid), r_hi(J.r_hi), r_lo(J.r_lo) {}
+    __device__ __forceinline__ static long long col_offset(const DwJob& J, int col) {
+        const int g = (int)((unsigned)col / (unsigned)J.cs), r = col - g * J.cs;
+        return (col < J.N && r < J.c_valid) ? (long long)g * J.c_hi + (long long)r * J.c_lo : -1;
+    }
+    template <int NJ>
+    __device__ __forceinline__ void rows4(int row0, const long long (&coff)[NJ], const f32x4 (&acc)[NJ]) const {
+        int g = (int)((unsigned)row0 / (unsigned)rs), r = row0 - g * rs;
+#pragma unroll
+        for (int reg = 0; reg < 4; ++reg) {
+            if (row0 + reg < M && r < r_valid) {
+                float* rowp = C + ((long long)g * r_hi + (long long)r * r_lo);
+#pragma unroll
+                for (int j = 0; j < NJ; ++j)
+                    if (coff[j] >= 0) { if (atomic) atomicAdd(rowp + coff[j], acc[j][reg]); else rowp[coff[j]] += acc[j][reg]; }
+            }
+            if (++r == rs) { r = 0; ++g; }
+        }
+    }
+};
 
 namespace g8 {
 constexpr int TRP = 544;
@@ -145,25 +169,15 @@
             if (more) st.store(lds + (cur ^ 1) * TR_STAGE, ra, rb);
             __syncthreads();
         }
-        const DwJob& J = jobs.job[ji];
-        float* Cj = J.C; const long long ldc = J.ldc; const int Mj = J.M, Nj = J.N, atomic = J.atomic, cm0 = m0, cn0 = n0;
+        const DwOut out(jobs.job[ji]);
+        long long coff[NJ];
+#pragma unroll
+        for (int j = 0; j < NJ; ++j) coff[j] = DwOut::col_offset(jobs.job[ji], n0 + (wn * NJ + j) * 16 + c);
+        const int cm0 = m0;
         const bool has_next = it + G < nitems;
         if (has_next) { it += G; G8_SETUP(); }
 #pragma unroll
-        for (int i = 0; i < 8; ++i)
-#pragma unroll
-            for (int j = 0; j < NJ; ++j) {
-                const int col = cn0 + (wn * NJ + j) * 16 + c, row0 = cm0 + (wm * 8 + i) * 16 + q * 4;
-                if (col < Nj) {
-#pragma unroll
-                    for (int reg = 0; reg < 4; ++reg) {
-                        if (row0 + reg < Mj) {
-                            float* dst = Cj + (long long)(row0 + reg) * ldc + col;
-                            if (atomic) atomicAdd(dst, acc[i][j][reg]); else *dst += acc[i][j][reg];
-                        }
-                    }
-                }
-            }
+        for (int i = 0; i < 8; ++i) out.rows4(cm0 + (wm * 8 + i) * 16 + q * 4, coff, acc[i]);
         if (!has_next) break;
     }
 #undef G8_SETUP
@@ -386,25 +400,16 @@
             };
             if (SHIFT && opsel) run(std::integral_constant<int, 2>{}); else run(std::integral_constant<int, 0>{});
         }
-        const DwJob& J = jobs.job[ji];
-        float* Cj = J.C; const long long ldc = J.ldc; const int Mj = J.M, Nj = J.N, atomic = J.atomic, cm0 = m0, cn0 = n0;
+        const DwOut out(jobs.job[ji]);
+        long long coff[4];
+#pragma unroll
+        for (int j = 0; j < 4; ++j) coff[j] = DwOut::col_offset(jobs.job[ji], n0 + (wn * 4 + j) * 16 + c);
+        const int cm0 = m0;
         const bool has_next = it + G < nitems;
         if (has_next) { it += G; G8K_SETUP(); }
 #pragma unroll
         for (int i = 0; i < 8; ++i)
-#pragma unroll
-            for (int j = 0; j < 4; ++j) {
-                const int col = cn0 + (wn * 4 + j) * 16 + c, row0 = cm0 + (wm * 8 + i) * 16 + q * 4;
-                if (col < Nj && !((ABL & 8) && acc[i][j][0] != 12345.f)) {
-#pragma unroll
-                    for (int reg = 0; reg < 4; ++reg) {
-                        if (row0 + reg < Mj) {
-                            float* dst = Cj + (long long)(row0 + reg) * ldc + col;
-                            if (atomic) atomicAdd(dst, acc[i][j][reg]); else *dst += acc[i][j][reg];
-                        }
-                    }
-                }
-            }
+            if (!((ABL & 8) && (acc[i][0][0] != 12345.f || acc[i][1][0] != 12345.f || acc[i][2][0] != 12345.f || acc[i][3][0] != 12345.f))) out.rows4(cm0 + (wm * 8 + i) * 16 + q * 4, coff, acc[i]);
         if (!has_next) break;
     }
 #undef G8K_SETUP
@@ -437,7 +442,18 @@
         for (int o = 0; o < 2; ++o)
             SS_CHECK(maps[o]->base % 8 == 0 && maps[o]->batch_stride % 8 == 0 && maps[o]->row_stride % 8 == 0, "ss_gemm_dw_grouped: job %d operand %d: strides must be multiples of 8 elements", i, o);
         DwJob& d = J.job[i];
-        d.A = (const bf16_t*)s.A; d.B = (const bf16_t*)s.B; d.C = s.C; d.ldc = s.ldc; d.M = s.M; d.N = s.N; d.K = s.K;
+        d.A = (const bf16_t*)s.A; d.B = (const bf16_t*)s.B; d.C = s.C; d.M = s.M; d.N = s.N; d.K = s.K;
+        const long long mapf[8] = {s.rs, s.r_valid, s.cs, s.c_valid, s.r_hi, s.r_lo, s.c_hi, s.c_lo};
+        bool dense = true;
+        for (int f = 0; f < 8; ++f) dense = dense && mapf[f] == 0;
+        if (dense) {
+            SS_CHECK(s.ldc >= s.N && s.ldc <= 0x7fffffff, "ss_gemm_dw_grouped: job %d: ldc=%lld must be in N..2^31-1", i, (long long)s.ldc);
+            d.rs = d.r_valid = d.cs = d.c_valid = 0x7fffffff; d.r_hi = 0; d.r_lo = (int)s.ldc; d.c_hi = 0; d.c_lo = 1;
+        } else {
+            SS_CHECK(s.rs > 0 && s.cs > 0 && s.r_valid > 0 && s.c_valid > 0, "ss_gemm_dw_grouped: job %d: output map needs rs, cs, r_valid, c_valid > 0", i);
+            for (int f = 4; f < 8; ++f) SS_CHECK(mapf[f] >= 0 && mapf[f] <= 0x7fffffff, "ss_gemm_dw_grouped: job %d: output map strides must be in 0..2^31-1", i);
+            d.rs = s.rs; d.r_valid = s.r_valid; d.cs = s.cs; d.c_valid = s.c_valid; d.r_hi = (int)s.r_hi; d.r_lo = (int)s.r_lo; d.c_hi = (int)s.c_hi; d.c_lo = (int)s.c_lo;
+        }
         d.amap.base = s.amap.base; d.amap.batch_stride = s.amap.batch_stride; d.amap.row_stride = s.amap.row_stride; d.amap.rows_per_batch = s.amap.rows_per_batch > 0 ? s.amap.rows_per_batch : 0x7fffffff;
         d.bmap.base = s.bmap.base; d.bmap.batch_stride = s.bmap.batch_stride; d.bmap.row_stride = s.bmap.row_stride; d.bmap.rows_per_batch = s.bmap.rows_per_batch > 0 ? s.bmap.rows_per_batch : 0x7fffffff;
         SS_CHECK(d.amap.rows_per_batch == d.bmap.rows_per_batch, "ss_gemm_dw_grouped: job %d: both operands must split their rows into batches of the same length", i);
diff --git a/silent_speech_amd/csrc/norm.hip b/silent_speech_amd/csrc/norm.hip
--- a/silent_speech_amd/csrc/norm.hip
+++ b/silent_speech_amd/csrc/norm.hip
@@ -618,6 +618,14 @@
     out[c] += t[0];
 }
 
+__global__ __launch_bounds__(256) void colsum_finalize_split_kernel(const float* __restrict__ partial, int nchunks, int C, float* __restrict__ out_a, int n_a, float* __restrict__ out_b, int n_b)
+{
+    float t[1]; int c;
+    if (!chunk_reduce<1>(partial, nchunks, C, t, c)) return;
+    if (c < n_a) out_a[c] += t[0];
+    else if (c - n_a < n_b) out_b[c - n_a] += t[0];
+}
+
 static int colsum_chunks(int rows) { int c = (rows + 31) / 32; if (c > 512) c = 512; if (c < 1) c = 1; return c; }
 extern "C" int64_t ss_colsum_scratch_floats(int rows, int C) { return (int64_t)colsum_chunks(rows) * C; }
 
@@ -631,6 +639,20 @@
     else SS_LAUNCH(colsum_partial_kernel<float>, dim3(nch), dim3(red_threads(C)), 0, stream, (const float*)x, rows, C, (long long)ld, rpc, scratch);
     SS_LAUNCH(colsum_finalize_kernel, dim3((C + 31) / 32), dim3(256), 0, stream, (const float*)scratch, nch, C, out_accum);
     SS_LAUNCH_CHECK("ss_colsum");
+    return 0;
+}
+
+extern "C" int ss_colsum_split(int dtype, const void* x, int rows, int C, int64_t ld, float* scratch, float* out_a, int n_a, float* out_b, int n_b, void* stream)
+{
+    SS_CHECK(x && out_a && scratch && (out_b || n_b == 0), "ss_colsum_split: null pointer");
+    SS_CHECK(C % 8 == 0 && C > 0 && rows >= 0 && ld % 8 == 0, "ss_colsum_split: C and ld must be multiples of 8");
+    SS_CHECK(n_a >= 0 && n_b >= 0 && n_a + n_b <= C, "ss_colsum_split: %d + %d destination columns of %d", n_a, n_b, C);
+    if (rows == 0) return 0;
+    const int nch = colsum_chunks(rows), rpc = (rows + nch - 1) / nch;
+    if (dtype == SS_BF16) SS_LAUNCH(colsum_partial_kernel<bf16_t>, dim3(nch), dim3(red_threads(C)), 0, stream, (const bf16_t*)x, rows, C, (long long)ld, rpc, scratch);
+    else SS_LAUNCH(colsum_partial_kernel<float>, dim3(nch), dim3(red_threads(C)), 0, stream, (const float*)x, rows, C, (long long)ld, rpc, scratch);
+    SS_LAUNCH(colsum_finalize_split_kernel, dim3((C + 31) / 32), dim3(256), 0, stream, (const float*)scratch, nch, C, out_a, n_a, out_b, n_b);
+    SS_LAUNCH_CHECK("ss_colsum_split");
     return 0;
 }
 
diff --git a/silent_speech_amd/csrc/plan.hip b/silent_speech_amd/csrc/plan.hip
--- a/silent_speech_amd/csrc/plan.hip
+++ b/silent_speech_amd/csrc/plan.hip
@@ -21,6 +21,7 @@
     void *wqkv = 0, *wqkvT = 0, *wo = 0, *woT = 0, *E = 0, *ET = 0, *EF = 0, *w1 = 0, *w2 = 0, *w1T = 0, *w2T = 0;
     float *b1 = 0, *b2 = 0, *g1 = 0, *be1 = 0, *g2 = 0, *be2 = 0;
     float *dg1 = 0, *dbe1 = 0, *dg2 = 0, *dbe2 = 0, *dw1 = 0, *db1 = 0, *dw2 = 0, *db2 = 0, *wo_stage = 0, *wqkv_stage = 0;
+    float *wo_grad = 0, *wq_grad = 0, *wk_grad = 0, *wv_grad = 0;
     PermB unpack;
 };
 
@@ -61,6 +62,8 @@
     void *w_raw_in = 0, *w_raw_in_T = 0, *w_head = 0, *w_head_T = 0;
     float *b_raw_in = 0, *dw_raw_in = 0, *db_raw_in = 0, *b_head = 0, *head_w_stage = 0, *head_b_stage = 0, *stage_arena = 0;
     long long stage_arena_bytes = 0;
+    float *w_out_grad = 0, *b_out_grad = 0, *w_aux_grad = 0, *b_aux_grad = 0;
+    long long n_out = 0, n_aux = 0;
     PermB unpack_enc, unpack_all;
     reduce_fn hook = 0; void* hook_user = 0;
     event_fn on_event = 0; void* event_user = 0;
@@ -139,11 +142,14 @@
             slot(p + "norm1.weight.grad", (void**)&L.dg1); slot(p + "norm1.bias.grad", (void**)&L.dbe1); slot(p + "norm2.weight.grad", (void**)&L.dg2); slot(p + "norm2.bias.grad", (void**)&L.dbe2);
             slot(p + "linear1.weight.grad", (void**)&L.dw1); slot(p + "linear1.bias.grad", (void**)&L.db1); slot(p + "linear2.weight.grad", (void**)&L.dw2); slot(p + "linear2.bias.grad", (void**)&L.db2);
             slot(p + "w_o.stage", (void**)&L.wo_stage); slot(p + "w_qkv.stage", (void**)&L.wqkv_stage);
+            slot(p + "w_o.grad", (void**)&L.wo_grad); slot(p + "w_q.grad", (void**)&L.wq_grad); slot(p + "w_k.grad", (void**)&L.wk_grad); slot(p + "w_v.grad", (void**)&L.wv_grad);
             slot_perm(p + "unpack", L.unpack);
         }
         slot("w_head", &w_head); slot("w_head_T", &w_head_T); slot("b_head", (void**)&b_head);
         slot("head_w.stage", (void**)&head_w_stage); slot("head_b.stage", (void**)&head_b_stage);
         slot("stage_arena", (void**)&stage_arena); slot("stage_arena.bytes", (void**)&stage_arena_bytes);
+        slot("w_out.weight.grad", (void**)&w_out_grad); slot("w_out.bias.grad", (void**)&b_out_grad); slot("w_aux.weight.grad", (void**)&w_aux_grad); slot("w_aux.bias.grad", (void**)&b_aux_grad);
+        slot("heads.n_out", (void**)&n_out); slot("heads.n_aux", (void**)&n_aux);
         slot_perm("unpack_encoder", unpack_enc); slot_perm("unpack_encoder_all", unpack_all);
     }
 
@@ -199,6 +205,11 @@
         if (X.dry) return 0;
         return timed(X, "colsum", 0, (double)rows * C * esz(), stream, [&] { return ss_colsum(D.dtype, x, rows, C, C, scratch, out, stream); });
     }
+    int colsum_split(Exec& X, const void* x, int rows, int C, float* out_a, int n_a, float* out_b, int n_b, void* stream) {
+        float* scratch = (float*)X.alloc((size_t)ss_colsum_scratch_floats(rows, C) * 4);
+        if (X.dry) return 0;
+        return timed(X, "colsum", 0, (double)rows * C * esz(), stream, [&] { return ss_colsum_split(D.dtype, x, rows, C, C, scratch, out_a, n_a, out_b, n_b, stream); });
+    }
     int permute_batch(Exec& X, const PermB& b, void* stream) {
         if (X.dry || !b.jobs || b.total <= 0) return 0;
         return timed(X, "grad_unlayout", 0, 0, stream, [&] { return ss_permute3d_batch(b.jobs, (const int32_t*)b.blocks, (int)b.total, (int)b.all_f32, stream); });
@@ -248,11 +259,16 @@
         return s < cap ? s : (cap < 1 ? 1 : cap);
     }
 
+    struct OutMap { int rs, r_valid; long long r_hi, r_lo; int cs, c_valid; long long c_hi, c_lo; };
+    static void set_map(ss_dw_job& j, const OutMap* om) {
+        if (!om) return;
+        j.rs = om->rs; j.r_valid = om->r_valid; j.r_hi = om->r_hi; j.r_lo = om->r_lo; j.cs = om->cs; j.c_valid = om->c_valid; j.c_hi = om->c_hi; j.c_lo = om->c_lo;
+    }
     struct DwGroup {
         Plan* P; Exec* X; bool grouped; int n = 0; ss_dw_job jobs[24];
-        int add(const void* dy, const void* x, float* grad, int N, int K, int rows, ss_rowmap am, ss_rowmap bm, void* stream) {
+        int add(const void* dy, const void* x, float* grad, int N, int K, int rows, ss_rowmap am, ss_rowmap bm, void* stream, const OutMap* om = nullptr) {
             if (grouped && P->use_planes()) {
-                if (n + 3 > 24 && launch(stream)) return 1;
+                if (n + 3 > 24 && flush(stream)) return 1;
                 const Pl a = P->planes(*X, dy, dy, extent(am, rows, N)), b = P->planes(*X, x, x, extent(bm, rows, K));
                 if (X->dry) return 0;
                 if (!a.hi || !b.hi) return 1;
@@ -260,20 +276,31 @@
                 for (int t = 0; t < 3; ++t) {
                     ss_dw_job& j = jobs[n++]; memset(&j, 0, sizeof(j));
                     j.A = as[t]; j.B = bs[t]; j.C = grad; j.amap = am; j.bmap = bm; j.ldc = K; j.M = N; j.N = K; j.K = rows; j.flags = 1;
+                    set_map(j, om);
                 }
                 return 0;
             }
             if (grouped) {
-                if (n == 8 && launch(stream)) return 1;
+                if (n == 8 && flush(stream)) return 1;
                 ss_dw_job& j = jobs[n++]; memset(&j, 0, sizeof(j));
                 j.A = dy; j.B = x; j.C = grad; j.amap = am; j.bmap = bm; j.ldc = K; j.M = N; j.N = K; j.K = rows;
+                set_map(j, om);
                 return 0;
             }
+            if (om) { ss_set_error("backward: an output-mapped weight gradient outside the grouped form"); return 1; }
             ss_gemm_epilogue e = EPI(); e.mode = 2;
             const bool ov = X->side && X->side != X->stream;
             P->fork(*X);
             if (ov) ss_gemm_set_blocks_per_cu(P->side_blocks);
             const int rc = P->gemm(*X, SS_F32, dy, x, grad, N, K, rows, am, bm, RM(K), &e, SS_OP_OC, SS_OP_OC, P->split_k(N, K, rows, ov), stream);
+            if (ov) ss_gemm_set_blocks_per_cu(2);
+            return rc;
+        }
+        int flush(void* stream) {
+            const bool ov = X->side && X->side != X->stream && stream == X->side;
+            P->fork(*X);
+            if (ov) ss_gemm_set_blocks_per_cu(P->side_blocks);
+            const int rc = launch(stream);
             if (ov) ss_gemm_set_blocks_per_cu(2);
             return rc;
         }
@@ -432,6 +459,20 @@
     const bool grouped = (dt == SS_BF16 || use_planes()) && dw_grouped;
     cur = c;
     const bool x3att = use_x3_attention(T);
+    const bool direct = grouped && !head_w_stage;
+    const int dh = D.d_qkv, n_o = (int)n_out, n_a = (int)n_aux;
+    if (!X.dry) {
+        if (direct) {
+            bool ok = w_out_grad && b_out_grad && n_o > 0 && (n_a == 0 || (w_aux_grad && b_aux_grad && n_o % 8 == 0)) && n_o + n_a <= nh;
+            for (int l = 0; l < c->n_layers; ++l) ok = ok && layers[l].wo_grad && layers[l].wq_grad && layers[l].wk_grad && layers[l].wv_grad;
+            SS_CHECK(ok, "ss_plan_backward: the grouped weight-gradient launches need every parameter-layout .grad slot bound");
+        } else {
+            bool ok = head_w_stage && head_b_stage && unpack_enc.jobs;
+            for (int l = 0; l < c->n_layers; ++l) ok = ok && layers[l].wo_stage && layers[l].wqkv_stage && layers[l].unpack.jobs;
+            SS_CHECK(ok, "ss_plan_backward: the staging buffers / un-layout tables of the weight gradients are not bound");
+        }
+        for (int i = 0; i < 3; ++i) SS_CHECK(blk[i].c1_stage && blk[i].c2_stage && blk[i].unpack.jobs, "ss_plan_backward: conv block %d: staging buffers / un-layout table not bound", i);
+    }
 
     const void* dh_t = dhead;
     if (dt != SS_F32) { void* t = X.alloc((size_t)M * nh * es); if (!X.dry) L_(timed(X, "cast", 0, (double)M * nh * (4 + es), stream, [&] { return ss_cast_f32(dhead, t, dt, (long long)M * nh, stream); })); dh_t = t; }
@@ -445,8 +486,15 @@
 #define SIDE_END() do { if (overlapped) ss_gemm_set_blocks_per_cu(2); } while (0)
 
     DwGroup grp{this, &XS, grouped};
-    L_(grp.add(dh_t, c->x_final, head_w_stage, nh, d, M, RM(nh), RM(d), side));
-    SIDE_BEGIN(); L_(colsum(X, dh_t, M, nh, head_b_stage, side)); SIDE_END();
+    if (direct) {
+        const OutMap mo{nh, n_o, 0, d, d, d, 0, 1}, ma{nh, n_a, 0, d, d, d, 0, 1};
+        L_(grp.add(dh_t, c->x_final, w_out_grad, n_a ? n_o : nh, d, M, RM(nh), RM(d), side, &mo));
+        if (n_a) L_(grp.add(dh_t, c->x_final, w_aux_grad, nh - n_o, d, M, RM(nh, 0, 0, n_o), RM(d), side, &ma));
+        SIDE_BEGIN(); L_(colsum_split(X, dh_t, M, nh, b_out_grad, n_o, b_aux_grad, n_a, side)); SIDE_END();
+    } else {
+        L_(grp.add(dh_t, c->x_final, head_w_stage, nh, d, M, RM(nh), RM(d), side));
+        SIDE_BEGIN(); L_(colsum(X, dh_t, M, nh, head_b_stage, side)); SIDE_END();
+    }
     void* G = X.alloc((size_t)M * d * es);
     L_(gemm(X, dt, dh_t, w_head_T, G, M, d, nh, RM(nh), RM(nh), RM(d)));
 
@@ -479,7 +527,10 @@
         void* dA = X.alloc((size_t)M * d * es);
         const Pl dAp = ln_floats ? new_planes(X, dA, (long long)M * d) : Pl{nullptr, nullptr};
         if (!X.dry) L_(timed(X, "ln_bwd", 0, (double)M * d * es * 4, stream, [&] { return ss_layernorm_backward_ws_planes(dt, G, s.z1, s.mean1, s.rstd1, w.g1, G, dA, dAp.hi, dAp.lo, w.dg1, w.dbe1, nullptr, ln_scratch, ln_floats, M, d, p_drop, seed, 4 * l + 1, stream); }));
-        L_(grp.add(dA, s.o, w.wo_stage, d, HD, M, RM(d), RM(HD), side));
+        if (direct) {
+            const OutMap om{dp, dh, (long long)dh * d, d, d, d, 0, 1};
+            L_(grp.add(s.o, dA, w.wo_grad, HD, d, M, RM(HD), RM(d), side, &om));
+        } else L_(grp.add(dA, s.o, w.wo_stage, d, HD, M, RM(d), RM(HD), side));
         void* dO = X.alloc((size_t)M * HD * es);
         void* dOT = nullptr;
         if (c->need_T) {
@@ -498,16 +549,21 @@
             }
         } else
         if (!X.dry) L_(timed(X, "attn_bwd", 2.0 * B * H * band_pairs(T, Dr) * dp * 5.0, (double)M * 8 * HD * es, stream, [&] { return ss_relpos_attention_backward_p(dt == SS_F32 && f32_x3 ? SS_F32X3 : dt, s.qkv, s.qkvT, w.E, w.ET, w.EF, s.o, s.lse, dO, dOT, dsc, dqkv, s.pimg, B, H, T, Tp, dp, Dr, c->scale, p_drop, seed, 4 * l, stream); }));
-        L_(grp.add(dqkv, s.x, w.wqkv_stage, 3 * HD, d, M, RM(3 * HD), RM(d), side));
+        if (direct) {
+            const OutMap om{d, d, 0, dh, dp, dh, (long long)d * dh, 1};
+            float* const gq[3] = {w.wq_grad, w.wk_grad, w.wv_grad};
+            for (int i = 2; i >= 0; --i) L_(grp.add(s.x, dqkv, gq[i], d, HD, M, RM(d), RM(3 * HD, 0, 0, (long long)i * HD), side, &om));
+        } else L_(grp.add(dqkv, s.x, w.wqkv_stage, 3 * HD, d, M, RM(3 * HD), RM(d), side));
         { ss_gemm_epilogue e = EPI(); e.mode = 1; L_(gemm(X, dt, dqkv, w.wqkvT, G, M, d, 3 * HD, RM(3 * HD), RM(3 * HD), RM(d), &e)); }
         if (l > 0) {
-            SIDE_BEGIN(); L_(grp.launch(side)); if (per_layer) L_(permute_batch(X, w.unpack, side)); SIDE_END();
+            SIDE_BEGIN(); L_(grp.launch(side)); if (per_layer && !direct) L_(permute_batch(X, w.unpack, side)); SIDE_END();
             if (on_event && !X.dry) on_event(event_user, 4 + l, side);
         }
     }
     L_(grp.add(G, c->conv_out, dw_raw_in, d, d, M, RM(d), RM(d), side));
     SIDE_BEGIN(); L_(grp.launch(side)); L_(colsum(X, G, M, d, db_raw_in, side));
-    if (per_layer) {
+    if (direct) {}
+    else if (per_layer) {
         if (c->n_layers > 0) L_(permute_batch(X, layers[0].unpack, side));
         L_(permute_batch(X, unpack_enc, side));
     } else L_(permute_batch(X, unpack_all, side));
@@ -668,7 +724,7 @@
     for (size_t i = 0; i < h->p->targets.size(); ++i) {
         const std::string& n = h->p->names[i];
         const bool optional = n.find(".grad") != std::string::npos || n.find(".stage") != std::string::npos || n.find("unpack") != std::string::npos || n.find("stage_arena") != std::string::npos ||
-                              n.find("num_batches_tracked") != std::string::npos;
+                              n.find("num_batches_tracked") != std::string::npos || n.find("heads.") != std::string::npos;
         SS_CHECK(*h->p->targets[i] || optional, "ss_plan_forward: slot '%s' is not bound", n.c_str());
     }
     Exec X{false, (char*)workspace, 0, (size_t)workspace_bytes, stream, nullptr};
@@ -684,7 +740,13 @@
     SS_CHECK(h && ctx && dhead, "ss_plan_backward: null pointer");
     Ctx* c = (Ctx*)ctx;
     SS_CHECK(c->ws && c->M > 0, "ss_plan_backward: context of an eval-mode or failed forward");
-    for (size_t i = 0; i < h->p->targets.size(); ++i) SS_CHECK(*h->p->targets[i] || h->p->names[i].find("w1b_") != std::string::npos, "ss_plan_backward: slot '%s' is not bound", h->p->names[i].c_str());
+    for (size_t i = 0; i < h->p->targets.size(); ++i) {
+        const std::string& n = h->p->names[i];
+        const bool optional = n.find("w1b_") != std::string::npos || n.find(".stage") != std::string::npos || n.find("unpack") != std::string::npos || n.find("stage_arena") != std::string::npos ||
+                              n.find("w_aux.") != std::string::npos || n.find("heads.") != std::string::npos || n.find("w_out.") != std::string::npos ||
+                              n.find("w_o.grad") != std::string::npos || n.find("w_q.grad") != std::string::npos || n.find("w_k.grad") != std::string::npos || n.find("w_v.grad") != std::string::npos;
+        SS_CHECK(*h->p->targets[i] || optional, "ss_plan_backward: slot '%s' is not bound", n.c_str());
+    }
     Exec X{false, c->ws, (size_t)c->ws_used, (size_t)c->ws_bytes, stream, side_stream};
     return h->p->backward(X, c, dhead);
 }
diff --git a/silent_speech_amd/engine.py b/silent_speech_amd/engine.py
--- a/silent_speech_amd/engine.py
+++ b/silent_speech_amd/engine.py
@@ -129,15 +129,24 @@
                 ('dtype', ctypes.c_int32), ('ln_eps', ctypes.c_float)]
 
 
+def dw_direct(model):
+    planes = model.compute_dtype == torch.float32 and model.f32_matmul == 'bf16x3' and os.environ.get('SS_AMD_X3_PLANES', '1') != '0'
+    grouped = (model.compute_dtype == torch.bfloat16 or planes) and os.environ.get('SS_AMD_DW_GROUPED', '1') != '0'
+    return grouped and (not model.has_aux_out or model.w_out.weight.shape[0] % 8 == 0)
+
+
 class GradUnpack(object):
 
     def __init__(self, model, dev):
         d, H, dh, dp = model.d_model, model.n_head, model.d_qkv, model.dp
         pr = prepared(model)
         nh = pr.n_head_cols
-        sizes = [('head_w', nh * d), ('head_b', nh)]
-        for l in range(len(model.transformer.layers)):
-            sizes += [('wo%d' % l, d * H * dp), ('wqkv%d' % l, 3 * H * dp * d)]
+        self.direct = dw_direct(model)
+        sizes = []
+        if not self.direct:
+            sizes += [('head_w', nh * d), ('head_b', nh)]
+            for l in range(len(model.transformer.layers)):
+                sizes += [('wo%d' % l, d * H * dp), ('wqkv%d' % l, 3 * H * dp * d)]
         for i, blk in enumerate(model.conv_blocks):
             O, I, _ = blk.conv1.weight.shape
             sizes += [('c2_%d' % i, O * 3 * O), ('c1_%d' % i, O * 3 * I)]
@@ -147,6 +156,16 @@
         for k, n in sizes:
             self.buf[k] = self.arena[off:off + n]
             off += (n + 3) // 4 * 4
+        self.conv_batches = []
+        for i, blk in enumerate(model.conv_blocks):
+            O, I, _ = blk.conv1.weight.shape
+            cb = ops.PermuteBatch()
+            cb.add(self.buf['c2_%d' % i], blk.conv2.weight.grad, (O, O, 3), (3 * O, 1, O), accumulate=True)
+            cb.add(self.buf['c1_%d' % i], blk.conv1.weight.grad, (O, I, 3), (3 * I, 1, I), accumulate=True)
+            self.conv_batches.append(cb)
+        self.sig = self.signature(model)
+        if self.direct:
+            return
         ub = ops.PermuteBatch()
         n_out = model.w_out.weight.shape[0]
         n_aux = model.w_aux.weight.shape[0] if model.has_aux_out else 0
@@ -175,19 +194,11 @@
             ua.add(self.buf['wo%d' % l], a.w_o.grad, (H, dh, d), (dp, 1, H * dp), accumulate=True)
             for i, wp in enumerate((a.w_q, a.w_k, a.w_v)):
                 ua.add(self.buf['wqkv%d' % l][i * H * dp * d:], wp.grad, (H, d, dh), (dp * d, 1, d), accumulate=True)
-        self.conv_batches = []
-        for i, blk in enumerate(model.conv_blocks):
-            O, I, _ = blk.conv1.weight.shape
-            cb = ops.PermuteBatch()
-            cb.add(self.buf['c2_%d' % i], blk.conv2.weight.grad, (O, O, 3), (3 * O, 1, O), accumulate=True)
-            cb.add(self.buf['c1_%d' % i], blk.conv1.weight.grad, (O, I, 3), (3 * I, 1, I), accumulate=True)
-            self.conv_batches.append(cb)
-        self.sig = self.signature(model)
 
     @staticmethod
     def signature(model):
         return (model._gflat.data_ptr() if getattr(model, '_gflat', None) is not None else 0,
-                tuple(p.grad.data_ptr() for p in model.optimized_parameters()), str(model.w_out.weight.device))
+                tuple(p.grad.data_ptr() for p in model.optimized_parameters()), str(model.w_out.weight.device), dw_direct(model))
 
 
 def grad_unpack(model, dev):
@@ -257,6 +268,7 @@
             t[prefix + '.jobs'], t[prefix + '.blocks'], t[prefix + '.total'], t[prefix + '.all_f32'] = jobs, jb, int(total), 1
 
         g = gu is not None
+        staged = g and not gu.direct
         for i, (blk, w) in enumerate(zip(model.conv_blocks, pr.blocks)):
             p = 'conv_blocks.%d.' % i
             for k in ('w1f', 'w2f', 'wr', 'wrT', 'w2b', 'w1b_even', 'w1b_odd'):
@@ -281,12 +293,19 @@
                 for k in ('norm1.weight', 'norm1.bias', 'norm2.weight', 'norm2.bias', 'linear1.weight', 'linear1.bias', 'linear2.weight', 'linear2.bias'):
                     mod, attr = k.split('.')
                     t[p + k + '.grad'] = getattr(getattr(layer, mod), attr).grad
+                a = layer.self_attn
+                t[p + 'w_o.grad'], t[p + 'w_q.grad'], t[p + 'w_k.grad'], t[p + 'w_v.grad'] = a.w_o.grad, a.w_q.grad, a.w_k.grad, a.w_v.grad
+            if staged:
                 t[p + 'w_o.stage'], t[p + 'w_qkv.stage'] = gu.buf['wo%d' % l], gu.buf['wqkv%d' % l]
                 batch(p + 'unpack', gu.layer_batches[l])
         t['w_head'], t['w_head_T'], t['b_head'] = pr.w_head, pr.w_head_T, pr.b_head
         if g:
+            t['w_out.weight.grad'], t['w_out.bias.grad'], t['heads.n_out'] = model.w_out.weight.grad, model.w_out.bias.grad, int(model.w_out.weight.shape[0])
+            if model.has_aux_out:
+                t['w_aux.weight.grad'], t['w_aux.bias.grad'], t['heads.n_aux'] = model.w_aux.weight.grad, model.w_aux.bias.grad, int(model.w_aux.weight.shape[0])
+            t['stage_arena'], t['stage_arena.bytes'] = gu.arena, int(gu.arena.numel() * 4)
+        if staged:
             t['head_w.stage'], t['head_b.stage'] = gu.buf['head_w'], gu.buf['head_b']
-            t['stage_arena'], t['stage_arena.bytes'] = gu.arena, int(gu.arena.numel() * 4)
             batch('unpack_encoder', gu.head_batch)
             batch('unpack_encoder_all', gu.all_batch)
         return t
diff --git a/silent_speech_amd/ops.py b/silent_speech_amd/ops.py
--- a/silent_speech_amd/ops.py
+++ b/silent_speech_amd/ops.py
@@ -147,20 +147,23 @@
 
 def gemm_dw_grouped(jobs):
     flat = []
-    for (dy, x, dw, M, N, K, amap, bmap, ldc) in jobs:
+    for job in jobs:
+        (dy, x, dw, M, N, K, amap, bmap, ldc), omap = job[:9], (job[9] if len(job) > 9 else None)
         if isinstance(dy, tuple):
             (dh, dl), (xh, xl) = dy, x
-            flat += [(dl, xh, dw, M, N, K, amap, bmap, ldc, 1), (dh, xl, dw, M, N, K, amap, bmap, ldc, 1), (dh, xh, dw, M, N, K, amap, bmap, ldc, 1)]
+            flat += [(dl, xh, dw, M, N, K, amap, bmap, ldc, 1, omap), (dh, xl, dw, M, N, K, amap, bmap, ldc, 1, omap), (dh, xh, dw, M, N, K, amap, bmap, ldc, 1, omap)]
         else:
-            flat.append((dy, x, dw, M, N, K, amap, bmap, ldc, 0))
+            flat.append((dy, x, dw, M, N, K, amap, bmap, ldc, 0, omap))
     cap = 24 if any(f[9] for f in flat) else 8
     for g0 in range(0, len(flat), cap):
         grp = flat[g0:g0 + cap]
         arr = (_lib.DwJob * len(grp))()
-        for j, (dy, x, dw, M, N, K, amap, bmap, ldc, flags) in zip(arr, grp):
+        for j, (dy, x, dw, M, N, K, amap, bmap, ldc, flags, omap) in zip(arr, grp):
             assert dy.dtype == torch.bfloat16 and x.dtype == torch.bfloat16 and dw.dtype == torch.float32
             j.A, j.B, j.C = _p(dy).value, _p(x).value, _p(dw).value
             j.amap, j.bmap, j.ldc, j.M, j.N, j.K, j.flags = amap, bmap, int(ldc), int(M), int(N), int(K), flags
+            if omap is not None:
+                j.rs, j.r_valid, j.r_hi, j.r_lo, j.cs, j.c_valid, j.c_hi, j.c_lo = (int(v) for v in omap)
         _lib.check(_L().ss_gemm_dw_grouped(len(grp), arr, _s(grp[0][2])), 'ss_gemm_dw_grouped')
 
 
@@ -245,6 +248,11 @@
 def colsum(x, rows, C, ld, out_accum):
     scratch = torch.empty(int(_L().ss_colsum_scratch_floats(rows, C)), dtype=torch.float32, device=x.device)
     _lib.check(_L().ss_colsum(_dt(x), _p(x), rows, C, ld, _p(scratch), _p(out_accum), _s(x)), 'ss_colsum')
+
+
+def colsum_split(x, rows, C, ld, out_a, n_a, out_b=None, n_b=0):
+    scratch = torch.empty(int(_L().ss_colsum_scratch_floats(rows, C)), dtype=torch.float32, device=x.device)
+    _lib.check(_L().ss_colsum_split(_dt(x), _p(x), rows, C, ld, _p(scratch), _p(out_a), int(n_a), _p(out_b), int(n_b), _s(x)), 'ss_colsum_split')
 
 
 def add_dropout_layernorm(x, branch_inout, gamma, beta, y, rows, C, eps=1e-5, p=0.0, seed=0, rng_stream=0, planes=None):
```

New measurement: 1.683 million (median of 3 runs). Within noise of the previous version (+0.0%).
